# mastbaum/sxmc

Hardware: AMD Instinct MI355X
Metric: NLL evals/sec (10^8 samples, 3 obs, 12 signals) + experiments/sec at 1/2/4/8 GPUs (higher is better)
Workload: dtype f64 exact; f32-on-u16-codes filter decides the unambiguous samples

## Files before the change

sxmc_amd/csrc/fill_kernels.inc.h:

```cpp
#pragma once

#include "sxmc_device_types.h"

#pragma clang fp contract(off)

#ifndef SXMC_MEASURE
#define SXMC_MEASURE 0
#endif

namespace sxfill {

__device__ __forceinline__ constexpr unsigned sx_dbg(unsigned dbg_arg) { return SXMC_MEASURE ? dbg_arg : 0u; }

template <int N>
struct IntC {
  static constexpr int value = N;
  constexpr operator int() const { return N; }
};
template <unsigned long... I>
struct ISeq {};
template <int N, unsigned long... I>
struct MakeISeq : MakeISeq<N - 1, (unsigned long)(N - 1), I...> {};
template <unsigned long... I>
struct MakeISeq<0, I...> {
// ... 350 lines not shown

    double lo[NOBS], hi[NOBS], sc[NOBS];
    int st[NOBS];
#pragma unroll
    for (int k = 0; k < NOBS; k++) {
      lo[k] = d.lower[k];
      hi[k] = d.upper[k];
      sc[k] = d.scale[k];
      st[k] = d.bin_stride[k];
    }

    unsigned cnt = 0;

    auto stage = [&](Columns<NSLOT, PREW>& buf, const unsigned long long vc) {
      double f[NSLOT][SXMC_VEC];
#pragma unroll
      for (int k = 0; k < NSLOT; k++) {
        if (slot_loaded<NOBS, PREW, PROG>(k)) {
          f[k][0] = (double)buf.v[k].x;
          f[k][1] = (double)buf.v[k].y;
          f[k][2] = (double)buf.v[k].z;
          f[k][3] = (double)buf.v[k].w;
        } else {
          f[k][0] = f[k][1] = f[k][2] = f[k][3] = 0.0;
        }
      }
      typename PreVec<PREW>::type prebits = buf.pre;
#pragma unroll
      for (int k = 0; k < NSLOT; k++) {
        if (slot_loaded<NOBS, PREW, PROG>(k)) {
#pragma unroll
          for (int q = 0; q < SXMC_VEC; q++) asm volatile("" : "+v"(f[k][q]));
        }
      }
      if constexpr (PREW != 0) asm volatile("" : "+v"(prebits));
      const unsigned long long vl = vc + step;
      load_columns<NOBS, NSLOT, PREW, PROG>(buf, col, precol, (vl < v1 && !(dbg & 2u)) ? vl : vlast);
      if (dbg & 1u) {
#pragma unroll
        for (int k = 0; k < NSLOT; k++) {
#pragma unroll
          for (int q = 0; q < SXMC_VEC; q++) cnt += (f[k][q] == 12345.678) ? 1u : 0u;
        }
        if constexpr (PREW != 0) cnt += (pre_value<PREW>(prebits, 0) == 12345u) ? 1u : 0u;
        return;
      }

      if constexpr (PROG::dynamic) {
        for (int s = 0; s < nsyst; s++) {
          apply_op<NSLOT>(f, (unsigned)__builtin_amdgcn_readlane((int)opword, s), coef);
        }
      } else {
        run_static<NSLOT>(f, craw, PROG{}, typename MakeISeq<PROG::n>::type{});
      }

      const unsigned dead = (vc < v1) ? 0u : 1u;
      unsigned okbin[SXMC_VEC];
#pragma unroll
      for (int q = 0; q < SXMC_VEC; q++) {
        unsigned bad = dead;
        int bin = 0;
        if constexpr (PREW != 0) {
          const unsigned pv = pre_value<PREW>(prebits, q);
          if constexpr (PREW != kPreGranule) bad += (pv == pre_sentinel<PREW>()) ? 1u : 0u;
          bin = (int)pv;
        }
#pragma unroll
        for (int k = 0; k < NOBS; k++) {
          if (!slot_loaded<NOBS, PREW, PROG>(k)) continue;
          const double x = f[k][q];
          bad += !(x >= lo[k]) ? 1u : 0u;
          bad += !(x < hi[k]) ? 1u : 0u;
          const int idx = (int)((x - lo[k]) * sc[k]);
          if (LDS_HIST) {
            bin = (k == NOBS - 1 && PREW != kPreGranule) ? bin + idx : __mul24(idx, st[k]) + bin;
          } else {
            bin += idx * st[k];
          }
        }
        const unsigned in_domain = (bad == 0u) ? 1u : 0u;
        cnt += in_domain;
        const bool store = (bad == 0u) && ((unsigned)bin < B) && !(dbg & 4u);
        if (LDS_HIST) {
          const unsigned slot = store ? (unsigned)bin : trash;
          __hip_atomic_fetch_add(&hist[slot], 1u, __ATOMIC_RELAXED, __HIP_MEMORY_SCOPE_WORKGROUP);
        } else {
          okbin[q] = store ? (unsigned)bin : 0xFFFFFFFFu;
        }
      }
      if (!LDS_HIST) {
        if (sparse) {
#pragma unroll
          for (int q = 0; q < SXMC_VEC; q++) {
            const unsigned hc = (okbin[q] != 0xFFFFFFFFu) ? (okbin[q] * 0xC2B2AE35u) >> cshift : 0u;
            const unsigned hd = (okbin[q] != 0xFFFFFFFFu) ? (okbin[q] * 0x27D4EB2Fu) >> cshift : 0u;
            if (!((hist[hc >> 5] >> (hc & 31u)) & (hist[hd >> 5] >> (hd & 31u)) & 1u)) okbin[q] = 0xFFFFFFFFu;
          }
          unsigned hb[SXMC_VEC], word[SXMC_VEC];
#pragma unroll
          for (int q = 0; q < SXMC_VEC; q++) {
            hb[q] = (okbin[q] != 0xFFFFFFFFu) ? (okbin[q] * 0x9E3779B1u) >> d.sparse_filter_shift : 0u;
            word[q] = to_global(d.sparse_filter)[hb[q] >> 5];
          }
#pragma unroll
          for (int q = 0; q < SXMC_VEC; q++) {
            if (okbin[q] != 0xFFFFFFFFu && ((word[q] >> (hb[q] & 31u)) & 1u)) sparse_lookup(d, gbins, okbin[q]);
          }
        } else {
#pragma unroll
          for (int q = 0; q < SXMC_VEC; q++) {
            if (okbin[q] != 0xFFFFFFFFu) {
              __hip_atomic_fetch_add(&gbins[okbin[q]], 1u, __ATOMIC_RELAXED, __HIP_MEMORY_SCOPE_AGENT);
            }
          }
        }
      }
    };

    unsigned long long v = vfirst;
    const unsigned long long niter = (v1 - v0 + step - 1) / step;
    for (unsigned long long it = 0; it < niter; ++it, v += step) stage(bufA, v);

#pragma unroll
    for (int off = kWave / 2; off > 0; off >>= 1) cnt += __shfl_down(cnt, off, kWave);
    if (lane == 0 && cnt != 0u) {
      __hip_atomic_fetch_add(s_norm, cnt, __ATOMIC_RELAXED, __HIP_MEMORY_SCOPE_WORKGROUP);
    }
    __syncthreads();

    if (LDS_HIST) {
#pragma unroll 4
      for (unsigned b = tid; b < B; b += nthreads) {
        const unsigned c = hist[b];
        if (c != 0u) __hip_atomic_fetch_add(&gbins[b], c, __ATOMIC_RELAXED, __HIP_MEMORY_SCOPE_AGENT);
      }
      if (si + 1u < seg_end) {
        __syncthreads();
        for (unsigned b = tid; b < B; b += nthreads) hist[b] = 0u;
      }
    }
    if (tid == 0) {
      const unsigned c = *s_norm;
      if (c != 0u) __hip_atomic_fetch_add(to_global(d.norm), c, __ATOMIC_RELAXED, __HIP_MEMORY_SCOPE_AGENT);
      *s_norm = 0u;
    }
    __syncthreads();
    lds_clean = true;
  }
}

constexpr int kPreOrdered = 5;
constexpr int kPreBoxed = 6;
constexpr unsigned kOrdMixed = 0xFFFFFFFEu, kOrdSkip = 0xFFFFFFFFu;
typedef float vfloat2 __attribute__((ext_vector_type(2)));

template <unsigned OPC>
__device__ __forceinline__ void apply_ordered_scalar(double& x, const double* c) {
  constexpr int type = (int)(OPC & 15u);
  static_assert(sx_op_npars(OPC) == 1 && (type == SXMC_SYST_SHIFT || type == SXMC_SYST_SCALE || type == SXMC_SYST_CTSCALE),
                "not a monotone systematic");
  const double pc = 0.0 + c[0] * 1.0;
  if constexpr (type == SXMC_SYST_SHIFT) x = x + pc;
  if constexpr (type == SXMC_SYST_SCALE) x = x * (1 + pc);
  if constexpr (type == SXMC_SYST_CTSCALE) x = 1 + (x - 1) * (1 + pc);
}
template <int ORD, unsigned... OPS, unsigned long... I>
__device__ __forceinline__ void run_ordered_scalar(double& x, const double* c, StaticProg<OPS...>, ISeq<I...>) {
  ([&] {
    if constexpr ((int)((OPS >> 4) & 15u) == ORD) apply_ordered_scalar<OPS>(x, c + sx_prog_cstart<OPS...>((int)I));
  }(), ...);
}
template <int NSLOT, int ORD, bool WANT, unsigned... OPS, unsigned long... I>
__device__ __forceinline__ void run_static_part(double (&f)[NSLOT][SXMC_VEC], const double* c, StaticProg<OPS...>,
                                                ISeq<I...>) {
  ([&] {
    if constexpr (((int)((OPS >> 4) & 15u) == ORD) == WANT) apply_static<NSLOT, OPS>(f, c + sx_prog_cstart<OPS...>((int)I));
  }(), ...);
}
template <int NQ>
struct AffineForm {
  double a[NQ];
  double c;
  double mag;
};

template <int NQ, unsigned OPC>
__device__ __forceinline__ void apply_affine(AffineForm<NQ> (&f)[NQ], const double* coef) {
  constexpr int type = (int)(OPC & 15u), K = (int)((OPC >> 4) & 15u), E = (int)((OPC >> 8) & 15u);
  static_assert(sx_op_npars(OPC) == 1 && K < NQ, "not an affine systematic");
  const double p = 0.0 + coef[0] * 1.0;
  const double ap = __builtin_fabs(p);
  if constexpr (type == SXMC_SYST_SHIFT) {
    f[K].c = f[K].c + p;
    f[K].mag = f[K].mag + ap;
  }
  if constexpr (type == SXMC_SYST_SCALE) {
    const double s = 1 + p;
#pragma unroll
    for (int m = 0; m < NQ; m++) f[K].a[m] = f[K].a[m] * s;
    f[K].c = f[K].c * s;
    f[K].mag = f[K].mag * (1 + ap);
  }
  if constexpr (type == SXMC_SYST_CTSCALE) {
    const double s = 1 + p;
#pragma unroll
    for (int m = 0; m < NQ; m++) f[K].a[m] = f[K].a[m] * s;
    f[K].c = 1 + (f[K].c - 1) * s;
    f[K].mag = 1 + (f[K].mag + 1) * (1 + ap);
  }
  if constexpr (type == SXMC_SYST_RESOLUTION_SCALE) {
    static_assert(E < NQ, "slot out of range");
#pragma unroll
    for (int m = 0; m < NQ; m++) f[K].a[m] = f[K].a[m] + p * (f[K].a[m] - f[E].a[m]);
    f[K].c = f[K].c + p * (f[K].c - f[E].c);
    f[K].mag = f[K].mag + ap * (f[K].mag + f[E].mag);
  }
}
template <int NQ, int ORD, unsigned... OPS, unsigned long... I>
__device__ __forceinline__ void run_affine(AffineForm<NQ> (&f)[NQ], const double* c, StaticProg<OPS...>, ISeq<I...>) {
  ([&] {
    if constexpr ((int)((OPS >> 4) & 15u) != ORD) apply_affine<NQ, OPS>(f, c + sx_prog_cstart<OPS...>((int)I));
  }(), ...);
}
template <int ORD, unsigned... OPS>
constexpr bool prog_is_affine(StaticProg<OPS...>) {
  return (true && ... && ((int)((OPS >> 4) & 15u) == ORD || sx_op_npars(OPS) == 1));
}
__device__ __forceinline__ float uniform_f(float x) {
  return __builtin_bit_cast(float, __builtin_amdgcn_readfirstlane(__builtin_bit_cast(int, x)));
}

typedef unsigned vuint2g __attribute__((ext_vector_type(2)));
typedef unsigned vuint4g __attribute__((ext_vector_type(4)));

template <int NOBS, int NSLOT, typename PROG, bool ORDERED = false>
__device__ __forceinline__ void fill_sparse_body(const SxSignalDesc* __restrict__ descs,
                                                 const SxSegment* __restrict__ segs,
                                                 const unsigned* __restrict__ blk_off, unsigned smax, unsigned dbg_arg) {
  const unsigned dbg = sx_dbg(dbg_arg);
  static_assert(!PROG::dynamic, "static programs only");
  static_assert(!ORDERED || (NOBS >= 1 && NOBS < NSLOT), "unsupported");
  constexpr int ORD = NSLOT - 1, NSTREAM = ORDERED ? NSLOT - 1 : NSLOT;
  typedef typename MakeISeq<PROG::n>::type Seq;
  extern __shared__ unsigned lds[];
  const unsigned tid = threadIdx.x;
  const unsigned lane = tid & (kWave - 1);
  const unsigned wave = tid / kWave;
  unsigned* wkeys = lds + (size_t)wave * 2u * smax;
  unsigned* wcnt = wkeys + smax;
  for (unsigned b = lane; b < smax; b += kWave) wcnt[b] = 0u;

  const unsigned seg_end = blk_off[blockIdx.x + 1];
  for (unsigned si = blk_off[blockIdx.x]; si < seg_end; ++si) {
    const SxSegment& sg = segs[si];
    const SxSignalDesc& d = descs[sg.sig];
    const unsigned long long v0 = sg.v0;
    const unsigned long long v1 = sg.v1;
    const unsigned long long step = sg.step;
    const unsigned B = (unsigned)d.sparse_real_nbins;
    gptr<unsigned> gcnt = to_global(d.bins);
    gptr<const unsigned> tkeys = to_global(d.sparse_tkeys);
    gptr<const unsigned> tslot = to_global(d.sparse_tslot);
    gptr<const vuint2g> dir = to_global(reinterpret_cast<const vuint2g*>(d.sparse_dir));

    double craw[PROG::ncoef > 0 ? PROG::ncoef : 1];
#pragma unroll
    for (int q = 0; q < PROG::ncoef; q++) craw[q] = to_global(d.params)[(long)d.coef_par[q] * d.param_stride];
    __builtin_amdgcn_sched_barrier(0);

    gptr<const vfloat4> col[NSLOT];
#pragma unroll
    for (int k = 0; k < NSLOT; k++) {
      col[k] = to_global(reinterpret_cast<const vfloat4*>(d.cols + (unsigned long long)d.slot_col[k] * d.col_pitch));
    }
    gptr<const vuint2g> gkp = to_global(reinterpret_cast<const vuint2g*>(d.pre));
    const unsigned long long vlast = v1 - 1;
    const unsigned long long vfirst = v0 + tid;

    vfloat4 raw[NSLOT];
    vuint2g kp;
    auto load = [&](unsigned long long v) {
#pragma unroll
      for (int k = 0; k < NSTREAM; k++) {
        raw[k] = __builtin_nontemporal_load(&col[k][v]);
        __builtin_amdgcn_sched_barrier(0);
      }
      kp = gkp[v >> 6];
      __builtin_amdgcn_sched_barrier(0);
    };
    load(vfirst < v1 ? vfirst : vlast);

    double lo[NOBS], hi[NOBS], sc[NOBS];
    int stv[NOBS];
    unsigned nb[NOBS];
#pragma unroll
    for (int k = 0; k < NOBS; k++) {
      lo[k] = d.lower[k];
      hi[k] = d.upper[k];
      sc[k] = d.scale[k];
      stv[k] = d.bin_stride[k];
      asm volatile("" : "+v"(stv[k]));
      nb[k] = (unsigned)d.nbins[k];
    }

    const double olo = d.lower[ORDERED ? NOBS : 0], ohi = d.upper[ORDERED ? NOBS : 0], osc = d.scale[ORDERED ? NOBS : 0];
    const int ost = d.bin_stride[ORDERED ? NOBS : 0];
// ... 1094 lines not shown
        const unsigned nwords = (unsigned)d.nbins[0] * oSp;
        const float invSp = 1.0f / (float)oSp;
#pragma unroll 4
        for (unsigned w = tid; w < nwords; w += nthreads) {
          const unsigned idx = (unsigned)(((float)w + 0.5f) * invSp);
          const unsigned r = w - idx * oSp;
          unsigned n = 0u;
          for (unsigned rep = 0; rep < R; rep++) n += hist[(unsigned)c * cstride + rep * rstride + oSp + w];
          if (r < oS) {
            total += n;
            if (n != 0u) __hip_atomic_fetch_add(&gbins[idx * oS + r], n, __ATOMIC_RELAXED, __HIP_MEMORY_SCOPE_AGENT);
          }
        }
      }
#pragma unroll 4
      for (unsigned w = tid; LDS_HIST && !outer && w < wend; w += nthreads) {
        unsigned n = 0u;
        for (unsigned r = 0; r < R; r++) n += hist[(unsigned)c * cstride + r * rstride + w];
        total += n;
        if (n != 0u) __hip_atomic_fetch_add(&gbins[lds_slot(w)], n, __ATOMIC_RELAXED, __HIP_MEMORY_SCOPE_AGENT);
      }
      if (use_q) {
#pragma unroll
        for (int off = kWave / 2; off > 0; off >>= 1) total += __shfl_down(total, off, kWave);
        if (lane == 0 && total != 0u) {
          __hip_atomic_fetch_add(&s_norm[c], total, __ATOMIC_RELAXED, __HIP_MEMORY_SCOPE_WORKGROUP);
        }
        __syncthreads();
      }
      if (LDS_HIST && more) {
        __syncthreads();
        for (unsigned b = 4u * tid; b < cstride; b += 4u * nthreads) {
          *reinterpret_cast<vuint4g*>(&hist[(unsigned)c * cstride + b]) = vuint4g{0u, 0u, 0u, 0u};
        }
      }
      if (tid == 0) {
        const unsigned n = s_norm[c];
        if (n != 0u) __hip_atomic_fetch_add(to_global(dc.norm), n, __ATOMIC_RELAXED, __HIP_MEMORY_SCOPE_AGENT);
        s_norm[c] = 0u;
      }
    }
    __syncthreads();
    lds_clean = true;
  }
  SX_WG_STAMP(2);
}

template <unsigned OPC, int XT>
__device__ __forceinline__ void apply_box_interval(double& xl, double& xh, double tl, double th, bool& fin, const double* c) {
  constexpr int type = (int)(OPC & 15u), E = (int)((OPC >> 8) & 15u);
  static_assert(sx_op_npars(OPC) == 1, "not a one-coefficient systematic");
  const double pc = 0.0 + c[0] * 1.0;
  if constexpr (type == SXMC_SYST_SHIFT) {
    xl = xl + pc;
    xh = xh + pc;
  }
  if constexpr (type == SXMC_SYST_SCALE) {
    const double s = 1 + pc, a = xl * s, b = xh * s;
    xl = s >= 0.0 ? a : b;
    xh = s >= 0.0 ? b : a;
  }
  if constexpr (type == SXMC_SYST_CTSCALE) {
    const double s = 1 + pc, a = 1 + (xl - 1) * s, b = 1 + (xh - 1) * s;
    xl = s >= 0.0 ? a : b;
    xh = s >= 0.0 ? b : a;
  }
  if constexpr (type == SXMC_SYST_RESOLUTION_SCALE) {
    static_assert(E == XT, "the boxed observable reads one truth field");
    const double dl = xl - th, dh = xh - tl;
    const double a = pc * dl, b = pc * dh;
    const double ml = pc >= 0.0 ? a : b, mh = pc >= 0.0 ? b : a;
    fin = fin && (__builtin_fabs(dl) < __builtin_inf()) && (__builtin_fabs(dh) < __builtin_inf()) &&
          (__builtin_fabs(ml) < __builtin_inf()) && (__builtin_fabs(mh) < __builtin_inf());
    xl = xl + ml;
    xh = xh + mh;
  }
  fin = fin && (__builtin_fabs(xl) < __builtin_inf()) && (__builtin_fabs(xh) < __builtin_inf());
}
template <int BX, int XT, unsigned... OPS, unsigned long... I>
__device__ __forceinline__ void run_box_interval(double& xl, double& xh, double tl, double th, bool& fin, const double* c,
                                                 StaticProg<OPS...>, ISeq<I...>) {
  ([&] {
    if constexpr ((int)((OPS >> 4) & 15u) == BX) apply_box_interval<OPS, XT>(xl, xh, tl, th, fin, c + sx_prog_cstart<OPS...>((int)I));
  }(), ...);
}
template <int BX, int XT, unsigned... OPS>
constexpr bool prog_is_boxable(StaticProg<OPS...>) {
  return (true && ... &&
          (sx_op_npars(OPS) == 1 && (int)((OPS >> 4) & 15u) != XT &&
           ((int)(OPS & 15u) != SXMC_SYST_RESOLUTION_SCALE ||
            ((int)((OPS >> 4) & 15u) == BX && (int)((OPS >> 8) & 15u) == XT))));
}

#ifndef SXMC_BOX_DRAIN
#define SXMC_BOX_DRAIN 2
#endif
#ifndef SXMC_BOX_GQ
#define SXMC_BOX_GQ 0
#endif
#ifndef SXMC_BOX_PREFETCH
#define SXMC_BOX_PREFETCH 0
#endif
template <int NOBS, int NSLOT, typename PROG>
__device__ __forceinline__ void fill_boxed_body(const SxSignalDesc* __restrict__ descs, const SxSegment* __restrict__ segs,
                                                const unsigned* __restrict__ blk_off, unsigned layout, unsigned dbg_arg) {
  const unsigned dbg = sx_dbg(dbg_arg);
  static_assert(!PROG::dynamic && NOBS == 1 && NSLOT == 3, "one streamed observable, one truth field, the boxed observable");
  constexpr int BX = 2, XT = 1;
  static_assert(prog_is_boxable<BX, XT>(PROG{}), "not a program the boxed form can run");
  constexpr int NC = PROG::ncoef > 0 ? PROG::ncoef : 1;
#ifndef SXMC_BOX_RING
#define SXMC_BOX_RING 8
#endif
  constexpr int kRing = SXMC_BOX_RING;
  constexpr int kDrain = SXMC_BOX_DRAIN;
  static_assert(64 % kRing == 0, "a block of 64 units is a whole number of rounds of the ring");
  typedef typename MakeISeq<PROG::n>::type Seq;
  extern __shared__ unsigned lds[];
  const unsigned tid = threadIdx.x;
  const unsigned nthreads = blockDim.x;
  const unsigned lane = tid & (kWave - 1);
  unsigned* s_norm = lds;
  unsigned* hist = lds + 4;
  const unsigned rstride = layout & 0xFFFFFFu, rlog = (layout >> 24) & 7u, R = 1u << rlog;
  const unsigned cstride = rstride << rlog;
  const unsigned myrep = (lane & (R - 1u)) * rstride;
  const unsigned qlog = layout >> 28;
  const unsigned qwave = qlog ? (1u << qlog) / (nthreads / kWave) : 0u;
  const unsigned gq_min = (unsigned)kRing + 1u;
  const unsigned gq_cap = qwave / 2u > gq_min ? qwave / 2u : gq_min, rq_cap = qwave > gq_cap ? qwave - gq_cap : 0u;
  const unsigned gq_drain = (SXMC_BOX_GQ > 0 && (unsigned)SXMC_BOX_GQ + (unsigned)kRing < gq_cap) ? (unsigned)SXMC_BOX_GQ + (unsigned)kRing : gq_cap;
  unsigned* qrows = lds + 4 + cstride + 64 + 4 + (tid / kWave) * (2u * qwave);
  unsigned* qgran = qrows + 2u * rq_cap;

  bool lds_clean = false;
  const unsigned seg_end = blk_off[blockIdx.x + 1];
  for (unsigned si = blk_off[blockIdx.x]; si < seg_end; ++si) {
    const SxSegment& sg = segs[si];
    const SxSignalDesc& d = descs[sg.sig];
    const unsigned long long v0 = sg.v0, v1 = sg.v1, step = sg.step;
    const unsigned B = (unsigned)d.total_nbins;
    double craw[NC];
#pragma unroll
    for (int q = 0; q < PROG::ncoef; q++) craw[q] = to_global(d.params)[(long)d.coef_par[q] * d.param_stride];
    __builtin_amdgcn_sched_barrier(0);

    gptr<const vfloat4> col[NSLOT];
#pragma unroll
    for (int k = 0; k < NSLOT; k++) {
      col[k] = to_global(reinterpret_cast<const vfloat4*>(d.cols + (unsigned long long)d.slot_col[k] * d.col_pitch));
    }
    gptr<const unsigned> precol = to_global(reinterpret_cast<const unsigned*>(d.pre));
    gptr<const vfloat4> boxes = to_global(reinterpret_cast<const vfloat4*>(d.boxes));
    gptr<const vuint2g> qcol = to_global(d.qcol != nullptr ? reinterpret_cast<const vuint2g*>(d.qcol)
                                                           : reinterpret_cast<const vuint2g*>(d.cols));
    const unsigned vfirst32 = (unsigned)(v0 + tid), step32 = (unsigned)step, vlast32 = (unsigned)(v1 - 1);
    const unsigned vwave32 = vfirst32 - lane;
    const unsigned niter32 = (unsigned)((v1 - v0 + step - 1) / step);

    if (!lds_clean) {
      for (unsigned b = tid; b < cstride; b += nthreads) hist[b] = 0u;
      if (tid < 4) s_norm[tid] = 0u;
      __syncthreads();
    }

    const double lo = d.lower[0], hi = d.upper[0], sc = d.scale[0];
    const int st = d.bin_stride[0];
    const unsigned nbk = (unsigned)d.nbins[0];
    const double olo = d.lower[NOBS], ohi = d.upper[NOBS], osc = d.scale[NOBS];
    const int ost = d.bin_stride[NOBS];
    int stv = st, ostv = ost;
    asm volatile("" : "+v"(stv));
    asm volatile("" : "+v"(ostv));
    const unsigned s_in = (unsigned)st, s_out = s_in * nbk;
    const unsigned oS = B / nbk, oSp = oS | 1u;
    const float inv_in = 1.0f / (float)s_in, inv_out = 1.0f / (float)s_out;
    auto fdiv = [](unsigned x, float inv) -> unsigned { return (unsigned)(((float)x + 0.5f) * inv); };
    auto hist_word = [&](unsigned bin) -> unsigned {
      const unsigned h = fdiv(bin, inv_out), rem = bin - h * s_out, idx = fdiv(rem, inv_in);
      return (idx + 1u) * oSp + h * s_in + (rem - idx * s_in);
    };

    bool wild = false;
#pragma unroll
    for (int q = 0; q < PROG::ncoef; q++) wild = wild || !(__builtin_fabs(craw[q]) < __builtin_inf());

    float af, gf, thr;
    bool use_q = d.qcol != nullptr && rq_cap >= 8u && !wild;
    {
      AffineForm<1> form[1];
      form[0].a[0] = 1.0;
      form[0].c = 0.0;
      const double wlo = d.qbase[0], whi = d.qbase[0] + 65534.0 * d.qstep[0];
      form[0].mag = __builtin_fmax(__builtin_fabs(wlo), __builtin_fabs(whi));
      run_affine<1, BX>(form, craw, PROG{}, Seq{});
      const double alpha = form[0].a[0] * d.qstep[0] * sc;
      const double sum_abs = __builtin_fabs(alpha);
      double g = form[0].c - lo;
      g = g + form[0].a[0] * (d.qbase[0] + 0.5 * d.qstep[0]);
      g = g * sc;
      const double mu = sum_abs * 65536.0 + __builtin_fabs(g) + (double)nbk + 0.25;
      const double epsq = 0.5 * sum_abs * (1.0 + 0x1p-19);
      const double eps = epsq + mu * 0x1p-21 + (form[0].mag + __builtin_fabs(lo)) * sc * 0x1p-44;
      const bool ok = eps < 0.125;
      const double e = eps * 1.01, slack = 0x1p-23;
      af = uniform_f((float)alpha);
      gf = uniform_f((float)(g + e));
      thr = uniform_f((float)(2.0 * e + slack));
      use_q = use_q && (uniform_i(ok ? 1 : 0) != 0);
    }

    unsigned vcnt = 0u;
    unsigned nrow = 0u, ngran = 0u;

    unsigned gword = kOrdSkip, greal = 0u;
    vfloat4 bx_next;
    unsigned pre_next;
    auto meta_load = [&](unsigned it) {
      unsigned vg = vwave32 + (it + lane) * step32;
      vg = vg <= vlast32 ? vg : vlast32;
      bx_next = boxes[vg >> 6];
      pre_next = precol[vg >> 6];
    };
    auto granule_meta = [&](unsigned it) {
      unsigned vg = vwave32 + (it + lane) * step32;
      const bool live = vg <= vlast32;
      vg = live ? vg : vlast32;
      if constexpr (!SXMC_BOX_PREFETCH) meta_load(it);
      const vfloat4 bx = bx_next;
      const unsigned pre = pre_next;
      if constexpr (SXMC_BOX_PREFETCH) meta_load(it + 64u);
      double xl = (double)bx.x, xh = (double)bx.y;
      const double tl = (double)bx.z, th = (double)bx.w;
      bool fin = (__builtin_fabs(xl) < __builtin_inf()) && (__builtin_fabs(xh) < __builtin_inf()) &&
                 (__builtin_fabs(tl) < __builtin_inf()) && (__builtin_fabs(th) < __builtin_inf());
      run_box_interval<BX, XT>(xl, xh, tl, th, fin, craw, PROG{}, Seq{});
      const int i0 = (int)((xl - olo) * osc), i1 = (int)((xh - olo) * osc);
      const int e0 = !(xl >= olo) ? -1 : (!(xl < ohi) ? 0x7FFFFFFF : i0);
      const int e1 = !(xh >= olo) ? -1 : (!(xh < ohi) ? 0x7FFFFFFF : i1);
      const unsigned off = (pre & 0xFFFFFFu) + (unsigned)e0 * (unsigned)ost;
      const unsigned h = fdiv(off, inv_out), rem = off - h * s_out;
      const bool canon = off < (1u << 22) && rem < s_in && (h + 1u) * s_out <= B;
      const bool mixed = !use_q || !fin || e0 != e1 || !canon;
      const bool skip = fin && e0 == e1 && (e0 < 0 || e0 == 0x7FFFFFFF);
      gword = !live ? kOrdSkip : skip ? kOrdSkip : mixed ? kOrdMixed : h * s_in + rem;
      greal = off;
    };

    auto push_granule = [&](unsigned it) {
      if (lane == 0) qgran[2u * ngran] = vwave32 + it * step32;
      ngran += 1u;
    };
    auto push_rows = [&](unsigned rare, unsigned v, unsigned real_off) -> bool {
      unsigned long long mask[SXMC_VEC];
      unsigned total = 0u;
#pragma unroll
      for (int q = 0; q < SXMC_VEC; q++) {
        mask[q] = __builtin_amdgcn_ballot_w64(((rare >> q) & 1u) != 0u);
        total += (unsigned)__builtin_popcountll(mask[q]);
      }
      if (nrow + total > rq_cap) return false;
#pragma unroll
      for (int q = 0; q < SXMC_VEC; q++) {
        if (mask[q] == 0ull) continue;
        const unsigned below = __builtin_amdgcn_mbcnt_hi((unsigned)(mask[q] >> 32),
                                                         __builtin_amdgcn_mbcnt_lo((unsigned)mask[q], 0u));
        if ((rare >> q) & 1u) {
          const unsigned pos = nrow + below;
          qrows[2u * pos] = v * SXMC_VEC + (unsigned)q;
          qrows[2u * pos + 1u] = real_off;
        }
        nrow += (unsigned)__builtin_popcountll(mask[q]);
      }
      return true;
    };

    const int oS4 = (int)(4u * oSp);
    const int oclamp = (dbg & 4u) ? -1 : (int)nbk;
    auto coarse_unit = [&](const vuint2g& w, unsigned it, unsigned v, unsigned word0) {
      int base4 = (int)(4u * (4u + myrep + word0) + 4u * oSp);
      asm volatile("" : "+v"(base4));
      const float c0 = (float)(w.x & 0xFFFFu), c1 = (float)(w.x >> 16), c2 = (float)(w.y & 0xFFFFu), c3 = (float)(w.y >> 16);
      const vfloat2 a2 = {af, af}, g2 = {gf, gf};
      const vfloat2 u01 = __builtin_elementwise_fma(a2, vfloat2{c0, c1}, g2);
      const vfloat2 u23 = __builtin_elementwise_fma(a2, vfloat2{c2, c3}, g2);
      const float us[SXMC_VEC] = {u01.x, u01.y, u23.x, u23.y};
      int addr[SXMC_VEC];
      bool amb[SXMC_VEC];
#pragma unroll
      for (int q = 0; q < SXMC_VEC; q++) {
        const float u = us[q];
        amb[q] = !(__builtin_amdgcn_fractf(u) >= thr);
        int idx;
        asm("v_cvt_flr_i32_f32 %0, %1" : "=v"(idx) : "v"(u));
        int ie;
        asm("v_med3_i32 %0, %1, -1, %2" : "=v"(ie) : "v"(amb[q] ? -1 : idx), "s"(oclamp));
        addr[q] = mad24(ie, oS4, base4);
      }
      const float cmax = __builtin_fmaxf(__builtin_fmaxf(c0, c1), __builtin_fmaxf(c2, c3));
      const bool special = cmax >= (float)SXMC_QCODE_EXACT;
      const bool anyamb = (amb[0] | amb[1]) | (amb[2] | amb[3]);
      if (__builtin_amdgcn_ballot_w64(anyamb || special) != 0ull) {
        const float cs[SXMC_VEC] = {c0, c1, c2, c3};
        unsigned rare = 0u;
#pragma unroll
        for (int q = 0; q < SXMC_VEC; q++) {
          rare |= amb[q] ? (1u << q) : 0u;
          if (cs[q] >= (float)SXMC_QCODE_EXACT) {
            addr[q] = base4 - oS4;
            rare = cs[q] >= (float)SXMC_QCODE_NEVER ? (rare & ~(1u << q)) : (rare | (1u << q));
          }
        }
        const unsigned real_off = (unsigned)__builtin_amdgcn_readlane((int)greal, (int)(it & 63u));
        if (!push_rows(rare, v, real_off)) {
          push_granule(it);
          return;
        }
      }
      if (dbg & 32u) {
        vcnt += (unsigned)(addr[0] ^ addr[1] ^ addr[2] ^ addr[3]) == 12345u ? 1u : 0u;
        return;
      }
#pragma unroll
      for (int q = 0; q < SXMC_VEC; q++) {
        unsigned* wp = reinterpret_cast<unsigned*>(reinterpret_cast<char*>(lds) + addr[q]);
        __hip_atomic_fetch_add(wp, 1u, __ATOMIC_RELAXED, __HIP_MEMORY_SCOPE_WORKGROUP);
      }
    };

    auto count_exact = [&](bool ind, int bin) {
      vcnt += (ind && !((unsigned)bin < B)) ? 1u : 0u;
      if (ind && ((unsigned)bin < B)) {
        __hip_atomic_fetch_add(&hist[myrep + hist_word((unsigned)bin)], 1u, __ATOMIC_RELAXED, __HIP_MEMORY_SCOPE_WORKGROUP);
      }
    };
    auto drain = [&]() {
      if (dbg & 16u) nrow = ngran = 0u;
      vfloat4 rawf[kDrain][NSLOT];
      unsigned prew[kDrain];
      auto load_granule = [&](int s, unsigned g) {
        const unsigned vw = (unsigned)uniform_i((int)qgran[2u * g]);
        const unsigned vc = vw + lane < vlast32 ? vw + lane : vlast32;
#pragma unroll
        for (int k = 0; k < NSLOT; k++) rawf[s][k] = __builtin_nontemporal_load(&col[k][vc]);
        prew[s] = precol[vc >> 6];
      };
      unsigned row = 0u, w1 = 0u;
      float rowf = 0.0f;
      if (lane < nrow) {
        row = qrows[2u * lane];
        w1 = qrows[2u * lane + 1u];
        rowf = ((gptr<const float>)col[0])[row];
      }
#pragma unroll
      for (int s = 0; s < kDrain; s++) {
        if ((unsigned)s < ngran) load_granule(s, (unsigned)s);
      }
      for (unsigned i0 = 0; i0 < nrow; i0 += kWave) {
        if (i0 != 0u && i0 + lane < nrow) {
          row = qrows[2u * (i0 + lane)];
          w1 = qrows[2u * (i0 + lane) + 1u];
          rowf = ((gptr<const float>)col[0])[row];
        }
        if (i0 + lane < nrow) {
          double f[NSLOT][SXMC_VEC];
#pragma unroll
          for (int k = 0; k < NSLOT; k++) f[k][0] = f[k][1] = f[k][2] = f[k][3] = 0.0;
          f[0][0] = f[0][1] = f[0][2] = f[0][3] = (double)rowf;
          run_static_part<NSLOT, BX, false>(f, craw, PROG{}, Seq{});
          const double x = f[0][0];
          const bool ind = (x >= lo) & (x < hi);
          const int idx = (int)((x - lo) * sc);
          count_exact(ind, mad24(idx, stv, (int)w1));
        }
      }
      for (unsigned g0 = 0; g0 < ngran; g0 += (unsigned)kDrain) {
        if (g0 != 0u) {
#pragma unroll
          for (int s = 0; s < kDrain; s++) {
            if (g0 + (unsigned)s < ngran) load_granule(s, g0 + (unsigned)s);
          }
        }
#pragma unroll
        for (int s = 0; s < kDrain; s++) {
          if (g0 + (unsigned)s >= ngran) break;
          const unsigned off = (unsigned)uniform_i((int)prew[s]) & 0xFFFFFFu;
          double f[NSLOT][SXMC_VEC];
#pragma unroll
          for (int k = 0; k < NSLOT; k++) {
            f[k][0] = (double)rawf[s][k].x;
            f[k][1] = (double)rawf[s][k].y;
            f[k][2] = (double)rawf[s][k].z;
            f[k][3] = (double)rawf[s][k].w;
          }
          run_static<NSLOT>(f, craw, PROG{}, Seq{});
#pragma unroll
          for (int q = 0; q < SXMC_VEC; q++) {
            const double x = f[0][q], y = f[BX][q];
            const bool ind = (x >= lo) & (x < hi) & (y >= olo) & (y < ohi);
            const int idx = (int)((x - lo) * sc), oidx = (int)((y - olo) * osc);
            count_exact(ind, mad24(oidx, ostv, mad24(idx, stv, (int)off)));
          }
        }
      }
      nrow = ngran = 0u;
    };

    vuint2g rq[kRing];
    const unsigned vfirst8 = vfirst32 * 8u, vlast8 = vlast32 * 8u, step8 = step32 * 8u;
    auto issue = [&](int slot, unsigned it) {
      unsigned o = vfirst8 + it * step8;
      o = o < vlast8 ? o : vlast8;
      rq[slot] = __builtin_nontemporal_load((gptr<const vuint2g>)((gptr<const char>)qcol + (unsigned long long)o));
      __builtin_amdgcn_sched_barrier(0);
    };
    const unsigned climit = (unsigned)uniform_i((int)oS);
    {
      unsigned it = 0u;
      if constexpr (SXMC_BOX_PREFETCH) meta_load(0u);
#pragma unroll
      for (int i = 0; i < kRing; i++) issue(i, (unsigned)i);
      while (it < niter32) {
        if ((it & 63u) == 0u) granule_meta(it);
        const unsigned block_end = niter32 < (it | 63u) + 1u ? niter32 : (it | 63u) + 1u;
        bool full = false;
        while (it < block_end && !full) {
#pragma unroll
          for (int i = 0; i < kRing; i++) {
#pragma unroll
            for (int e = 0; e < 2; e++) asm volatile("" : "+v"(rq[i][e]));
            const unsigned iu = it + (unsigned)i;
            if (iu < block_end) {
              const unsigned word0 = (unsigned)__builtin_amdgcn_readlane((int)gword, (int)(iu & 63u));
              if (dbg & 1u) {
                vcnt += (rq[i].x == 12345u && word0 == 77u) ? 1u : 0u;
              } else if (word0 < climit) coarse_unit(rq[i], iu, vfirst32 + iu * step32, word0);
              else if (word0 == kOrdMixed) push_granule(iu);
            }
            issue(i, iu + (unsigned)kRing);
          }
          it = block_end - it < (unsigned)kRing ? block_end : it + (unsigned)kRing;
          full = ngran + (unsigned)kRing > gq_drain;
        }
        if (full) {
          drain();
          __builtin_amdgcn_s_waitcnt(0);
        }
      }
    }
    drain();

    {
      unsigned t = vcnt;
#pragma unroll
      for (int off = kWave / 2; off > 0; off >>= 1) t += __shfl_down(t, off, kWave);
      if (lane == 0 && t != 0u) __hip_atomic_fetch_add(&s_norm[0], t, __ATOMIC_RELAXED, __HIP_MEMORY_SCOPE_WORKGROUP);
    }
    __syncthreads();
    {
      gptr<unsigned> gbins = to_global(d.bins);
      const bool more = si + 1u < seg_end;
      const unsigned nwords = nbk * oSp;
      const float invSp = 1.0f / (float)oSp;
      unsigned total = 0u;
#pragma unroll 4
      for (unsigned w = tid; w < nwords; w += nthreads) {
        const unsigned idx = fdiv(w, invSp), r = w - idx * oSp;
        unsigned n = 0u;
        for (unsigned rep = 0; rep < R; rep++) n += hist[rep * rstride + oSp + w];
        if (r < oS) {
          total += n;
          const unsigned h = fdiv(r, inv_in);
          if (n != 0u) {
            __hip_atomic_fetch_add(&gbins[h * s_out + idx * s_in + (r - h * s_in)], n, __ATOMIC_RELAXED, __HIP_MEMORY_SCOPE_AGENT);
          }
        }
      }
#pragma unroll
      for (int off = kWave / 2; off > 0; off >>= 1) total += __shfl_down(total, off, kWave);
      if (lane == 0 && total != 0u) __hip_atomic_fetch_add(&s_norm[0], total, __ATOMIC_RELAXED, __HIP_MEMORY_SCOPE_WORKGROUP);
      __syncthreads();
      if (more) {
        for (unsigned b = 4u * tid; b < cstride; b += 4u * nthreads) {
          *reinterpret_cast<vuint4g*>(&hist[b]) = vuint4g{0u, 0u, 0u, 0u};
        }
      }
      if (tid == 0) {
        const unsigned n = s_norm[0];
        if (n != 0u) __hip_atomic_fetch_add(to_global(d.norm), n, __ATOMIC_RELAXED, __HIP_MEMORY_SCOPE_AGENT);
        s_norm[0] = 0u;
      }
    }
    __syncthreads();
    lds_clean = true;
  }
}

template <int NOBS, int NSLOT, bool LDS_HIST, typename PROG, int PREW>
__global__ __launch_bounds__(1024) void fill_kernel(const SxSignalDesc* __restrict__ descs,
                                                    const SxSegment* __restrict__ segs,
                                                    const unsigned* __restrict__ blk_off, unsigned hist_words,
                                                    unsigned dbg) {
  fill_body<NOBS, NSLOT, LDS_HIST, PROG, PREW>(descs, segs, blk_off, hist_words, dbg);
}

template <int NOBS, int NSLOT, typename PROG>
__global__ __launch_bounds__(1024) void fill_sparse_kernel(const SxSignalDesc* __restrict__ descs,
                                                           const SxSegment* __restrict__ segs,
                                                           const unsigned* __restrict__ blk_off, unsigned smax,
                                                           unsigned dbg) {
  fill_sparse_body<NOBS, NSLOT, PROG>(descs, segs, blk_off, smax, dbg);
}

#ifndef SXMC_ORDERED_BOUND
#define SXMC_ORDERED_BOUND 1024
#endif
template <int NOBS, int NSLOT, typename PROG, bool LDS_HIST = true>
__global__ __launch_bounds__(SXMC_ORDERED_BOUND) void fill_ordered_kernel(const SxSignalDesc* __restrict__ descs,
                                                            const SxSegment* __restrict__ segs,
                                                            const unsigned* __restrict__ blk_off, unsigned layout,
                                                            unsigned dbg) {
  SxChainDescs one;
  one.d[0] = one.d[1] = one.d[2] = one.d[3] = descs;
  fill_ordered_body<NOBS, NSLOT, PROG, 1, LDS_HIST>(one, segs, blk_off, layout, dbg);
}

template <int NOBS, int NSLOT, typename PROG>
__global__ __launch_bounds__(SXMC_ORDERED_BOUND) void fill_boxed_kernel(const SxSignalDesc* __restrict__ descs,
                                                          const SxSegment* __restrict__ segs,
                                                          const unsigned* __restrict__ blk_off, unsigned layout,
                                                          unsigned dbg) {
  fill_boxed_body<NOBS, NSLOT, PROG>(descs, segs, blk_off, layout, dbg);
}

}
```

sxmc_amd/csrc/layout_kernels.hip:

```cpp
#include "nll_device.h"

#include <hipcub/hipcub.hpp>

#include <cmath>
#include <cstring>
#include <limits>

#pragma clang fp contract(off)

namespace {

struct KeyPlan {
  unsigned mask;
  unsigned outside;
  unsigned radix[SXMC_MAX_NFIELDS];
};

__global__ __launch_bounds__(256) void bucket_key_kernel(const SxSignalDesc* __restrict__ dp, KeyPlan plan,
                                                         const unsigned* __restrict__ rows_in,
                                                         unsigned* __restrict__ keys, unsigned* __restrict__ rows) {
  const SxSignalDesc& d = *dp;
  const unsigned long long n = d.nsamples;
  const unsigned long long step = (unsigned long long)gridDim.x * blockDim.x;
  for (unsigned long long i = (unsigned long long)blockIdx.x * blockDim.x + threadIdx.x; i < n; i += step) {
    const unsigned long long row = rows_in ? rows_in[i] : i;
    bool ok = true;
    unsigned key = 0;
    for (int k = 0; k < d.nobs; k++) {
      if (!((plan.mask >> k) & 1u)) continue;
      const double x = (double)d.cols[(unsigned long long)k * d.col_pitch + row];
      ok = ok && (x >= d.lower[k]) && (x < d.upper[k]);
      key += (unsigned)(int)((x - d.lower[k]) * d.scale[k]) * plan.radix[k];
    }
    keys[i] = ok ? key : plan.outside;
    rows[i] = (unsigned)row;
  }
}

__global__ __launch_bounds__(256) void order_key_kernel(const float* __restrict__ col, unsigned long long n,
                                                        unsigned* __restrict__ keys, unsigned* __restrict__ rows) {
  const unsigned long long step = (unsigned long long)gridDim.x * blockDim.x;
  for (unsigned long long i = (unsigned long long)blockIdx.x * blockDim.x + threadIdx.x; i < n; i += step) {
    const float x = col[i];
    const unsigned u = __float_as_uint(x);
    keys[i] = (x != x) ? 0xFFFFFFFFu : ((u >> 31) ? ~u : (u | 0x80000000u));
    rows[i] = (unsigned)i;
  }
}

__global__ __launch_bounds__(256) void bucket_edges_kernel(const float* __restrict__ col,
                                                           const unsigned* __restrict__ valid,
                                                           unsigned long long ngranules, float* __restrict__ edges) {
  const unsigned long long step = (unsigned long long)gridDim.x * blockDim.x;
  for (unsigned long long p = (unsigned long long)blockIdx.x * blockDim.x + threadIdx.x; p < ngranules; p += step) {
    const unsigned nv = valid[p] ? valid[p] : 1u;
    edges[2 * p] = col[p * 256ull];
    edges[2 * p + 1] = col[p * 256ull + nv - 1u];
  }
}

struct BoxStrata {
  int n;
  unsigned bound[16];
};
__global__ __launch_bounds__(256) void box_key_kernel(const float* __restrict__ colx, const float* __restrict__ colt,
                                                      unsigned long long n, int pass, BoxStrata strata,
                                                      unsigned* __restrict__ keys, unsigned* __restrict__ rows) {
  const unsigned long long step = (unsigned long long)gridDim.x * blockDim.x;
  for (unsigned long long i = (unsigned long long)blockIdx.x * blockDim.x + threadIdx.x; i < n; i += step) {
    const float x = colx[i], d = x - colt[i];
    const unsigned ud = __float_as_uint(d), kd = (ud >> 31) ? ~ud : (ud | 0x80000000u);
    unsigned key;
    if (pass == 1) {
      key = (d != d) ? 0xFFFFFFFFu : kd;
    } else {
      const unsigned ux = __float_as_uint(x), kx = (ux >> 31) ? ~ux : (ux | 0x80000000u);
      unsigned s = 0;
      for (int k = 0; k + 1 < strata.n; k++) s += strata.bound[k] <= kd ? 1u : 0u;
      key = (d != d || x != x) ? 0xFFFFFFFFu : ((s << 28) | (kx >> 4));
    }
    keys[i] = key;
    rows[i] = (unsigned)i;
  }
}

__global__ __launch_bounds__(256) void bucket_boxes_kernel(const float* __restrict__ colx, const float* __restrict__ colt,
                                                           const unsigned* __restrict__ valid,
                                                           unsigned long long ngranules, float* __restrict__ boxes) {
  const unsigned lane = threadIdx.x & 63u;
  const unsigned long long wave = ((unsigned long long)blockIdx.x * blockDim.x + threadIdx.x) >> 6;
  const unsigned long long nwaves = ((unsigned long long)gridDim.x * blockDim.x) >> 6;
  for (unsigned long long p = wave; p < ngranules; p += nwaves) {
    const unsigned nv = valid[p];
    float xl = __builtin_inff(), xh = -__builtin_inff(), tl = __builtin_inff(), th = -__builtin_inff();
    bool bad = false;
    for (unsigned i = lane; i < nv; i += 64u) {
      const float x = colx[p * 256ull + i], t = colt[p * 256ull + i];
      bad = bad || !(fabsf(x) < __builtin_inff()) || !(fabsf(t) < __builtin_inff());
      xl = fminf(xl, x);
      xh = fmaxf(xh, x);
      tl = fminf(tl, t);
      th = fmaxf(th, t);
    }
    for (int off = 32; off > 0; off >>= 1) {
      xl = fminf(xl, __shfl_down(xl, off, 64));
      xh = fmaxf(xh, __shfl_down(xh, off, 64));
      tl = fminf(tl, __shfl_down(tl, off, 64));
      th = fmaxf(th, __shfl_down(th, off, 64));
    }
    const bool anybad = __ballot(bad) != 0ull || nv == 0u;
    if (lane == 0) {
      const float nanv = __int_as_float(0x7fc00000);
      boxes[4 * p] = anybad ? nanv : xl;
      boxes[4 * p + 1] = anybad ? nanv : xh;
      boxes[4 * p + 2] = anybad ? nanv : tl;
      boxes[4 * p + 3] = anybad ? nanv : th;
    }
  }
}

__global__ __launch_bounds__(256) void bucket_first_kernel(const unsigned* __restrict__ sorted_keys,
                                                           unsigned long long n, unsigned* __restrict__ first) {
  const unsigned long long step = (unsigned long long)gridDim.x * blockDim.x;
  for (unsigned long long i = (unsigned long long)blockIdx.x * blockDim.x + threadIdx.x; i < n; i += step) {
    const unsigned k = sorted_keys[i];
    if (i == 0 || sorted_keys[i - 1] != k) first[k] = (unsigned)i;
  }
}

struct GatherCols {
  int ncols;
  int col[SXMC_MAX_NFIELDS];
};

__global__ __launch_bounds__(256) void bucket_gather_kernel(const float* __restrict__ cols, unsigned long long pitch,
                                                            GatherCols gc, const unsigned* __restrict__ sorted_rows,
                                                            const unsigned* __restrict__ src,
                                                            const unsigned* __restrict__ valid,
                                                            unsigned long long ngranules, float* __restrict__ out,
                                                            unsigned long long out_pitch) {
  for (unsigned long long p = blockIdx.x; p < ngranules; p += gridDim.x) {
    const unsigned i = threadIdx.x;
    const bool live = i < valid[p];
    const unsigned row = live ? sorted_rows[(unsigned long long)src[p] + i] : 0u;
    for (int c = 0; c < gc.ncols; c++) {
      out[(unsigned long long)c * out_pitch + p * 256ull + i] =
          live ? cols[(unsigned long long)gc.col[c] * pitch + row] : __int_as_float(0x7fc00000);
    }
  }
}

struct CodePlan {
  int nslots;
  double base[SXMC_MAX_QSLOTS], step[SXMC_MAX_QSLOTS];
};

__device__ __forceinline__ unsigned ordered_bits(float x) {
  const unsigned u = __float_as_uint(x);
  return (u >> 31) ? ~u : (u | 0x80000000u);
}

__global__ __launch_bounds__(256) void column_minmax_kernel(const float* __restrict__ cols, unsigned long long pitch,
                                                            int ncols, unsigned long long n, unsigned* __restrict__ mm) {
  const unsigned long long step = (unsigned long long)gridDim.x * blockDim.x;
  for (int c = 0; c < ncols; c++) {
    unsigned lo = 0xFFFFFFFFu, hi = 0u;
    for (unsigned long long i = (unsigned long long)blockIdx.x * blockDim.x + threadIdx.x; i < n; i += step) {
      const float x = cols[(unsigned long long)c * pitch + i];
      if (fabsf(x) < __builtin_inff()) {
        const unsigned b = ordered_bits(x);
        lo = b < lo ? b : lo;
        hi = b > hi ? b : hi;
      }
    }
    for (int off = 32; off > 0; off >>= 1) {
      const unsigned l2 = __shfl_down(lo, off, 64), h2 = __shfl_down(hi, off, 64);
      lo = l2 < lo ? l2 : lo;
      hi = h2 > hi ? h2 : hi;
    }
    if ((threadIdx.x & 63u) == 0u) {
      if (lo != 0xFFFFFFFFu) atomicMin(&mm[2 * c], lo);
      if (hi != 0u) atomicMax(&mm[2 * c + 1], hi);
    }
  }
}

__global__ __launch_bounds__(256) void column_codes_kernel(const float* __restrict__ cols, unsigned long long pitch,
                                                           CodePlan plan, unsigned long long n,
                                                           unsigned* __restrict__ qcol, unsigned* __restrict__ tally) {
  const unsigned long long step = (unsigned long long)gridDim.x * blockDim.x;
  unsigned nexact = 0u, nnever = 0u;
  for (unsigned long long i = (unsigned long long)blockIdx.x * blockDim.x + threadIdx.x; i < n; i += step) {
    unsigned code[SXMC_MAX_QSLOTS] = {0u, 0u, 0u, 0u};
    bool never = false, exact = false;
    for (int m = 0; m < plan.nslots; m++) {
      const double x = (double)cols[(unsigned long long)m * pitch + i];
      if (!(fabs(x) < __builtin_inf())) {
        never = true;
        continue;
      }
      const double t = (x - plan.base[m]) / plan.step[m];
      if (!(t >= 0.0 && t < (double)(SXMC_QCODE_MAX + 1u))) {
        exact = true;
        continue;
      }
      const unsigned q = (unsigned)t;
      const double centre = plan.base[m] + ((double)q + 0.5) * plan.step[m];
      if (!(fabs(x - centre) <= 0.5 * plan.step[m] * (1.0 + 0x1p-20))) exact = true;
      code[m] = q;
    }
    if (never) code[0] = SXMC_QCODE_NEVER; else if (exact) code[0] = SXMC_QCODE_EXACT;
    nexact += (!never && exact) ? 1u : 0u;
    nnever += never ? 1u : 0u;
    for (int w = 0; w < (plan.nslots + 1) / 2; w++) {
      qcol[(unsigned long long)w * pitch + i] = (code[2 * w] << 16) | (2 * w + 1 < plan.nslots ? code[2 * w + 1] : 0u);
    }
  }
  if (nexact) atomicAdd(&tally[0], nexact);
  if (nnever) atomicAdd(&tally[1], nnever);
}

__global__ __launch_bounds__(256) void column_codes16_kernel(const float* __restrict__ col, double base, double qstep,
                                                             unsigned long long n, unsigned short* __restrict__ qcol,
                                                             unsigned* __restrict__ tally) {
  const unsigned long long step = (unsigned long long)gridDim.x * blockDim.x;
  unsigned nexact = 0u, nnever = 0u;
  for (unsigned long long i = (unsigned long long)blockIdx.x * blockDim.x + threadIdx.x; i < n; i += step) {
    const double x = (double)col[i];
    unsigned code;
    if (!(fabs(x) < __builtin_inf())) {
      code = SXMC_QCODE_NEVER;
      nnever++;
    } else {
      const double t = (x - base) / qstep;
      bool exact = !(t >= 0.0 && t < (double)(SXMC_QCODE_MAX + 1u));
      const unsigned q = exact ? 0u : (unsigned)t;
      const double centre = base + ((double)q + 0.5) * qstep;
      if (!(fabs(x - centre) <= 0.5 * qstep * (1.0 + 0x1p-20))) exact = true;
      code = exact ? SXMC_QCODE_EXACT : q;
      nexact += exact ? 1u : 0u;
    }
    qcol[i] = (unsigned short)code;
  }
  if (nexact) atomicAdd(&tally[0], nexact);
  if (nnever) atomicAdd(&tally[1], nnever);
}

struct SampleGeom {
  int nobs;
  int has_cuts;
  int nbins[3];
  double lower[3], upper[3], width[3];
  double scale[3];
  float bottom[3], top[3];
  float cut_lo[3], cut_hi[3];
};

__device__ __forceinline__ int sample_side(float xf, unsigned idx, double lower, double upper, double scale) {
  const double x = (double)xf;
  if (!(x >= lower)) return -1;
  if (!(x < upper)) return 1;
  const long long j = (long long)((x - lower) * scale);
  return j < (long long)idx ? -1 : j > (long long)idx ? 1 : 0;
}

__device__ __forceinline__ float sample_float(double xd, unsigned idx, const SampleGeom& g, int k) {
  const float x0 = (float)xd;
  float xf = x0;
  for (int step = 0; step < 4; step++) {
    const int s = sample_side(xf, idx, g.lower[k], g.upper[k], g.scale[k]);
    if (s == 0) return xf;
    xf = nextafterf(xf, s < 0 ? __builtin_inff() : -__builtin_inff());
  }
  if (sample_side(xf, idx, g.lower[k], g.upper[k], g.scale[k]) == 0) return xf;
  xf = x0;
  if (!((double)xf >= g.lower[k])) xf = g.bottom[k];
  if (!((double)xf < g.upper[k])) xf = g.top[k];
  return xf;
}

__global__ __launch_bounds__(256) void random_sample_kernel(const unsigned* __restrict__ cdf, unsigned nbins_total,
                                                            SampleGeom g, unsigned long long seed,
                                                            unsigned long long n, float dataset,
                                                            float* __restrict__ out, unsigned* __restrict__ exhausted) {
  const unsigned total = cdf[nbins_total - 1];
  const unsigned long long step = (unsigned long long)gridDim.x * blockDim.x;
  for (unsigned long long e = (unsigned long long)blockIdx.x * blockDim.x + threadIdx.x; e < n; e += step) {
    float x[3] = {0.0f, 0.0f, 0.0f};
    for (unsigned attempt = 0; attempt < 1024; attempt++) {
      const sxdev::Philox4 r = sxdev::philox4x32_10(e, attempt, seed);
      const unsigned target = (unsigned)(((unsigned long long)r.x * total) >> 32);
      unsigned lo = 0, hi = nbins_total - 1;
      while (lo < hi) {
        const unsigned mid = (lo + hi) >> 1;
        if (cdf[mid] > target) hi = mid; else lo = mid + 1;
      }
      unsigned flat = lo;
      const unsigned u[3] = {r.y, r.z, r.w};
      bool ok = true;
      for (int k = g.nobs - 1; k >= 0; k--) {
        const unsigned idx = flat % (unsigned)g.nbins[k];
        flat /= (unsigned)g.nbins[k];
        const double xd = g.lower[k] + ((double)idx + ((double)u[k] + 0.5) * 2.3283064365386963e-10) * g.width[k];
        x[k] = sample_float(xd, idx, g, k);
        if (g.has_cuts) ok = ok && !(x[k] > g.cut_hi[k] || x[k] < g.cut_lo[k]);
      }
      if (ok) break;
      if (attempt == 1023) atomicAdd(exhausted, 1u);
    }
    for (int k = 0; k < g.nobs; k++) out[e * (unsigned long long)(g.nobs + 1) + k] = x[k];
    out[e * (unsigned long long)(g.nobs + 1) + g.nobs] = dataset;
  }
}

unsigned grid_for(unsigned long long n, unsigned cap) {
  unsigned long long b = (n + 255) / 256;
  if (b < 1) b = 1;
  return (unsigned)(b > cap ? cap : b);
}

}

hipError_t sx_bucket_keys(const SxSignalDesc* d_desc, unsigned long long nsamples, unsigned mask, const unsigned* radix,
                          unsigned outside, const unsigned* d_rows_in, unsigned* d_keys, unsigned* d_rows,
                          hipStream_t s) {
  if (nsamples == 0) return hipSuccess;
  KeyPlan plan;
  plan.mask = mask;
  plan.outside = outside;
  for (int k = 0; k < SXMC_MAX_NFIELDS; k++) plan.radix[k] = radix[k];
  hipLaunchKernelGGL(bucket_key_kernel, dim3(grid_for(nsamples, 16384)), dim3(256), 0, s, d_desc, plan, d_rows_in, d_keys,
                     d_rows);
  return hipGetLastError();
}

hipError_t sx_order_keys(const float* d_col, unsigned long long nsamples, unsigned* d_keys, unsigned* d_rows,
                         hipStream_t s) {
  if (nsamples == 0) return hipSuccess;
  hipLaunchKernelGGL(order_key_kernel, dim3(grid_for(nsamples, 16384)), dim3(256), 0, s, d_col, nsamples, d_keys, d_rows);
  return hipGetLastError();
}

hipError_t sx_box_keys(const float* d_colx, const float* d_colt, unsigned long long nsamples, int pass, int nstrata,
                       const unsigned* bounds, unsigned* d_keys, unsigned* d_rows, hipStream_t s) {
  if (nsamples == 0) return hipSuccess;
  if (nstrata < 1 || nstrata > 16) return hipErrorInvalidValue;
  BoxStrata st{};
  st.n = nstrata;
  for (int k = 0; k + 1 < nstrata; k++) st.bound[k] = bounds ? bounds[k] : 0u;
  hipLaunchKernelGGL(box_key_kernel, dim3(grid_for(nsamples, 16384)), dim3(256), 0, s, d_colx, d_colt, nsamples, pass, st,
                     d_keys, d_rows);
  return hipGetLastError();
}

hipError_t sx_bucket_boxes(const float* d_colx, const float* d_colt, const unsigned* d_valid, unsigned long long ngranules,
                           float* d_boxes, hipStream_t s) {
  if (ngranules == 0) return hipSuccess;
  hipLaunchKernelGGL(bucket_boxes_kernel, dim3(grid_for(ngranules * 64ull, 16384)), dim3(256), 0, s, d_colx, d_colt, d_valid,
                     ngranules, d_boxes);
  return hipGetLastError();
}

hipError_t sx_bucket_edges(const float* d_col, const unsigned* d_valid, unsigned long long ngranules, float* d_edges,
                           hipStream_t s) {
  if (ngranules == 0) return hipSuccess;
  hipLaunchKernelGGL(bucket_edges_kernel, dim3(grid_for(ngranules, 4096)), dim3(256), 0, s, d_col, d_valid, ngranules,
                     d_edges);
  return hipGetLastError();
}

hipError_t sx_bucket_sort(const unsigned* keys_in, unsigned* keys_out, const unsigned* rows_in, unsigned* rows_out,
                          unsigned long long n, int bits, hipStream_t s) {
  if (n == 0) return hipSuccess;
  if (n > 0x7FFFFFFFull) return hipErrorInvalidValue;
  size_t temp_bytes = 0;
  hipError_t e = hipcub::DeviceRadixSort::SortPairs(nullptr, temp_bytes, keys_in, keys_out, rows_in, rows_out, (int)n, 0,
                                                    bits, s);
  if (e != hipSuccess) return e;
  void* temp = nullptr;
  e = hipMalloc(&temp, temp_bytes ? temp_bytes : 16);
  if (e != hipSuccess) return e;
  e = hipcub::DeviceRadixSort::SortPairs(temp, temp_bytes, keys_in, keys_out, rows_in, rows_out, (int)n, 0, bits, s);
  hipError_t e2 = hipStreamSynchronize(s);
  (void)hipFree(temp);
  return e != hipSuccess ? e : e2;
}

hipError_t sx_bucket_first(const unsigned* sorted_keys, unsigned long long n, unsigned* d_first, hipStream_t s) {
  if (n == 0) return hipSuccess;
  hipLaunchKernelGGL(bucket_first_kernel, dim3(grid_for(n, 16384)), dim3(256), 0, s, sorted_keys, n, d_first);
  return hipGetLastError();
}

hipError_t sx_bucket_gather(const float* cols, unsigned long long pitch, int ncols, const int* col_list,
                            const unsigned* sorted_rows, const unsigned* d_src, const unsigned* d_valid,
                            unsigned long long ngranules, float* out, unsigned long long out_pitch, hipStream_t s) {
  if (ngranules == 0 || ncols == 0) return hipSuccess;
  GatherCols gc;
  gc.ncols = ncols;
  for (int c = 0; c < SXMC_MAX_NFIELDS; c++) gc.col[c] = c < ncols ? col_list[c] : 0;
  const unsigned grid = (unsigned)(ngranules > 65536ull * 4 ? 65536ull * 4 : ngranules);
  hipLaunchKernelGGL(bucket_gather_kernel, dim3(grid), dim3(256), 0, s, cols, pitch, gc, sorted_rows, d_src, d_valid,
                     ngranules, out, out_pitch);
  return hipGetLastError();
}

hipError_t sx_column_minmax(const float* cols, unsigned long long pitch, int ncols, unsigned long long n, float* out,
                            hipStream_t s) {
  if (ncols <= 0 || ncols > SXMC_MAX_NFIELDS) return hipErrorInvalidValue;
  unsigned h[2 * SXMC_MAX_NFIELDS];
  for (int c = 0; c < ncols; c++) {
    h[2 * c] = 0xFFFFFFFFu;
    h[2 * c + 1] = 0u;
  }
  unsigned* d = nullptr;
  hipError_t e = hipMalloc((void**)&d, sizeof(unsigned) * 2 * ncols);
  if (e != hipSuccess) return e;
  e = hipMemcpyAsync(d, h, sizeof(unsigned) * 2 * ncols, hipMemcpyHostToDevice, s);
  if (e == hipSuccess && n) {
    hipLaunchKernelGGL(column_minmax_kernel, dim3(grid_for(n, 2048)), dim3(256), 0, s, cols, pitch, ncols, n, d);
    e = hipGetLastError();
  }
  if (e == hipSuccess) e = hipMemcpyAsync(h, d, sizeof(unsigned) * 2 * ncols, hipMemcpyDeviceToHost, s);
  hipError_t e2 = hipStreamSynchronize(s);
  (void)hipFree(d);
  if (e != hipSuccess) return e;
  if (e2 != hipSuccess) return e2;
  for (int c = 0; c < 2 * ncols; c++) {
    const bool none = h[2 * (c / 2)] == 0xFFFFFFFFu && h[2 * (c / 2) + 1] == 0u;
    const unsigned b = h[c], u = (b >> 31) ? (b & 0x7FFFFFFFu) : ~b;
    float x;
    std::memcpy(&x, &u, 4);
    out[c] = none ? ((c & 1) ? -1.0f : 1.0f) : x;
  }
  return hipSuccess;
}

hipError_t sx_column_codes(const float* cols, unsigned long long pitch, int nslots, const double* base, const double* step,
                           unsigned long long n, unsigned* qcol, unsigned long long* tally, hipStream_t s) {
  if (nslots < 1 || nslots > SXMC_MAX_QSLOTS) return hipErrorInvalidValue;
  CodePlan plan{};
  plan.nslots = nslots;
  for (int m = 0; m < nslots; m++) {
    plan.base[m] = base[m];
    plan.step[m] = step[m];
  }
  unsigned* d = nullptr;
  hipError_t e = hipMalloc((void**)&d, sizeof(unsigned) * 2);
  if (e != hipSuccess) return e;
  e = hipMemsetAsync(d, 0, sizeof(unsigned) * 2, s);
  if (e == hipSuccess && n) {
    hipLaunchKernelGGL(column_codes_kernel, dim3(grid_for(n, 16384)), dim3(256), 0, s, cols, pitch, plan, n, qcol, d);
    e = hipGetLastError();
  }
  unsigned h[2] = {0u, 0u};
  if (e == hipSuccess) e = hipMemcpyAsync(h, d, sizeof h, hipMemcpyDeviceToHost, s);
  hipError_t e2 = hipStreamSynchronize(s);
  (void)hipFree(d);
  if (tally) {
    tally[0] = h[0];
    tally[1] = h[1];
  }
  return e != hipSuccess ? e : e2;
}

hipError_t sx_column_codes16(const float* col, double base, double step, unsigned long long n, unsigned short* qcol,
                             unsigned long long* tally, hipStream_t s) {
  unsigned* d = nullptr;
  hipError_t e = hipMalloc((void**)&d, sizeof(unsigned) * 2);
  if (e != hipSuccess) return e;
  e = hipMemsetAsync(d, 0, sizeof(unsigned) * 2, s);
  if (e == hipSuccess && n) {
    hipLaunchKernelGGL(column_codes16_kernel, dim3(grid_for(n, 16384)), dim3(256), 0, s, col, base, step, n, qcol, d);
    e = hipGetLastError();
  }
  unsigned h[2] = {0u, 0u};
  if (e == hipSuccess) e = hipMemcpyAsync(h, d, sizeof h, hipMemcpyDeviceToHost, s);
  hipError_t e2 = hipStreamSynchronize(s);
  (void)hipFree(d);
  if (tally) {
    tally[0] = h[0];
    tally[1] = h[1];
  }
  return e != hipSuccess ? e : e2;
}

hipError_t sx_hist_cdf(const unsigned* d_bins, unsigned* d_cdf, int nbins_total, hipStream_t s) {
  size_t temp_bytes = 0;
  hipError_t e = hipcub::DeviceScan::InclusiveSum(nullptr, temp_bytes, d_bins, d_cdf, nbins_total, s);
  if (e != hipSuccess) return e;
  void* temp = nullptr;
  e = hipMalloc(&temp, temp_bytes ? temp_bytes : 16);
  if (e != hipSuccess) return e;
  e = hipcub::DeviceScan::InclusiveSum(temp, temp_bytes, d_bins, d_cdf, nbins_total, s);
  hipError_t e2 = hipStreamSynchronize(s);
  (void)hipFree(temp);
  return e != hipSuccess ? e : e2;
}

hipError_t sx_inclusive_sum_u32(const unsigned* d_in, unsigned* d_out, int n, void* temp, size_t& temp_bytes,
                                hipStream_t s) {
  return hipcub::DeviceScan::InclusiveSum(temp, temp_bytes, d_in, d_out, n, s);
}

hipError_t sx_random_sample(const unsigned* d_cdf, int nbins_total, int nobs, const int* nbins, const double* lower,
                            const double* upper, const double* scale, const float* cut_lo, const float* cut_hi,
                            unsigned long long seed, unsigned long long n, float dataset, float* d_out,
// ... 24 lines not shown
```

sxmc_amd/csrc/sxmc_device.h:

```cpp
#pragma once

#include <hip/hip_runtime.h>
#include <stdint.h>

#include <string>

#include "../../include/sxmc_hip.h"

#include "sxmc_device_types.h"

struct SxStepArgs {
  size_t nsignals, nsources;
  const double* means;
  const double* sigmas;
  sxmc_rng_state* rng;
  double* nll_current;
  double* nll_proposed;
  double* v_current;
  double* v_proposed;
  int* accepted;
  int* counter;
  float* jump_buffer;
  int nparameters;
  int debug_mode;
  const float* jump_width;
  const double* nexpected;
  const unsigned* n_mc;
  const short* source_id;
  const unsigned* norms;
  unsigned* gate = nullptr;
  unsigned gate_value = 0;
};

#define SXMC_MAX_LOCKSTEP 4
struct SxChainEnd {
  const SxSignalDesc* lookup_descs;
  const SxSignalDesc* hist_descs;
  unsigned long long nrows;
  const unsigned* weight;
  double* sums;
  unsigned* ticket;
  unsigned nblocks;
  SxStepArgs a;
};
struct SxChainEnds {
  SxChainEnd c[SXMC_MAX_LOCKSTEP];
};

struct SxLaunchShape {
  int nobs;
  int nslot;
  int lds_hist;
  int threads;
  int grid;
  size_t lds_bytes;
  int debug_mode;
  int static_prog;
  void* rtc_fill;
  void* rtc_sparse;
  int sparse_runs;
  size_t sparse_lds_bytes;
  unsigned lds_layout;
  int pre_width;
  void* ev_start = nullptr;
  void* ev_stop = nullptr;
  const void* tail = nullptr;
  int tail_blocks = 0;
};
bool sx_fill_has_step_form(const SxLaunchShape& sh);
size_t sx_tail_args_bytes();
void sx_tail_args_fill(void* image, const SxSignalDesc* lookup_descs, const SxSignalDesc* hist_descs, int nsig,
                       int max_bins, unsigned long long npoints, const unsigned* weight, unsigned long long* slots,
                       double* last_good, unsigned* sync, int nvb, const struct SxStepArgs& a);

struct SxRtcSpec {
  int nobs, nslot, lds_hist, pre_width, sparse_runs;
  int nchain;
  int max_threads;
  int nops;
  unsigned ops[SXMC_MAX_SYST];
};
bool sx_rtc_compile_only(const SxRtcSpec& k, size_t* code_bytes, std::string* err);
void* sx_rtc_get(const SxRtcSpec& k, std::string* err);
struct SxChainDescsHost {
  const SxSignalDesc* d[4];
};
hipError_t sx_rtc_launch_multi(void* fn, int grid, int threads, size_t lds_bytes, const SxChainDescsHost& chains,
                               const SxSegment* segs, const unsigned* blk_off, unsigned hist_words, unsigned dbg,
                               hipStream_t s, void* ev_start = nullptr, void* ev_stop = nullptr);
hipError_t sx_rtc_launch(void* fn, int grid, int threads, size_t lds_bytes, const SxSignalDesc* descs,
                         const SxSegment* segs, const unsigned* blk_off, unsigned w, unsigned dbg, hipStream_t s,
                         void* ev_start = nullptr, void* ev_stop = nullptr);

hipError_t sx_launch_zero(const SxSignalDesc* d_descs, int nsig, int max_bins, unsigned* ticket, hipStream_t s);
hipError_t sx_launch_step_end(const SxSignalDesc* lookup_descs, const SxSignalDesc* hist_descs, int nsig, int max_bins,
                              unsigned long long npoints, const unsigned* weight, unsigned long long* slots,
                              double* last_good, unsigned* sync, int nvb, const SxStepArgs& a, hipStream_t s);
hipError_t sx_launch_step_end2(const SxSignalDesc* lookup_a, const SxSignalDesc* lookup_b, const SxSignalDesc* hist_a,
                               const SxSignalDesc* hist_b, int nsig, int max_bins, unsigned long long npoints,
                               const unsigned* weight_a, const unsigned* weight_b, unsigned long long* slots,
                               double* last_good, unsigned* sync, int nvb, const unsigned* norms_b, double* v_b,
                               const int* cap, const SxStepArgs& a, hipStream_t s);
hipError_t sx_step_end_slots_init(unsigned long long* slots, double* last_good, int n);
int sx_step_end_resident_capacity(int nsig, int cus);
hipError_t sx_launch_chain_ends(const SxChainEnds& e, int nchains, int nsig, int max_bins, int block, hipStream_t s);
hipError_t sx_launch_finish_zero(const SxSignalDesc* d_descs, int nsig, int max_bins, size_t npartial,
                                 const double* sums, unsigned* ticket, const SxStepArgs& a, int block, hipStream_t s);
hipError_t sx_launch_eval_nll_finish(const SxSignalDesc* d_descs, int nsig, unsigned long long npoints,
                                      const unsigned* weight, double* sums, unsigned* ticket, const SxStepArgs& a,
                                      int grid, int block, hipStream_t s);
hipError_t sx_launch_eval_nll2(const SxSignalDesc* descs_a, const SxSignalDesc* descs_b, int nsig,
                               unsigned long long npoints, const unsigned* weight_a, const unsigned* weight_b,
                               const double* pars_a, const double* pars_b, const double* nexpected,
                               const unsigned* n_mc, const short* source_id, const unsigned* norms_a,
                               const unsigned* norms_b, double* sums_a, double* sums_b, int half, int block,
                               hipStream_t s);
hipError_t sx_launch_finish2_zero(const SxSignalDesc* descs_a, const SxSignalDesc* descs_b, int nsig, int max_bins,
                                  size_t npartial, const double* sums_a, const double* sums_b, const unsigned* norms_b,
                                  double* v_b, const int* cap, const SxStepArgs& a, int block, hipStream_t s);
hipError_t sx_launch_peek_next_proposal(int nparameters, const sxmc_rng_state* rng, const float* jump_width,
                                        const double* v_current, double* out, hipStream_t s);
hipError_t sx_launch_tail_step(const SxSignalDesc* d_descs, int nsig, unsigned long long npoints,
                               const unsigned* weight, const SxStepArgs& a, hipStream_t s);
hipError_t sx_launch_fill(const SxLaunchShape& shape, const SxSignalDesc* d_descs, const SxSegment* d_segs,
                          const unsigned* d_blk_off, hipStream_t s);
hipError_t sx_launch_fill_sparse_runs(const SxLaunchShape& shape, const SxSignalDesc* d_descs, const SxSegment* d_segs,
                                      const unsigned* d_blk_off, hipStream_t s);
bool sx_fill_static_supports_sparse_runs(int prog);

bool sx_fill_has_specialization(int nobs, int nslot);
int sx_fill_find_static_program(int nobs, int nslot, int nops, const unsigned* ops);
int sx_fill_find_ordered_program(int nobs, int nslot, int nops, const unsigned* ops);
int sx_fill_find_boxed_program(int nobs, int nslot, int nops, const unsigned* ops);
bool sx_fill_static_supports(int prog, int lds_hist, int prebin);
hipError_t sx_launch_prebin(const SxSignalDesc* d_desc, unsigned long long npad, unsigned mask, int width, void* out,
                            hipStream_t s);
hipError_t sx_bucket_keys(const SxSignalDesc* d_desc, unsigned long long nsamples, unsigned mask, const unsigned* radix,
                          unsigned outside, const unsigned* d_rows_in, unsigned* d_keys, unsigned* d_rows,
                          hipStream_t s);
hipError_t sx_order_keys(const float* d_col, unsigned long long nsamples, unsigned* d_keys, unsigned* d_rows,
                         hipStream_t s);
hipError_t sx_bucket_edges(const float* d_col, const unsigned* d_valid, unsigned long long ngranules, float* d_edges,
                           hipStream_t s);
hipError_t sx_box_keys(const float* d_colx, const float* d_colt, unsigned long long nsamples, int pass, int nstrata,
                       const unsigned* bounds, unsigned* d_keys, unsigned* d_rows, hipStream_t s);
hipError_t sx_bucket_boxes(const float* d_colx, const float* d_colt, const unsigned* d_valid, unsigned long long ngranules,
                           float* d_boxes, hipStream_t s);
hipError_t sx_column_codes16(const float* col, double base, double step, unsigned long long n, unsigned short* qcol,
                             unsigned long long* tally, hipStream_t s);
hipError_t sx_bucket_sort(const unsigned* keys_in, unsigned* keys_out, const unsigned* rows_in, unsigned* rows_out,
                          unsigned long long n, int bits, hipStream_t s);
hipError_t sx_bucket_first(const unsigned* sorted_keys, unsigned long long n, unsigned* d_first, hipStream_t s);
hipError_t sx_bucket_gather(const float* cols, unsigned long long pitch, int ncols, const int* col_list,
                            const unsigned* sorted_rows, const unsigned* d_src, const unsigned* d_valid,
                            unsigned long long ngranules, float* out, unsigned long long out_pitch, hipStream_t s);
hipError_t sx_column_minmax(const float* cols, unsigned long long pitch, int ncols, unsigned long long n, float* out,
                            hipStream_t s);
hipError_t sx_column_codes(const float* cols, unsigned long long pitch, int nslots, const double* base, const double* step,
                           unsigned long long n, unsigned* qcol, unsigned long long* tally, hipStream_t s);
hipError_t sx_hist_cdf(const unsigned* d_bins, unsigned* d_cdf, int nbins_total, hipStream_t s);
hipError_t sx_random_sample(const unsigned* d_cdf, int nbins_total, int nobs, const int* nbins, const double* lower,
                            const double* upper, const double* scale, const float* cut_lo, const float* cut_hi,
                            unsigned long long seed, unsigned long long n, float dataset, float* d_out,
                            unsigned* d_exhausted, hipStream_t s);
hipError_t sx_launch_eval_pdf(const SxSignalDesc* d_descs, int nsig, unsigned long long max_points,
                              hipStream_t s);
hipError_t sx_launch_eval_nll(const SxSignalDesc* d_descs, int nsig, unsigned long long npoints,
                              const unsigned* weight, const double* pars, const double* nexpected, const unsigned* n_mc,
                              const short* source_id, const unsigned* norms, double* sums,
                              int grid, int block, hipStream_t s);
hipError_t sx_launch_pow_int(const double* x, int n, int i, double* out, hipStream_t s);
hipError_t sx_launch_transpose(const float* aos, float* cols, unsigned long long nsamples,
                               int nfields, unsigned long long col_pitch, hipStream_t s);
hipError_t sx_launch_untranspose_obs(const float* cols, float* out, unsigned long long nsamples,
                                     int nobs, unsigned long long col_pitch, float dataset,
                                     hipStream_t s);

#define SXMC_KDE_MAX_DIM 4
#define SXMC_KDE_TILE 256
struct SxKdeArgs {
  float* rows;
  unsigned long long npad;
  unsigned* norm;
  double lower[SXMC_KDE_MAX_DIM];
  double upper[SXMC_KDE_MAX_DIM];
  double cscale[SXMC_KDE_MAX_DIM];
  double inv_h_sqrt2[SXMC_KDE_MAX_DIM];
};
hipError_t sx_kde_prepass(const SxSignalDesc& d, const SxKdeArgs& a, hipStream_t s);
hipError_t sx_kde_pairs(int D, const float* pts, unsigned long long pitch, const float* rows, unsigned tiles_per_split,
                        unsigned ntiles, int nsplit, double* part, hipStream_t s);
hipError_t sx_kde_combine(const double* part, unsigned long long pitch, int nsplit, unsigned long long npoints,
                          const int* codes, const unsigned* norm, double prefactor, float* out, long stride,
                          hipStream_t s);
struct SxKdeSampleArgs {
  double lower[SXMC_KDE_MAX_DIM];
  double upper[SXMC_KDE_MAX_DIM];
  double h[SXMC_KDE_MAX_DIM];
  double inv_cscale[SXMC_KDE_MAX_DIM];
  float bottom[SXMC_KDE_MAX_DIM];
  float top[SXMC_KDE_MAX_DIM];
  float cut_lo[SXMC_KDE_MAX_DIM];
  float cut_hi[SXMC_KDE_MAX_DIM];
  int has_cuts;
  float dataset;
};
hipError_t sx_kde_compact(const float* rows, int D, unsigned long long npad, unsigned* flag, unsigned* pos,
                          unsigned* idx, void* temp, size_t temp_bytes, hipStream_t s);
hipError_t sx_inclusive_sum_u32(const unsigned* d_in, unsigned* d_out, int n, void* temp, size_t& temp_bytes,
                                hipStream_t s);
hipError_t sx_kde_sample(int D, const float* rows, const unsigned* idx, unsigned n, const SxKdeSampleArgs& g,
                         unsigned long long seed, unsigned long long nevents, float* out, unsigned* exhausted,
                         hipStream_t s);
```

sxmc_amd/csrc/sxmc_device_types.h:

```cpp
#pragma once

#ifndef SXMC_MAX_NFIELDS
#define SXMC_MAX_NFIELDS 10
#define SXMC_MAX_SYST 16
#define SXMC_MAX_SYST_PARS 8
#define SXMC_SYST_SHIFT 0
#define SXMC_SYST_SCALE 1
#define SXMC_SYST_RESOLUTION_SCALE 2
#define SXMC_SYST_CTSCALE 3
#endif

#define SXMC_VEC 4
#define SXMC_OP_NOP (-1)
#define SXMC_SPARSE_EMPTY 0xFFu
#define SXMC_SPARSE_SLOW 0xFEu
#define SXMC_SPARSE_SMAX_LOG2 9
#define SXMC_MAX_QSLOTS 4
#define SXMC_QCODE_MAX 65533u
#define SXMC_QCODE_EXACT 0xFFFEu
#define SXMC_QCODE_NEVER 0xFFFFu

struct SxSystOp {
  short type;
  short obs_slot;
  short extra_slot;
  short npars;
  short pars[SXMC_MAX_SYST_PARS];
  short coef_start;
  short pad[3];
};

struct SxSignalDesc {
  const float* cols;
  unsigned long long col_pitch;
  unsigned long long nsamples;
  unsigned long long nvec;
  unsigned long long vec_start;
  unsigned* bins;
  unsigned* norm;
  int total_nbins;
  int nobs;
  int nslot;
  int nsyst;
  int ncoef;
  int param_stride;
  const double* params;
  int slot_col[SXMC_MAX_NFIELDS];
  int bin_stride[SXMC_MAX_NFIELDS];
  double lower[SXMC_MAX_NFIELDS];
  double upper[SXMC_MAX_NFIELDS];
  double scale[SXMC_MAX_NFIELDS];
  SxSystOp syst[SXMC_MAX_SYST];
  short coef_par[64];
  const void* pre;
  const float* edges;
  const float* boxes;
  const unsigned* sparse_filter;
  const unsigned* sparse_table;
  int sparse_filter_shift;
  int sparse_table_shift;
  int sparse_real_nbins;
  int sparse_coarse_shift;
  const unsigned* sparse_coarse;
  const unsigned* sparse_dir;
  const unsigned* sparse_tkeys;
  const unsigned* sparse_tslot;
  int nbins[SXMC_MAX_NFIELDS];
  const int* read_bins;
  unsigned long long npoints;
  float* pdf_out;
  int pdf_stride;
  int pad0;
  double bin_volume;
  const unsigned* qcol;
  double qbase[SXMC_MAX_QSLOTS];
  double qstep[SXMC_MAX_QSLOTS];
  unsigned* step_gate;
};

struct SxSegment {
  int sig;
  int pad;
  unsigned long long v0, v1, step;
};
```

sxmc_amd/csrc/sxmc_group.cpp:

```cpp
#include "sxmc_host.h"

using namespace sxhost;

namespace sxhost {
std::atomic<int> g_stepping_groups{0};
}

extern "C" {

int sxmc_group_create(const sxmc_hist_t* members, int nmembers, sxmc_group_t* out) {
  SX_REQUIRE(out && nmembers >= 0 && (members || nmembers == 0), "bad arguments");
  for (int i = 0; i < nmembers; i++) SX_REQUIRE(members[i], "null member");
  sxmc_group* g = new sxmc_group;
  g->members.assign(members, members + nmembers);
  hipError_t e = hipMalloc((void**)&g->d_ticket, 256);
  if (e == hipSuccess) e = hipMemset(g->d_ticket, 0, 256);
  if (e == hipSuccess) e = hipMalloc((void**)&g->d_step_sums, 1024 * sizeof(double));
  if (e == hipSuccess) e = hipMalloc((void**)&g->d_coop_slots, sizeof(unsigned long long) * 128);
  if (e == hipSuccess) e = hipMalloc((void**)&g->d_coop_last, sizeof(double) * 128);
  if (e == hipSuccess) e = sx_step_end_slots_init(g->d_coop_slots, g->d_coop_last, 128);
  if (e != hipSuccess) {
    if (g->d_ticket) (void)hipFree(g->d_ticket);
    if (g->d_step_sums) (void)hipFree(g->d_step_sums);
    if (g->d_coop_slots) (void)hipFree(g->d_coop_slots);
// ... 40 lines not shown
  SX_REQUIRE(bin_blocks_per_cu >= 0 && bin_blocks_per_cu <= 16, "bin_blocks_per_cu out of range");
  g->cfg_threads = bin_threads;
  g->cfg_bpc = bin_blocks_per_cu;
  return SXMC_OK;
}

int sxmc_group_optimize(sxmc_group_t g, sxmc_stream_t s, int* chosen_threads) {
  SX_FLUSH();
  SX_ORDER(s);
  SX_REQUIRE(g, "null group");
  SX_REQUIRE(!t_capturing, "not while recording a graph");
  if (chosen_threads) *chosen_threads = 0;
  int rc = group_refresh(g);
  if (rc) return rc;
  rc = group_check_bound(g, false);
  if (rc) return rc;
  if (g->classes.empty() || g->cfg_threads > 0 || g->cfg_bpc > 0) return SXMC_OK;
  for (const LaunchClass& c : g->classes)
    if (!c.light) return SXMC_OK;
  hipStream_t st = (hipStream_t)s;
  hipEvent_t e0, e1;
  SX_HIP(hipEventCreate(&e0));
  SX_HIP(hipEventCreate(&e1));
  bool has_codes = false;
  for (const LaunchClass& c : g->classes) has_codes = has_codes || c.codes;
  typedef std::pair<int, int> Shape;
  const std::vector<Shape> candidates =
      has_codes ? std::vector<Shape>{{512, 2}, {768, 1}, {1024, 1}, {896, 1}, {640, 1}}
                : std::vector<Shape>{{512, 1}, {448, 1}, {576, 1}, {640, 1}, {768, 1}};
  int best_threads = 0, best_bpc = 0;
  float best_ms = 0;
  int failure = SXMC_OK;
  auto timed_fill = [&]() -> float {
    float ms = 1e30f;
    for (int rep = 0; rep < 8 && failure == SXMC_OK; rep++) {
      hipError_t e = hipEventRecord(e0, st);
      g->trial_launches++;
      if (e == hipSuccess) failure = group_fill(g, st, false);
      if (failure == SXMC_OK && e == hipSuccess) e = hipEventRecord(e1, st);
      if (failure == SXMC_OK && e == hipSuccess) e = hipEventSynchronize(e1);
      float t = 0;
      if (failure == SXMC_OK && e == hipSuccess) e = hipEventElapsedTime(&t, e0, e1);
      if (failure == SXMC_OK && e != hipSuccess) failure = fail(SXMC_ERR_HIP, std::string("optimize: ") + hipGetErrorString(e));
      if (rep > 0 && t < ms) ms = t;
    }
    return ms;
  };
  for (const Shape& shape : candidates) {
    const int cand = shape.first;
    g->cfg_threads = cand;
    g->cfg_bpc = shape.second;
    if ((failure = group_refresh(g)) != SXMC_OK) break;
    const float ms = timed_fill();
    if (failure != SXMC_OK) break;
    if (best_threads == 0 || ms < best_ms) {
      best_threads = cand;
      best_bpc = shape.second;
      best_ms = ms;
    }
  }
  const bool is_auto = best_threads == candidates[0].first && best_bpc == candidates[0].second;
  g->cfg_threads = (failure == SXMC_OK && !is_auto) ? best_threads : 0;
  g->cfg_bpc = (failure == SXMC_OK && !is_auto) ? best_bpc : 0;
  bool has_bucketed = false;
  for (const LaunchClass& c : g->classes) has_bucketed = has_bucketed || ((c.shape.pre_width == 3 || c.shape.pre_width == 5 || c.shape.pre_width == 6) && c.shape.lds_hist);
  if (failure == SXMC_OK && has_bucketed && g->cfg_teams == 0) {
    float ms_of[2] = {best_ms, 1e30f};
    for (int pass = 0; pass < 2 && failure == SXMC_OK; pass++) {
      g->cfg_teams = pass == 0 ? 0 : 3;
      if ((failure = group_refresh(g)) != SXMC_OK) break;
      const float ms = timed_fill();
      ms_of[pass] = ms;
    }
    g->cfg_teams = (failure == SXMC_OK && ms_of[1] < 0.985f * ms_of[0]) ? 3 : 0;
  }
  if (failure == SXMC_OK && has_codes && g->cfg_codes < 0) {
    float ms_of[2] = {1e30f, 1e30f};
    for (int pass = 0; pass < 2 && failure == SXMC_OK; pass++) {
      g->cfg_codes = pass == 0 ? -1 : 0;
      if ((failure = group_refresh(g)) != SXMC_OK) break;
      const float ms = timed_fill();
      ms_of[pass] = ms;
    }
    g->cfg_codes = (failure == SXMC_OK && ms_of[1] < 0.97f * ms_of[0]) ? 0 : -1;
  }
  (void)hipEventDestroy(e0);
  (void)hipEventDestroy(e1);
  if (failure != SXMC_OK) return failure;
  if (chosen_threads) *chosen_threads = best_threads;
  return group_refresh(g);
}

int sxmc_group_set_partition_teams(sxmc_group_t g, int teams) {
  SX_REQUIRE(g, "null group");
  SX_REQUIRE(teams >= 0 && teams <= 64, "teams must be 0 (default: one) to 64");
  g->cfg_teams = teams;
  return SXMC_OK;
}

int sxmc_group_set_partition(sxmc_group_t g, int mode) {
  SX_REQUIRE(g, "null group");
  SX_REQUIRE(mode >= 0 && mode <= 2, "partition mode must be 0 (auto), 1 (sliced) or 2 (interleaved)");
  g->cfg_partition = mode;
  return SXMC_OK;
}

int sxmc_group_set_sparse(sxmc_group_t g, int enable) {
  SX_REQUIRE(g, "null group");
  g->cfg_sparse = enable ? 1 : 0;
  return SXMC_OK;
}

int sxmc_group_set_prebinning(sxmc_group_t g, int enable) {
  SX_REQUIRE(g, "null group");
  g->cfg_prebin = enable ? 1 : 0;
  return SXMC_OK;
}

int sxmc_group_set_bucketing(sxmc_group_t g, int enable) {
  SX_REQUIRE(g, "null group");
  g->cfg_bucket = enable ? 1 : 0;
  return SXMC_OK;
}

int sxmc_group_set_ordering(sxmc_group_t g, int enable) {
  SX_REQUIRE(g, "null group");
  g->cfg_order = enable == 2 ? 2 : enable ? 1 : 0;
  return SXMC_OK;
}

int sxmc_group_set_boxes(sxmc_group_t g, int enable) {
  SX_REQUIRE(g, "null group");
  g->cfg_box = enable < 0 ? -1 : enable ? 1 : 0;
  g->box_blocked = false;
  return SXMC_OK;
}

int sxmc_group_set_box_limit(sxmc_group_t g, double bins) {
  SX_REQUIRE(g && bins >= 0.0, "bad arguments");
  g->box_limit = (float)bins;
  return SXMC_OK;
}

int sxmc_group_set_fill_form(sxmc_group_t g, int form) {
  SX_REQUIRE(g && (form == 1 || form == 2), "form: 1 boxed, 2 ordered");
  SX_FLUSH();
  int rc = group_refresh(g);
  if (rc) return rc;
  SX_REQUIRE(g->twin && !g->twin->classes.empty() && g->cfg_box < 0, "the group's plan has one form only");
  g->fill_form = form;
  return SXMC_OK;
}

static int box_image_width(sxmc_group* g, double* width) {
  *width = HUGE_VAL;
  const LaunchClass* cls = nullptr;
  for (const LaunchClass& c : g->classes) cls = (c.dual && !cls) ? &c : cls;
  if (!cls || cls->member_idx.empty() || cls->box_obs < 0) return SXMC_OK;
  const SxSignalDesc& d = g->h_descs[(size_t)cls->member_idx[0]];
  if (!d.params) return SXMC_OK;
  int lo_idx = 1 << 30, hi_idx = -1;
  for (int q = 0; q < d.nsyst; q++) {
    if (d.syst[q].obs_slot != cls->box_obs) continue;
    lo_idx = std::min(lo_idx, (int)d.syst[q].pars[0]);
    hi_idx = std::max(hi_idx, (int)d.syst[q].pars[0]);
  }
  if (hi_idx < 0 || d.param_stride < 1 || (long)(hi_idx - lo_idx) * d.param_stride >= 256) return SXMC_OK;
  if (!g->h_pin) SX_HIP(hipHostMalloc((void**)&g->h_pin, 256 * sizeof(double)));
  const size_t span = (size_t)(hi_idx - lo_idx) * (size_t)d.param_stride + 1;
  SX_HIP(hipMemcpyAsync(g->h_pin, d.params + (long)lo_idx * d.param_stride, span * sizeof(double), hipMemcpyDeviceToHost,
                        g->last_stream));
  SX_HIP(hipStreamSynchronize(g->last_stream));
  double xl = 0.5 * (d.lower[cls->box_obs] + d.upper[cls->box_obs]), xh = xl + (double)cls->box_dx;
  const double tl = xl, th = xl + (double)cls->box_dt;
  bool fin = true;
  for (int q = 0; q < d.nsyst && fin; q++) {
    const SxSystOp& op = d.syst[q];
    if (op.obs_slot != cls->box_obs) continue;
    const double c0 = g->h_pin[(size_t)((int)op.pars[0] - lo_idx) * (size_t)d.param_stride];
    const double pc = 0.0 + c0 * 1.0;
    if (op.type == SXMC_SYST_SHIFT) {
      xl = xl + pc;
      xh = xh + pc;
    } else if (op.type == SXMC_SYST_SCALE || op.type == SXMC_SYST_CTSCALE) {
      const double s = 1 + pc;
      const double a = op.type == SXMC_SYST_SCALE ? xl * s : 1 + (xl - 1) * s;
      const double b = op.type == SXMC_SYST_SCALE ? xh * s : 1 + (xh - 1) * s;
      xl = s >= 0.0 ? a : b;
      xh = s >= 0.0 ? b : a;
    } else if (op.type == SXMC_SYST_RESOLUTION_SCALE) {
      const double dl = xl - th, dh = xh - tl, a = pc * dl, b = pc * dh;
      xl = xl + (pc >= 0.0 ? a : b);
      xh = xh + (pc >= 0.0 ? b : a);
    }
    fin = std::isfinite(xl) && std::isfinite(xh);
  }
  if (fin) *width = (xh - xl) * d.scale[cls->box_obs];
  return SXMC_OK;
}

int sxmc_group_adapt_fill_form(sxmc_group_t g, int* form, int* changed) {
  SX_REQUIRE(g, "null group");
  SX_FLUSH();
  if (form) *form = 0;
  if (changed) *changed = 0;
  if (t_capturing) return fail(SXMC_ERR_STATE, "the form of the fill is not chosen while a graph is being recorded");
  int rc = group_refresh(g);
  if (rc) return rc;
  if (!(g->twin && !g->twin->classes.empty() && g->cfg_box < 0)) return SXMC_OK;
  SX_HIP(hipStreamSynchronize(g->last_stream));
  double width = HUGE_VAL;
  rc = box_image_width(g, &width);
  if (rc) return rc;
  const int want = width < 0.8 * (double)g->box_limit ? 1 : (width < (double)g->box_limit ? g->fill_form : 2);
  if (changed) *changed = want != g->fill_form ? 1 : 0;
  g->fill_form = want;
  if (form) *form = want;
  return SXMC_OK;
}

int sxmc_group_fill_form(sxmc_group_t g, int* form) {
  SX_REQUIRE(g && form, "null argument");
  SX_FLUSH();
  int rc = group_refresh(g);
  if (rc) return rc;
  *form = (g->twin && !g->twin->classes.empty() && g->cfg_box < 0) ? g->fill_form : 0;
  return SXMC_OK;
}

int sxmc_group_set_codes(sxmc_group_t g, int enable) {
  SX_REQUIRE(g, "null group");
  g->cfg_codes = enable < 0 ? -1 : enable ? 1 : 0;
  return SXMC_OK;
}

int sxmc_group_set_codes_queue_log(sxmc_group_t g, int log2_entries) {
  SX_REQUIRE(g, "null group");
  SX_REQUIRE(log2_entries == 0 || (log2_entries >= (int)kMinQueueLog && log2_entries <= 11),
             "the queues of ambiguous rows hold 2^9 .. 2^11 entries (0: as many as fit)");
  g->cfg_queue_log = log2_entries;
  return SXMC_OK;
}

int sxmc_group_codes_info(sxmc_group_t g, int* members, unsigned long long* rows, unsigned long long* exact_rows,
                          unsigned long long* never_rows) {
  SX_REQUIRE(g && members && rows && exact_rows && never_rows, "null argument");
  int rc = group_refresh(g);
  if (rc) return rc;
  *members = 0;
  *rows = *exact_rows = *never_rows = 0;
  for (const LaunchClass& c : g->classes) {
    if (!c.codes) continue;
    for (int idx : c.member_idx) {
      const SampleStore::Bucketed* bk = g->member_bucket[(size_t)idx];
      if (!bk || !bk->d_qcol) continue;
      *members += 1;
      *rows += (unsigned long long)bk->ngranules * 256ull;
      *exact_rows += bk->q_exact_rows;
      *never_rows += bk->q_never_rows;
    }
  }
  return SXMC_OK;
}

int sxmc_group_codes_windows(sxmc_group_t g, int member, int* nfields, double* base, double* step) {
  SX_REQUIRE(g && nfields && base && step, "null argument");
  SX_REQUIRE(member >= 0 && member < (int)g->members.size(), "no such member");
  int rc = group_refresh(g);
  if (rc) return rc;
  *nfields = 0;
  for (const LaunchClass& c : g->classes) {
    if (!c.codes) continue;
    for (int idx : c.member_idx) {
      const SampleStore::Bucketed* bk = g->member_bucket[(size_t)idx];
      if (idx != member || !bk || !bk->d_qcol) continue;
      *nfields = bk->nq;
      for (int m = 0; m < bk->nq; m++) {
        base[m] = bk->qbase[m];
        step[m] = bk->qstep[m];
      }
    }
  }
  return SXMC_OK;
}

int sxmc_group_set_runtime_kernels(sxmc_group_t g, int enable) {
  SX_REQUIRE(g, "null group");
  g->cfg_rtc = enable ? 1 : 0;
  return SXMC_OK;
}

int sxmc_group_launch_info(sxmc_group_t g, char* out, size_t n) {
  SX_REQUIRE(g && out && n > 0, "null argument");
  int rc = group_refresh(g);
  if (rc) return rc;
  std::string text;
  const bool two = g->twin && !g->twin->classes.empty() && g->cfg_box < 0;
  const sxmc_group* plan = (two && g->fill_form == 2) ? g->twin : g;
  for (size_t i = 0; i < plan->classes.size(); i++) {
    const LaunchClass& c = plan->classes[i];
    char line[512];
    const char* kind = c.shape.rtc_fill ? "runtime" : c.shape.static_prog >= 0 ? "builtin" : c.shape.nobs ? "decoded" : "generic";
    std::snprintf(line, sizeof line,
                  "launch %zu: members=%zu nobs=%d nslot=%d hist=%s program=%s table=%s%s threads=%d grid=%d partition=%d teams=%d\n",
                  i, c.member_idx.size(), c.shape.nobs, c.shape.nslot, c.shape.lds_hist ? "lds" : "global", kind,
                  c.shape.pre_width == 6 ? (c.dual ? "boxed+codes(now)|ordered+codes" : "boxed+codes")
                  : (two && plan == g->twin && c.shape.pre_width == 5) ? (c.codes ? "boxed+codes|ordered+codes(now)" : "boxed+codes|ordered(now)")
                  : c.shape.pre_width == 5 ? (c.codes ? "ordered+codes" : "ordered") : c.shape.pre_width == 3 ? "bucketed" : c.shape.pre_width ? "prebinned" : "rows",
                  c.runs_mode ? (c.shape.rtc_sparse ? "+runs(runtime)" : "+runs(builtin)") : "", c.shape.threads,
                  c.shape.grid, c.partition, c.teams);
    text += line;
  }
  if (!g->rtc_note.empty()) text += "runtime specialisation failed: " + g->rtc_note.substr(0, 300) + "\n";
  if (!g->plan_note.empty()) text += "note: " + g->plan_note + "\n";
  std::snprintf(out, n, "%s", text.c_str());
  return SXMC_OK;
}

int sxmc_group_set_lut_output(sxmc_group_t g, int enable) {
  SX_REQUIRE(g, "null group");
  g->cfg_lut = enable ? 1 : 0;
  return SXMC_OK;
}

#if SXMC_MEASURE
int sxmc_measure_set_gated_step(sxmc_group_t g, sxmc_stream_t fill_stream, int node) {
  SX_REQUIRE(g && node >= 0 && node < 16, "bad arguments");
  g->split_fill_stream = (hipStream_t)fill_stream;
  g->split_node = node;
  return SXMC_OK;
}
int sxmc_measure_stream_fork(sxmc_stream_t from, sxmc_stream_t to) {
  SX_REQUIRE(from && to, "null stream");
  hipEvent_t ev = nullptr;
  SX_HIP(hipEventCreateWithFlags(&ev, hipEventDisableTiming));
  SX_HIP(hipEventRecord(ev, (hipStream_t)from));
  SX_HIP(hipStreamWaitEvent((hipStream_t)to, ev, 0));
  return SXMC_OK;
}

int sxmc_group_set_debug_mode(sxmc_group_t g, int mode) {
  SX_REQUIRE(g, "null group");
  g->debug_mode = mode;
  return SXMC_OK;
}
#endif

int sxmc_group_eval_async(sxmc_group_t g, int do_eval_pdf, sxmc_stream_t s) {
  SX_FLUSH();
  SX_ORDER(s);
  SX_REQUIRE(g, "null group");
  int rc = group_refresh(g);
  if (rc) return rc;
  rc = group_check_bound(g, do_eval_pdf != 0);
  if (rc) return rc;
  hipStream_t st = (hipStream_t)s;
  g->last_stream = st;
  const bool sparse = do_eval_pdf && g->sparse_ready && g->cfg_sparse;
  rc = group_fill(g, st, sparse);
  if (rc) return rc;
  if (do_eval_pdf && g->max_points > 0) {
    SX_HIP(sx_launch_eval_pdf(sparse ? g->d_descs_sparse : g->d_descs, (int)g->members.size(), g->max_points, st));
  }
  return SXMC_OK;
}

int sxmc_group_eval_nll_async(sxmc_group_t g, sxmc_stream_t s, const double* d_pars, const double* d_nexpected,
                              const unsigned* d_n_mc, const short* d_source_id, const unsigned* d_norms,
                              double* d_sums, int* npartial_out) {
  SX_FLUSH();
  SX_ORDER(s);
  SX_REQUIRE(g && d_pars && d_nexpected && d_n_mc && d_source_id && d_norms && d_sums && npartial_out,
             "null argument");
  int rc = group_refresh(g);
  if (rc) return rc;
  rc = group_check_bound(g, true);
  if (rc) return rc;
  if (!g->same_points) return fail(SXMC_ERR_STATE, "members do not share one set of evaluation points");
  hipStream_t st = (hipStream_t)s;
  g->last_stream = st;
  const bool sparse = g->sparse_ready && g->cfg_sparse;
  if (!g->cfg_lut) {
    rc = ensure_event_classes(g, sparse);
    if (rc) return rc;
  }
  rc = group_fill(g, st, sparse);
  if (rc) return rc;
  SX_REQUIRE(g->members.size() <= 1024, "too many members for the fused evaluation");
  unsigned long long ne = g->members[0]->npoints;
  const SxSignalDesc* descs = sparse ? g->d_descs_sparse : g->d_descs;
  const unsigned* weight = nullptr;
  if (!g->cfg_lut) {
    rc = ensure_event_classes(g, sparse);
    if (rc) return rc;
    const sxmc_group::EventClasses& ec = g->ec[sparse ? 1 : 0];
    ne = ec.K;
    descs = ec.d_descs;
    weight = ec.d_weight;
  }
  const int block = 128;
  const int grid = (int)std::min<unsigned long long>(1024, std::max<unsigned long long>(1, (ne + block - 1) / block));
  SX_HIP(sx_launch_eval_nll(descs, (int)g->members.size(), ne, weight, d_pars, d_nexpected, d_n_mc, d_source_id,
                            d_norms, d_sums, grid, block, st));
  *npartial_out = grid;
  return SXMC_OK;
}

int sxmc_group_mcmc_step_async(sxmc_group_t g, sxmc_stream_t s, const double* d_means, const double* d_sigmas,
                               sxmc_rng_state* d_rng, double* d_nll_current, double* d_nll_proposed,
                               double* d_v_current, double* d_v_proposed, int* d_accepted, int* d_counter,
                               float* d_jump_buffer, int nparameters, size_t nsources, const float* d_jump_width,
                               const double* d_nexpected, const unsigned* d_n_mc, const short* d_source_id,
                               const unsigned* d_norms, int debug_mode) {
  SX_FLUSH();
  SX_ORDER(s);
  SX_REQUIRE(g && d_means && d_sigmas && d_rng && d_nll_current && d_nll_proposed && d_v_current && d_v_proposed &&
                 d_accepted && d_counter && d_jump_buffer && d_jump_width && d_nexpected && d_n_mc && d_source_id &&
                 d_norms,
             "null argument");
  SX_REQUIRE(nparameters > 0, "nparameters must be positive");
  int rc = group_refresh(g);
  if (rc) return rc;
  rc = group_check_bound(g, true);
  if (rc) return rc;
  if (!g->same_points) return fail(SXMC_ERR_STATE, "members do not share one set of evaluation points");
  SX_REQUIRE(g->members.size() <= 1024, "too many members for the fused step");
  hipStream_t st = (hipStream_t)s;
  g->last_stream = st;
  const bool sparse = g->sparse_ready && g->cfg_sparse;
  unsigned long long ne = g->members[0]->npoints;
  const SxSignalDesc* descs = sparse ? g->d_descs_sparse : g->d_descs;
  const unsigned* weight = nullptr;
  if (!g->cfg_lut) {
    rc = ensure_event_classes(g, sparse);
    if (rc) return rc;
    const sxmc_group::EventClasses& ec = g->ec[sparse ? 1 : 0];
    ne = ec.K;
    descs = ec.d_descs;
    weight = ec.d_weight;
  }
  rc = group_fill(g, st, sparse);
  if (rc) return rc;
  const int block = 128;
  const int grid = (int)std::min<unsigned long long>(1024, std::max<unsigned long long>(1, (ne + block - 1) / block));
  SxStepArgs a;
  a.nsignals = g->members.size();
  a.nsources = nsources;
  a.means = d_means;
  a.sigmas = d_sigmas;
  a.rng = d_rng;
  a.nll_current = d_nll_current;
  a.nll_proposed = d_nll_proposed;
  a.v_current = d_v_current;
  a.v_proposed = d_v_proposed;
  a.accepted = d_accepted;
  a.counter = d_counter;
  a.jump_buffer = d_jump_buffer;
  a.nparameters = nparameters;
  a.debug_mode = debug_mode;
  a.jump_width = d_jump_width;
  a.nexpected = d_nexpected;
  a.n_mc = d_n_mc;
  a.source_id = d_source_id;
  a.norms = d_norms;
// ... 234 lines not shown

int sxmc_group_last_step_launches(sxmc_group_t g, int* launches) {
  SX_REQUIRE(g && launches, "null argument");
  *launches = g->last_step_launches;
  return SXMC_OK;
}

int sxmc_group_set_tail_kernel(sxmc_group_t g, int enable) {
  SX_REQUIRE(g, "null group");
  g->cfg_tail = enable ? 1 : 0;
  return SXMC_OK;
}

int sxmc_group_set_cooperative_step_end(sxmc_group_t g, int enable) {
  SX_REQUIRE(g, "null group");
  g->cfg_coop = enable ? 1 : 0;
  return SXMC_OK;
}

int sxmc_group_set_fused_step(sxmc_group_t g, int enable) {
  SX_REQUIRE(g, "null group");
  g->cfg_fused = enable ? 1 : 0;
  return SXMC_OK;
}

int sxmc_group_step_end_timeouts(sxmc_group_t g, sxmc_stream_t s, unsigned* timeouts) {
  SX_REQUIRE(g && timeouts, "null argument");
  SX_FLUSH();
  if (int rc_ = settle()) return rc_;
  if (s) {
    SX_HIP(hipMemcpyAsync(timeouts, g->d_ticket + 6, sizeof(unsigned), hipMemcpyDeviceToHost, (hipStream_t)s));
    SX_HIP(hipStreamSynchronize((hipStream_t)s));
  } else {
    SX_HIP(hipMemcpy(timeouts, g->d_ticket + 6, sizeof(unsigned), hipMemcpyDeviceToHost));
  }
  if (*timeouts != 0u) {
    hipStream_t st = (hipStream_t)s;
    SX_HIP(hipStreamSynchronize(g->last_stream));
    SX_HIP(sx_step_end_slots_init(g->d_coop_slots, g->d_coop_last, 128));
    SX_HIP(hipMemsetAsync(g->d_ticket, 0, 256, st));
    SX_HIP(hipStreamSynchronize(st));
    g->prezeroed = 0;
    for (sxmc_hist* h : g->members) h->cleared_by = nullptr;
    g->cfg_coop = 0;
  }
  return SXMC_OK;
}

int sxmc_rtc_compile_check(int nobs, int nslot, int lds_hist, int pre_width, int sparse_runs, const unsigned* ops,
                           int nops, size_t* code_bytes) {
  SX_REQUIRE(nops >= 0 && nops <= SXMC_MAX_SYST && (ops || nops == 0), "bad program");
  SxRtcSpec k{};
  k.nobs = nobs;
  k.nslot = nslot;
  k.lds_hist = lds_hist;
  k.pre_width = pre_width;
  k.sparse_runs = sparse_runs;
  k.nops = nops;
  for (int i = 0; i < nops; i++) k.ops[i] = ops[i];
  std::string err;
  if (!sx_rtc_compile_only(k, code_bytes, &err)) return fail(SXMC_ERR_HIP, err);
  return SXMC_OK;
}

int sxmc_rtc_compile_check_lockstep(int nobs, int nslot, int pre_width, int nchains, const unsigned* ops, int nops,
                                    size_t* code_bytes) {
  SX_REQUIRE(nops >= 0 && nops <= SXMC_MAX_SYST && (ops || nops == 0) && nchains >= 2 && nchains <= 4, "bad program");
  SxRtcSpec k{};
  k.nobs = nobs;
  k.nslot = nslot;
  k.lds_hist = 1;
  k.pre_width = pre_width;
  k.nchain = nchains;
  k.nops = nops;
  for (int i = 0; i < nops; i++) k.ops[i] = ops[i];
  std::string err;
  if (!sx_rtc_compile_only(k, code_bytes, &err)) return fail(SXMC_ERR_HIP, err);
  return SXMC_OK;
}

int sxmc_group_synchronize(sxmc_group_t g) {
  SX_FLUSH();
  if (int rc_ = settle()) return rc_;
  SX_REQUIRE(g, "null group");
  SX_HIP(hipStreamSynchronize(g->last_stream));
  return SXMC_OK;
}

int sxmc_group_profile(sxmc_group_t g, int enable, int capacity) {
  SX_REQUIRE(g, "null group");
  g->prof = enable != 0;
  g->prof_n = 0;
  if (g->prof) {
    if (capacity < 1) capacity = 1;
    while ((int)g->ev0.size() < capacity) {
      hipEvent_t a, b;
      SX_HIP(hipEventCreate(&a));
      SX_HIP(hipEventCreate(&b));
      g->ev0.push_back(a);
      g->ev1.push_back(b);
    }
  }
  return SXMC_OK;
}

int sxmc_group_profile_read(sxmc_group_t g, double* fill_ms_total, int* nlaunches) {
  SX_REQUIRE(g && fill_ms_total && nlaunches, "null argument");
  double tot = 0;
  for (int i = 0; i < g->prof_n; i++) {
    SX_HIP(hipEventSynchronize(g->ev1[i]));
    float ms = 0;
    SX_HIP(hipEventElapsedTime(&ms, g->ev0[i], g->ev1[i]));
    tot += ms;
  }
  *fill_ms_total = tot;
  *nlaunches = g->prof_n;
  return SXMC_OK;
}

int sxmc_group_algorithmic_bytes(sxmc_group_t g, double* fill_read, double* hist, double* event) {
  SX_REQUIRE(g && fill_read && hist && event, "null argument");
  int rc = group_refresh(g);
  if (rc) return rc;
  if (g->twin && !g->twin->classes.empty() && g->cfg_box < 0 && g->fill_form == 2) {
    double fr2 = 0, hb2 = 0, ev2 = 0, fr1 = 0;
    rc = sxmc_group_algorithmic_bytes(g->twin, &fr2, &hb2, &ev2);
    if (rc) return rc;
    g->fill_form = 1;
    rc = sxmc_group_algorithmic_bytes(g, &fr1, hist, event);
    g->fill_form = 2;
    *fill_read = fr2;
    return rc;
  }
  double fr = 0, hb = 0, ev = 0;
  for (size_t i = 0; i < g->members.size(); i++) {
    const sxmc_hist* h = g->members[i];
    const SxSignalDesc& d = g->h_descs[i];
    int pre_w = 0, pre_dims = 0;
    bool codes = false;
    for (const LaunchClass& c : g->classes) {
      for (int idx : c.member_idx) {
        if (idx == (int)i && c.shape.pre_width) {
          pre_w = c.shape.pre_width;
          for (int k = 0; k < d.nobs; k++) pre_dims += (c.pre_mask >> k) & 1u;
        }
        if (idx == (int)i) codes = c.codes;
      }
    }
    if (const SampleStore::Bucketed* bk = i < g->member_bucket.size() ? g->member_bucket[i] : nullptr) {
      const bool ord = bk->sort && bk->sort->ordered >= 0;
      const bool box = ord && bk->sort->box_truth >= 0;
      const double row_bytes = (codes && bk->d_qcol) ? (bk->q16 ? 2.0 : 4.0 * (double)((bk->nq + 1) / 2))
                                                     : 4.0 * (double)(bk->fields.size() - (ord ? 1 : 0));
      fr += (double)bk->nkept * row_bytes + ((box ? 16.0 : ord ? 8.0 : 0.0) + (bk->runs > 1 ? 8.0 : 4.0)) * (double)bk->ngranules;
    } else {
      fr += (double)h->nsamples * (4.0 * (d.nslot - pre_dims) + pre_w);
    }
    if (h->total_nbins <= kLdsMaxBins) {
      hb += 4.0 * (double)h->total_nbins;
    } else if (g->sparse_ready && g->cfg_sparse) {
      hb += 2.0 * 4.0 * (double)std::max(h->ntargets, 1);
    } else {
      hb += 2.0 * 4.0 * (double)h->total_nbins;
    }
    ev += 16.0 * (double)d.npoints;
  }
  *fill_read = fr;
  *hist = hb;
  *event = ev;
  return SXMC_OK;
}

}
```

sxmc_amd/csrc/sxmc_host.h:

```cpp
#pragma once

#include <hip/hip_runtime.h>

#include <algorithm>
#include <atomic>
#include <chrono>
#include <climits>
#include <cmath>
#include <cstdio>
#include <cstdlib>
#include <cstring>
#include <memory>
#include <mutex>
#include <shared_mutex>
#include <string>
#include <thread>
#include <vector>

#include <rocprofiler-sdk-roctx/roctx.h>

#include "sxmc_device.h"
#include "sxmc_plan.h"

extern "C" {
hipError_t sx_nll_init_rngs(int, int, hipStream_t, int, unsigned long long, sxmc_rng_state*);
hipError_t sx_nll_philox_dump(hipStream_t, sxmc_rng_state*, unsigned*, int);
hipError_t sx_nll_pick_new_vector(int, int, hipStream_t, int, sxmc_rng_state*, const float*, const double*,
                                  double*);
hipError_t sx_nll_jump_decider(int, int, hipStream_t, sxmc_rng_state*, double*, const double*, double*,
                               const double*, unsigned, int*, int*, float*);
hipError_t sx_nll_event_chunks(int, int, hipStream_t, const float*, const double*, size_t, size_t,
                               const double*, const unsigned*, const short*, const unsigned*, double*);
hipError_t sx_nll_event_reduce(int, hipStream_t, size_t, const double*, double*);
hipError_t sx_nll_total(hipStream_t, size_t, const double*, size_t, size_t, const double*, const double*,
                        const double*, const double*, const unsigned*, const short*, const unsigned*, double*);
hipError_t sx_nll_finish_combo(int, hipStream_t, size_t, const double*, size_t, size_t, const double*,
                               const double*, sxmc_rng_state*, double*, double*, double*, double*, int*, int*,
                               float*, int, const float*, const double*, const unsigned*, const short*,
                               const unsigned*, bool);
}


#ifndef SXMC_MEASURE
#define SXMC_MEASURE 0
#endif

struct sxmc_group;
struct sxmc_hist;

namespace sxhost {

extern thread_local std::string g_last_error;
extern thread_local bool t_capturing;
extern thread_local unsigned long long t_capture_epoch;
extern thread_local std::vector<sxmc_group*> t_capture_groups;
int fail(int code, const std::string& msg);
inline const char* measure_env(const char* name) {
#if SXMC_MEASURE
  return std::getenv(name);
#else
  (void)name;
  return nullptr;
#endif
}
bool tracing();
struct TraceRange {
  bool on;
  explicit TraceRange(const char* name) : on(tracing()) {
    if (on) roctxRangePushA(name);
  }
  ~TraceRange() {
    if (on) roctxRangePop();
  }
  TraceRange(const TraceRange&) = delete;
  TraceRange& operator=(const TraceRange&) = delete;
};


}

#define SX_HIP(expr)                                                                                                \
  do {                                                                                                              \
    hipError_t _e = (expr);                                                                                         \
    if (_e != hipSuccess) {                                                                                         \
      return ::sxhost::fail(SXMC_ERR_HIP, std::string(#expr) + ": " + hipGetErrorString(_e) + " (" __FILE__ ":" +    \
                                              std::to_string(__LINE__) + ")");                                       \
    }                                                                                                               \
  } while (0)

#define SX_REQUIRE(cond, msg)                                  \
  do {                                                         \
    if (!(cond)) return ::sxhost::fail(SXMC_ERR_INVALID, msg); \
  } while (0)

namespace sxhost {
constexpr int kLdsMaxBins = 40960 - 128;

struct HostSyst {
  int type, obs, extra_field;
  std::vector<short> pars;
};

struct DeviceProps {
  int cus = 0;
  int lds_per_cu = 0;
  bool valid = false;
};

int get_props(DeviceProps& p);
}

struct SampleStore {
  float* d_cols = nullptr;
  struct PreColumn {
    unsigned mask;
    int width;
    void* ptr;
  };
  std::vector<PreColumn> pre;
  std::mutex pre_mutex;
  void* find_pre(unsigned mask, int width) const {
    for (const PreColumn& p : pre)
      if (p.mask == mask && p.width == width) return p.ptr;
    return nullptr;
  }
  struct BucketSort {
    unsigned mask = 0;
    int ordered = -1;
    int box_truth = -1;
    bool rejected = true;
    unsigned* d_rows = nullptr;
    size_t nkept = 0;
    unsigned nkeys_total = 0;
    unsigned radix[SXMC_MAX_NFIELDS] = {0};
    std::vector<unsigned> keys;
    std::vector<unsigned> key_pre;
    std::vector<unsigned> lsrc, lvalid, lwhich;
  };
  struct Bucketed {
    unsigned mask = 0;
    std::vector<int> fields;
    int runs = 1;
    bool complete = false;
    const BucketSort* sort = nullptr;
    float* d_cols = nullptr;
    size_t pitch = 0;
    unsigned* d_gpre = nullptr;
    unsigned* d_gkp = nullptr;
    float* d_gedge = nullptr;
    float* d_gbox = nullptr;
    double box_dx = 0, box_dt = 0;
    bool q16 = false;
    size_t ngranules = 0;
    size_t nkept = 0;
    unsigned* d_qcol = nullptr;
    int nq = 0;
    bool codes_tried = false;
    double qbase[SXMC_MAX_QSLOTS] = {0}, qstep[SXMC_MAX_QSLOTS] = {0};
    unsigned long long q_exact_rows = 0, q_never_rows = 0;
  };
  std::vector<std::unique_ptr<BucketSort>> sorts;
  std::vector<std::unique_ptr<Bucketed>> bucketed;
  BucketSort* find_sort(unsigned mask, int ordered, int box_truth = -1) const {
    for (const auto& b : sorts)
      if (b->mask == mask && b->ordered == ordered && b->box_truth == box_truth) return b.get();
    return nullptr;
  }
  Bucketed* find_bucketed(const BucketSort* sort, const std::vector<int>& fields, int runs) const {
    for (const auto& b : bucketed)
      if (b->sort == sort && b->fields == fields && b->runs == runs) return b.get();
    return nullptr;
  }
  ~SampleStore() {
    if (d_cols) (void)hipFree(d_cols);
    for (PreColumn& p : pre) (void)hipFree(p.ptr);
    for (auto& b : bucketed) {
      if (b->d_cols) (void)hipFree(b->d_cols);
      if (b->d_gpre) (void)hipFree(b->d_gpre);
      if (b->d_gkp) (void)hipFree(b->d_gkp);
      if (b->d_gedge) (void)hipFree(b->d_gedge);
      if (b->d_gbox) (void)hipFree(b->d_gbox);
      if (b->d_qcol) (void)hipFree(b->d_qcol);
    }
    for (auto& b : sorts)
      if (b->d_rows) (void)hipFree(b->d_rows);
  }
};

struct sxmc_hist {
  std::shared_ptr<SampleStore> store;
  int nfields = 0, nobs = 0;
  size_t nsamples = 0, nvec = 0, pitch = 0;
  unsigned dataset = 0;
  std::vector<double> lower, upper, scale;
  std::vector<int> nbins, stride;
  int total_nbins = 0;
  double bin_volume = 0;
  unsigned* d_bins = nullptr;
  int* d_read_bins = nullptr;
  size_t read_bins_cap = 0;
  std::vector<void*> retired;
  unsigned* d_cdf = nullptr;
  float* d_sample = nullptr;
  size_t cap_sample = 0;
  bool has_points = false;
  size_t npoints = 0;
  float* pdf = nullptr;
  int pdf_off = 0, pdf_stride = 1;
  unsigned* norm = nullptr;
  int norm_off = 0;
  const double* params = nullptr;
  int par_off = 0, par_stride = 1;
  std::vector<sxhost::HostSyst> systs;
  hipStream_t stream = nullptr;
  unsigned long long version = 1;
  sxmc_group* self = nullptr;
  int cfg_threads = 0, cfg_bpc = 0;
  bool outputs_host_visible = false;
  bool want_optimize = true;
  unsigned* d_cnt = nullptr;
  int* d_read_slot = nullptr;
  unsigned* d_filter = nullptr;
  unsigned* d_table = nullptr;
  unsigned* d_coarse = nullptr;
  int ntargets = 0, filter_shift = 0, table_shift = 0, coarse_shift = 0;
  unsigned* d_bdir = nullptr;
  unsigned* d_btkeys = nullptr;
  unsigned* d_btslot = nullptr;
  unsigned btab_mask = 0;
  unsigned long long btab_points_version = 0;
  bool btab_valid = false;
  std::vector<unsigned> targets;
  std::vector<int> h_read_bins;
  std::vector<int> h_read_slot;
  unsigned long long points_version = 0;
  bool bins_valid = true;
  const sxmc_group* cleared_by = nullptr;
  std::shared_ptr<struct DeferredBatch> deferred;
  std::shared_ptr<struct BatchInFlight> inflight;
};

struct DeferredBatch {
  std::mutex m;
  std::vector<sxmc_hist*> members;
  std::atomic<size_t> n{0};
  int do_eval_pdf = 0;
  std::thread::id owner;
};

struct BatchInFlight {
  hipStream_t stream = nullptr;
  std::atomic<bool> done{false};
  bool host_visible = false;
};


namespace sxhost {
struct LaunchClass {
  SxLaunchShape shape;
  std::vector<unsigned> prog;
  bool prog_simple = false;
  unsigned pre_mask = 0;
  std::vector<int> member_idx;
  SxSignalDesc* d_descs = nullptr;
  SxSignalDesc* d_descs_sparse = nullptr;
  SxSegment* d_segs = nullptr;
  unsigned* d_blk_off = nullptr;
  unsigned long long total_vec = 0;
  int partition = 0;
  bool light = false;
  bool runs_mode = false;
  int teams = 1;
  bool codes = false;
  bool dual = false;
  float box_dx = 0, box_dt = 0;
  int box_obs = -1, box_truth = -1;
  unsigned padded_rstride = 0;
  unsigned plain_rstride = 0;
};

void free_class(LaunchClass& c);
}

struct sxmc_group {
  std::vector<sxmc_hist*> members;
  std::vector<unsigned long long> seen;
  std::vector<unsigned long long> seen_points;
  std::vector<SxSignalDesc> h_descs;
  SxSignalDesc* d_descs = nullptr;
  SxSignalDesc* d_descs_sparse = nullptr;
  bool sparse_ready = false;
  int max_bins_sparse = 0;
  int cfg_sparse = 1;
  std::vector<sxhost::LaunchClass> classes;
  int cfg_threads = 0, cfg_bpc = 0;
  int cfg_seen_threads = -1, cfg_seen_bpc = -1;
  int cfg_partition = 0, cfg_seen_partition = -1;
  int cfg_teams = 0, cfg_seen_teams = -1;
  int cfg_prebin = 1, cfg_seen_prebin = -1;
  int cfg_bucket = 1, cfg_seen_bucket = -1;
  bool order_blocked = false;
  int cfg_order = 1, cfg_seen_order = -1;
  int cfg_box = -1, cfg_seen_box = -2;
  bool box_blocked = false;
// ... 131 lines not shown
```

sxmc_amd/csrc/sxmc_launch_plan.cpp:

```cpp
#include "sxmc_host.h"

using namespace sxhost;

namespace sxhost {

using sxplan::apportion_workgroups;
std::vector<unsigned long long> unit_counts(const std::vector<SxSignalDesc>& descs) {
  std::vector<unsigned long long> nvec;
  for (const SxSignalDesc& d : descs) nvec.push_back(d.nvec);
  return nvec;
}
void interleaved_segments(const std::vector<SxSignalDesc>& descs, const std::vector<int>& K, int threads, int grid,
                          std::vector<SxSegment>& segs, std::vector<unsigned>& blk_off) {
  sxplan::interleaved_segments(unit_counts(descs), K, threads, grid, segs, blk_off);
}
void build_partition(const std::vector<SxSignalDesc>& descs, int grid, int threads, int want_mode,
                     std::vector<SxSegment>& segs, std::vector<unsigned>& blk_off, int& mode_out,
                     unsigned long long align = 1, int groups = 1) {
  sxplan::build_partition(unit_counts(descs), grid, threads, want_mode, segs, blk_off, mode_out, align, groups);
}


void member_slots(const sxmc_hist* h, std::vector<int>& slot_col) {
  slot_col.clear();
  for (int k = 0; k < h->nobs; k++) slot_col.push_back(k);
  std::vector<int> extra;
  for (const HostSyst& s : h->systs) {
    if (s.obs >= h->nobs) extra.push_back(s.obs);
    if (s.type == SXMC_SYST_RESOLUTION_SCALE && s.extra_field >= h->nobs) extra.push_back(s.extra_field);
  }
  std::sort(extra.begin(), extra.end());
  extra.erase(std::unique(extra.begin(), extra.end()), extra.end());
  for (int c : extra) slot_col.push_back(c);
}

int slot_of(const std::vector<int>& slot_col, int field) {
  for (size_t k = 0; k < slot_col.size(); k++)
    if (slot_col[k] == field) return (int)k;
  return 0;
}

void free_bucket_tables(sxmc_hist* h) {
  if (h->d_bdir) (void)hipFree(h->d_bdir);
  if (h->d_btkeys) (void)hipFree(h->d_btkeys);
  if (h->d_btslot) (void)hipFree(h->d_btslot);
  h->d_bdir = h->d_btkeys = h->d_btslot = nullptr;
  h->btab_valid = false;
}

void free_sparse(sxmc_hist* h) {
  free_bucket_tables(h);
  if (h->d_cnt) (void)hipFree(h->d_cnt);
  if (h->d_read_slot) (void)hipFree(h->d_read_slot);
  if (h->d_filter) (void)hipFree(h->d_filter);
  if (h->d_table) (void)hipFree(h->d_table);
  if (h->d_coarse) (void)hipFree(h->d_coarse);
  h->d_coarse = nullptr;
  h->d_cnt = nullptr;
  h->d_read_slot = nullptr;
  h->d_filter = nullptr;
  h->d_table = nullptr;
  h->ntargets = 0;
  h->targets.clear();
  h->h_read_slot.clear();
}

using sxplan::ceil_log2;

int build_sparse(sxmc_hist* h, const std::vector<int>& rb) {
  free_sparse(h);
  sxplan::SparseTables st;
  sxplan::build_sparse_tables(rb, st);
  const std::vector<unsigned>&targets = st.targets, &filter = st.filter, &table = st.table, &coarse = st.coarse;
  const std::vector<int>& slot = st.slot;
  const size_t T = targets.size();
  const int cbits = st.cbits, fbits = st.fbits, tbits = st.tbits;
  SX_HIP(hipMalloc((void**)&h->d_cnt, sizeof(unsigned) * std::max<size_t>(T, 4)));
  SX_HIP(hipMemset(h->d_cnt, 0, sizeof(unsigned) * std::max<size_t>(T, 4)));
  SX_HIP(hipMalloc((void**)&h->d_read_slot, sizeof(int) * std::max<size_t>(slot.size(), 1)));
  if (!slot.empty()) SX_HIP(hipMemcpy(h->d_read_slot, slot.data(), sizeof(int) * slot.size(), hipMemcpyHostToDevice));
  SX_HIP(hipMalloc((void**)&h->d_filter, sizeof(unsigned) * filter.size()));
  SX_HIP(hipMemcpy(h->d_filter, filter.data(), sizeof(unsigned) * filter.size(), hipMemcpyHostToDevice));
  SX_HIP(hipMalloc((void**)&h->d_table, sizeof(unsigned) * table.size()));
  SX_HIP(hipMemcpy(h->d_table, table.data(), sizeof(unsigned) * table.size(), hipMemcpyHostToDevice));
  SX_HIP(hipMalloc((void**)&h->d_coarse, sizeof(unsigned) * coarse.size()));
  SX_HIP(hipMemcpy(h->d_coarse, coarse.data(), sizeof(unsigned) * coarse.size(), hipMemcpyHostToDevice));
  h->h_read_slot = slot;
  h->coarse_shift = 32 - cbits;
  h->ntargets = (int)T;
  h->targets = targets;
  h->filter_shift = 32 - fbits;
  h->table_shift = 32 - tbits;
  return SXMC_OK;
}

void make_sparse_desc(const sxmc_hist* h, SxSignalDesc& d) {
  d.sparse_real_nbins = h->total_nbins;
  d.bins = h->d_cnt;
  d.total_nbins = std::max(h->ntargets, 1);
  d.read_bins = h->d_read_slot;
  d.sparse_filter = h->d_filter;
  d.sparse_table = h->d_table;
  d.sparse_filter_shift = h->filter_shift;
  d.sparse_table_shift = h->table_shift;
  d.sparse_coarse = h->d_coarse;
  d.sparse_coarse_shift = h->coarse_shift;
}

int fill_desc(const sxmc_hist* h, SxSignalDesc& d) {
  std::memset(&d, 0, sizeof(d));
  std::vector<int> slot_col;
  member_slots(h, slot_col);
  d.cols = h->store->d_cols;
  d.col_pitch = h->pitch;
  d.nsamples = h->nsamples;
  d.nvec = h->nvec;
  d.bins = h->d_bins;
  d.norm = h->norm ? h->norm + h->norm_off : nullptr;
  d.total_nbins = h->total_nbins;
  d.nobs = h->nobs;
  d.nslot = (int)slot_col.size();
  d.nsyst = (int)h->systs.size();
  d.param_stride = h->par_stride;
  d.params = h->params ? h->params + h->par_off : nullptr;
  for (int k = 0; k < d.nslot; k++) d.slot_col[k] = slot_col[k];
  for (int k = 0; k < h->nobs; k++) {
    d.nbins[k] = h->nbins[(size_t)k];
    d.bin_stride[k] = h->stride[k];
    d.lower[k] = h->lower[k];
    d.upper[k] = h->upper[k];
    d.scale[k] = h->scale[k];
  }
  int ncoef = 0;
  for (int s = 0; s < d.nsyst; s++) {
    const HostSyst& hs = h->systs[s];
    SxSystOp& op = d.syst[s];
    op.type = (short)hs.type;
    op.obs_slot = (short)slot_of(slot_col, hs.obs);
    op.extra_slot = (short)(hs.type == SXMC_SYST_RESOLUTION_SCALE ? slot_of(slot_col, hs.extra_field) : 0);
    op.npars = (short)hs.pars.size();
    op.coef_start = (short)ncoef;
    for (size_t i = 0; i < hs.pars.size(); i++) {
      op.pars[i] = hs.pars[i];
      if (ncoef < 64) d.coef_par[ncoef] = hs.pars[i];
      ncoef++;
    }
  }
  d.ncoef = ncoef;
  d.read_bins = h->has_points ? h->d_read_bins : nullptr;
  d.npoints = h->has_points ? h->npoints : 0;
  d.pdf_out = h->pdf ? h->pdf + h->pdf_off : nullptr;
  d.pdf_stride = h->pdf_stride;
  d.bin_volume = h->bin_volume;
  return SXMC_OK;
}

struct DevBuf {
  void* p = nullptr;
  ~DevBuf() {
    if (p) (void)hipFree(p);
  }
  hipError_t alloc(size_t bytes) { return hipMalloc(&p, bytes ? bytes : 16); }
  template <typename T>
  T* as() const {
    return static_cast<T*>(p);
  }
};

int box_strata() {
  static const int n = [] {
    const char* e = measure_env("SXMC_BOX_STRATA");
    return e ? std::min(std::max(std::atoi(e), 1), 16) : 2;
  }();
  return n;
}

int get_bucket_sort(sxmc_hist* h, const SxSignalDesc* d_full_desc, unsigned mask, int ordered,
                    const SampleStore::BucketSort** out, int box_truth = -1) {
  *out = nullptr;
  SampleStore& st = *h->store;
  std::lock_guard<std::mutex> lock(st.pre_mutex);
  if (SampleStore::BucketSort* have = st.find_sort(mask, ordered, box_truth)) {
    *out = have->rejected ? nullptr : have;
    return SXMC_OK;
  }
  st.sorts.push_back(std::make_unique<SampleStore::BucketSort>());
  SampleStore::BucketSort* b = st.sorts.back().get();
  b->mask = mask;
  b->ordered = ordered;
  b->box_truth = box_truth;
  const size_t n = h->nsamples;
  if (n == 0 || n > 0x7FFFFF00ull) return SXMC_OK;

  unsigned long long nkeys = 1;
  for (int k = h->nobs - 1; k >= 0; k--) {
    if (!((mask >> k) & 1u)) continue;
    b->radix[k] = (unsigned)nkeys;
    nkeys *= (unsigned long long)h->nbins[(size_t)k] + 1ull;
    if (nkeys > (1ull << 20)) return SXMC_OK;
  }
  const unsigned outside = (unsigned)nkeys;
  const int bits = ceil_log2((size_t)nkeys + 1);

  DevBuf keys0, keys1, rows0, dfirst;
  SX_HIP(keys0.alloc(n * 4));
  SX_HIP(keys1.alloc(n * 4));
  SX_HIP(rows0.alloc(n * 4));
  SX_HIP(hipMalloc((void**)&b->d_rows, n * 4));
  SX_HIP(dfirst.alloc((nkeys + 1) * 4));
  SX_HIP(hipMemset(dfirst.p, 0xFF, (nkeys + 1) * 4));
  const unsigned* order_rows = nullptr;
  DevBuf rows1;
  if (ordered >= 0) {
    SX_HIP(rows1.alloc(n * 4));
    if (box_truth >= 0) {
      const float* colx = st.d_cols + (size_t)ordered * h->pitch;
      const float* colt = st.d_cols + (size_t)box_truth * h->pitch;
      const int nstrata = box_strata();
      unsigned bounds[16] = {0};
      if (nstrata > 1) {
        SX_HIP(sx_box_keys(colx, colt, n, 1, 1, nullptr, keys0.as<unsigned>(), rows0.as<unsigned>(), nullptr));
        SX_HIP(sx_bucket_sort(keys0.as<unsigned>(), keys1.as<unsigned>(), rows0.as<unsigned>(), rows1.as<unsigned>(), n, 32,
                              nullptr));
        for (int k = 0; k + 1 < nstrata; k++) {
          SX_HIP(hipMemcpy(&bounds[k], keys1.as<unsigned>() + (size_t)((double)n * (k + 1) / nstrata), 4,
                           hipMemcpyDeviceToHost));
        }
      }
      SX_HIP(sx_box_keys(colx, colt, n, 2, nstrata, bounds, keys0.as<unsigned>(), rows0.as<unsigned>(), nullptr));
    } else {
      SX_HIP(sx_order_keys(st.d_cols + (size_t)ordered * h->pitch, n, keys0.as<unsigned>(),
                           rows0.as<unsigned>(), nullptr));
    }
    SX_HIP(sx_bucket_sort(keys0.as<unsigned>(), keys1.as<unsigned>(), rows0.as<unsigned>(), rows1.as<unsigned>(), n, 32,
                          nullptr));
    order_rows = rows1.as<unsigned>();
  }
  SX_HIP(sx_bucket_keys(d_full_desc, n, mask, b->radix, outside, order_rows, keys0.as<unsigned>(), rows0.as<unsigned>(),
                        nullptr));
  SX_HIP(sx_bucket_sort(keys0.as<unsigned>(), keys1.as<unsigned>(), rows0.as<unsigned>(), b->d_rows, n, bits, nullptr));
  SX_HIP(sx_bucket_first(keys1.as<unsigned>(), n, dfirst.as<unsigned>(), nullptr));
  std::vector<unsigned> first((size_t)nkeys + 1);
  SX_HIP(hipMemcpy(first.data(), dfirst.p, first.size() * 4, hipMemcpyDeviceToHost));

  sxplan::GranulePlan gp;
  sxplan::bucket_granules(first, outside, n, gp);
  if (!gp.worth_it) {
    (void)hipFree(b->d_rows);
    b->d_rows = nullptr;
    return SXMC_OK;
  }
  b->lsrc = gp.lsrc;
  b->lvalid = gp.lvalid;
  b->lwhich = gp.lwhich;
  b->keys = gp.present;
  b->nkeys_total = outside;
  b->nkept = gp.kept;
  sxplan::bucket_key_offsets(gp.present, mask, b->radix, h->nbins.data(), h->stride.data(), h->nobs, b->key_pre);
  b->rejected = false;
  *out = b;
  return SXMC_OK;
}

int get_bucketed(sxmc_hist* h, const SampleStore::BucketSort* bs, const std::vector<int>& fields, int runs,
                 const SampleStore::Bucketed** out) {
  *out = nullptr;
  SampleStore& st = *h->store;
  std::lock_guard<std::mutex> lock(st.pre_mutex);
  if (SampleStore::Bucketed* have = st.find_bucketed(bs, fields, runs)) {
    if (!have->complete) return fail(SXMC_ERR_HIP, "an earlier attempt to lay this table out failed");
    *out = have;
    return SXMC_OK;
  }
  SX_REQUIRE(!fields.empty() && runs >= 1, "bad bucketed layout request");
  const bool pack_rows = bs->ordered >= 0 && h->total_nbins <= kLdsMaxBins;
  st.bucketed.push_back(std::make_unique<SampleStore::Bucketed>());
  SampleStore::Bucketed* b = st.bucketed.back().get();
  b->mask = bs->mask;
  b->fields = fields;
  b->runs = runs;
  b->sort = bs;
  sxplan::BucketedLayout lay;
  sxplan::bucketed_layout(bs->lsrc, bs->lvalid, bs->lwhich, bs->keys, bs->key_pre, bs->nkeys_total, runs, pack_rows, lay);
  const size_t P = lay.P, A = lay.A;
  const std::vector<unsigned>&psrc = lay.psrc, &pvalid = lay.pvalid, &ppre = lay.ppre, &pkp = lay.pkp;
  b->ngranules = P;
  b->nkept = bs->nkept;
  b->pitch = std::max<size_t>(64, P * 256);
  DevBuf dsrc, dvalid;
  SX_HIP(hipMalloc((void**)&b->d_cols, sizeof(float) * b->pitch * fields.size()));
  SX_HIP(hipMalloc((void**)&b->d_gpre, sizeof(unsigned) * A));
  SX_HIP(hipMalloc((void**)&b->d_gkp, sizeof(unsigned) * 2 * A));
  SX_HIP(hipMemcpy(b->d_gpre, ppre.data(), sizeof(unsigned) * A, hipMemcpyHostToDevice));
  SX_HIP(hipMemcpy(b->d_gkp, pkp.data(), sizeof(unsigned) * 2 * A, hipMemcpyHostToDevice));
  SX_HIP(dsrc.alloc(A * 4));
  SX_HIP(dvalid.alloc(A * 4));
  SX_HIP(hipMemcpy(dsrc.p, psrc.data(), A * 4, hipMemcpyHostToDevice));
  SX_HIP(hipMemcpy(dvalid.p, pvalid.data(), A * 4, hipMemcpyHostToDevice));
  SX_HIP(sx_bucket_gather(st.d_cols, h->pitch, (int)fields.size(), fields.data(), bs->d_rows, dsrc.as<unsigned>(),
                          dvalid.as<unsigned>(), P, b->d_cols, b->pitch, nullptr));
  if (bs->ordered >= 0 && bs->box_truth >= 0) {
    SX_REQUIRE(fields.size() >= 2, "a boxed layout streams its observable and the truth field");
    SX_HIP(hipMalloc((void**)&b->d_gbox, sizeof(float) * 4 * A));
    SX_HIP(hipMemset(b->d_gbox, 0xFF, sizeof(float) * 4 * A));
    SX_HIP(sx_bucket_boxes(b->d_cols + (fields.size() - 1) * b->pitch, b->d_cols + (fields.size() - 2) * b->pitch,
                           dvalid.as<unsigned>(), P, b->d_gbox, nullptr));
    {
      std::vector<float> hb(4 * P);
      if (P) SX_HIP(hipMemcpy(hb.data(), b->d_gbox, sizeof(float) * 4 * P, hipMemcpyDeviceToHost));
      std::vector<double> ex, et;
      for (size_t p = 0; p < P; p++) {
        const float x0 = hb[4 * p], x1 = hb[4 * p + 1], t0 = hb[4 * p + 2], t1 = hb[4 * p + 3];
        if (!(std::isfinite(x0) && std::isfinite(x1) && std::isfinite(t0) && std::isfinite(t1))) continue;
        ex.push_back((double)x1 - (double)x0);
        et.push_back((double)t1 - (double)t0);
      }
      auto trimmed = [](std::vector<double>& v) {
        if (v.empty()) return 0.0;
        std::sort(v.begin(), v.end());
        const size_t keep = std::max<size_t>(1, v.size() * 9 / 10);
        double sum = 0;
        for (size_t i = 0; i < keep; i++) sum += v[i];
        return sum / (double)keep;
      };
      b->box_dx = trimmed(ex);
      b->box_dt = trimmed(et);
    }
  } else if (bs->ordered >= 0) {
    SX_HIP(hipMalloc((void**)&b->d_gedge, sizeof(float) * 2 * A));
    SX_HIP(hipMemset(b->d_gedge, 0, sizeof(float) * 2 * A));
    SX_HIP(sx_bucket_edges(b->d_cols + (fields.size() - 1) * b->pitch, dvalid.as<unsigned>(), P, b->d_gedge, nullptr));
  }
  SX_HIP(hipDeviceSynchronize());
  b->complete = true;
  *out = b;
  return SXMC_OK;
}

bool codes_enabled(const sxmc_group* g) {
  if (g->cfg_codes >= 0) return g->cfg_codes != 0;
  static const bool on = [] {
    const char* e = std::getenv("SXMC_CODES");
    return !e || std::atoi(e) != 0;
  }();
  return on;
}

int get_bucket_codes(sxmc_hist* h, const SampleStore::Bucketed* bkc, const SxSignalDesc& cd) {
  SampleStore& st = *h->store;
  std::lock_guard<std::mutex> lock(st.pre_mutex);
  SampleStore::Bucketed* b = const_cast<SampleStore::Bucketed*>(bkc);
  if (b->codes_tried) return SXMC_OK;
  b->codes_tried = true;
  const bool boxed = b->sort && b->sort->ordered >= 0 && b->sort->box_truth >= 0;
  const int nq = (int)b->fields.size() - ((b->sort && b->sort->ordered >= 0) ? 1 : 0) - (boxed ? 1 : 0);
  if ((boxed ? nq != 1 : nq < 2) || nq > SXMC_MAX_QSLOTS || b->ngranules == 0 || b->ngranules >= ((size_t)1 << 22) || !b->sort) {
    return SXMC_OK;
  }
  const unsigned long long n = (unsigned long long)b->ngranules * 256ull;
  float mm[2 * SXMC_MAX_NFIELDS];
  SX_HIP(sx_column_minmax(b->d_cols, b->pitch, nq, n, mm, nullptr));
  sxplan::CodeWindows cw;
  sxplan::code_windows(mm, nq, cd.nobs, cd.lower, cd.upper, cw);
  for (int m = 0; m < nq; m++) {
    b->qbase[m] = cw.base[(size_t)m];
    b->qstep[m] = cw.step[(size_t)m];
  }
  double ambiguous = 0;
  for (int m = 0; m < nq && m < cd.nobs; m++) ambiguous += (double)cd.nbins[m] * cw.step[(size_t)m] / (cd.upper[m] - cd.lower[m]);
  static const bool gate_lifted = [] {
    const char* e = measure_env("SXMC_CODES_GATE");
    return e && e[0] == '1';
  }();
  if (!(ambiguous <= 2e-3) && !gate_lifted) return SXMC_OK;
  if (hipMalloc((void**)&b->d_qcol, boxed ? sizeof(unsigned short) * b->pitch
                                          : sizeof(unsigned) * b->pitch * (size_t)((nq + 1) / 2)) != hipSuccess) {
    (void)hipGetLastError();
    b->d_qcol = nullptr;
    return SXMC_OK;
  }
  unsigned long long tally[2] = {0, 0};
  b->q16 = boxed;
  hipError_t e = boxed ? sx_column_codes16(b->d_cols, b->qbase[0], b->qstep[0], n, reinterpret_cast<unsigned short*>(b->d_qcol),
                                           tally, nullptr)
                       : sx_column_codes(b->d_cols, b->pitch, nq, b->qbase, b->qstep, n, b->d_qcol, tally, nullptr);
  if (e != hipSuccess || (double)tally[0] > 0.02 * (double)std::max<size_t>(b->nkept, 1)) {
    (void)hipFree(b->d_qcol);
    b->d_qcol = nullptr;
    if (e != hipSuccess) return fail(SXMC_ERR_HIP, std::string("codes of a bucketed table: ") + hipGetErrorString(e));
    return SXMC_OK;
  }
  b->nq = nq;
  b->q_exact_rows = tally[0];
  b->q_never_rows = tally[1];
  return SXMC_OK;
}

using sxplan::ordered_rstride_padded;
using sxplan::ordered_queue_bytes;
unsigned ordered_queue_log(size_t room, int cap) {
  unsigned qlog = 11;
  if (cap > 0) qlog = (unsigned)std::min(std::max(cap, (int)kMinQueueLog), 11);
  while (qlog >= kMinQueueLog && ordered_queue_bytes(qlog) > room) qlog--;
  return qlog >= kMinQueueLog ? qlog : 0;
}

int build_bucket_tables(sxmc_hist* h, const SampleStore::BucketSort* bs) {
  if (h->btab_valid && h->btab_mask == bs->mask && h->btab_points_version == h->points_version) return SXMC_OK;
  free_bucket_tables(h);
  sxplan::BucketTables bt;
  sxplan::bucket_tables(bs->nkeys_total, bs->mask, bs->radix, h->nbins.data(), h->stride.data(), h->nobs, h->targets, bt);
  const std::vector<unsigned>&dir = bt.dir, &tkeys = bt.tkeys, &tslot = bt.tslot;
  SX_HIP(hipMalloc((void**)&h->d_bdir, sizeof(unsigned) * dir.size()));
  SX_HIP(hipMemcpy(h->d_bdir, dir.data(), sizeof(unsigned) * dir.size(), hipMemcpyHostToDevice));
  SX_HIP(hipMalloc((void**)&h->d_btkeys, sizeof(unsigned) * std::max<size_t>(tkeys.size(), 4)));
  SX_HIP(hipMalloc((void**)&h->d_btslot, sizeof(unsigned) * std::max<size_t>(tkeys.size(), 4)));
  if (!tkeys.empty()) {
    SX_HIP(hipMemcpy(h->d_btkeys, tkeys.data(), sizeof(unsigned) * tkeys.size(), hipMemcpyHostToDevice));
    SX_HIP(hipMemcpy(h->d_btslot, tslot.data(), sizeof(unsigned) * tslot.size(), hipMemcpyHostToDevice));
  }
  h->btab_mask = bs->mask;
  h->btab_points_version = h->points_version;
  h->btab_valid = true;
  return SXMC_OK;
}

unsigned ordered_rstride(int max_bins) { return (((unsigned)max_bins + 63u) & ~63u) + 16u; }
size_t ordered_lds_bytes(int max_bins, int nchain, unsigned rlog) {
  return (4 + ((size_t)nchain * ordered_rstride(max_bins) << rlog) + 64) * 4;
}

void compact_desc(const SxSignalDesc& full, const std::vector<int>& keep, int nobs2, SxSignalDesc& cd, int ordered = -1) {
  cd = full;
  if (ordered >= 0) {
    cd.bin_stride[nobs2] = full.bin_stride[ordered];
    cd.nbins[nobs2] = full.nbins[ordered];
    cd.lower[nobs2] = full.lower[ordered];
    cd.upper[nobs2] = full.upper[ordered];
    cd.scale[nobs2] = full.scale[ordered];
  }
  int nslot = 0;
  for (int k = 0; k < full.nslot; k++) {
    if (keep[(size_t)k] < 0) continue;
    const int q = keep[(size_t)k];
    cd.slot_col[q] = q;
    if (q < nobs2) {
      cd.bin_stride[q] = full.bin_stride[k];
      cd.nbins[q] = full.nbins[k];
      cd.lower[q] = full.lower[k];
      cd.upper[q] = full.upper[k];
      cd.scale[q] = full.scale[k];
    }
    nslot++;
  }
  cd.nobs = nobs2;
  cd.nslot = nslot;
  for (int q = 0; q < full.nsyst; q++) {
    cd.syst[q].obs_slot = (short)keep[(size_t)full.syst[q].obs_slot];
    cd.syst[q].extra_slot =
        (short)(full.syst[q].type == SXMC_SYST_RESOLUTION_SCALE ? keep[(size_t)full.syst[q].extra_slot] : 0);
  }
}

bool fused_step_requested(const sxmc_group* g) {
  static const int env_default = [] {
    const char* e = std::getenv("SXMC_FUSED_STEP");
    return (e && e[0] == '1') ? 1 : 0;
  }();
// ... 833 lines not shown
```

sxmc_amd/csrc/sxmc_plan.h:

```cpp
#pragma once

#include <algorithm>
#include <cmath>
#include <cstddef>
#include <utility>
#include <vector>

#include "sxmc_device_types.h"

namespace sxplan {

inline int ceil_log2(size_t x) {
  int b = 0;
  while (((size_t)1 << b) < x) b++;
  return b;
}

inline bool apportion_workgroups(const std::vector<unsigned long long>& sizes, int grid, int threads,
                                 std::vector<int>& K) {
  K.assign(sizes.size(), 0);
  unsigned long long total = 0;
  for (unsigned long long n : sizes) total += n;
  if (total == 0) return true;
  int used = 0;
// ... 78 lines not shown
    for (size_t j = 0; j < nvec.size() && r0 < r1; j++) {
      const unsigned long long s0 = start, s1 = start + nvec[j];
      start = s1;
      if (s1 <= r0) continue;
      SxSegment sg{};
      sg.sig = (int)j;
      sg.v0 = r0 - s0;
      sg.v1 = std::min(r1, s1) - s0;
      sg.step = (unsigned long long)threads;
      segs.push_back(sg);
      r0 = std::min(r1, s1);
    }
    blk_off.push_back((unsigned)segs.size());
  }
  mode_out = 1;
}

inline void eval_point_bins(const float* points, size_t n, int D, const double* lower, const double* upper,
                            const double* scale, const int* stride, int total_nbins, unsigned dataset,
                            std::vector<int>& rb) {
  const size_t row = (size_t)D + 1;
  rb.resize(n);
  for (size_t ip = 0; ip < n; ip++) {
    bool in_domain = true;
    int bin_id = 0;
    for (int k = 0; k < D; k++) {
      const double element = points[row * ip + (size_t)k];
      if (!(element >= lower[k] && element < upper[k])) {
        in_domain = false;
        break;
      }
      bin_id += (int)((element - lower[k]) * scale[k]) * stride[k];
    }
    if (in_domain && (unsigned)bin_id >= (unsigned)total_nbins) in_domain = false;
    if (points[row * ip + (size_t)D] != (float)dataset) bin_id = -2;
    rb[ip] = in_domain ? bin_id : -1;
  }
}

struct SparseTables {
  std::vector<unsigned> targets;
  std::vector<int> slot;
  std::vector<unsigned> coarse, filter, table;
  int cbits = 0, fbits = 0, tbits = 0;
};

inline void build_sparse_tables(const std::vector<int>& rb, SparseTables& o) {
  o.targets.clear();
  for (int b : rb)
    if (b >= 0) o.targets.push_back((unsigned)b);
  std::sort(o.targets.begin(), o.targets.end());
  o.targets.erase(std::unique(o.targets.begin(), o.targets.end()), o.targets.end());
  const size_t T = o.targets.size();
  o.slot.resize(rb.size());
  for (size_t i = 0; i < rb.size(); i++) {
    o.slot[i] = rb[i] < 0 ? rb[i]
                          : (int)(std::lower_bound(o.targets.begin(), o.targets.end(), (unsigned)rb[i]) - o.targets.begin());
  }
  o.fbits = std::min(26, std::max(16, ceil_log2(64 * std::max<size_t>(T, 1))));
  o.tbits = std::max(6, ceil_log2(2 * std::max<size_t>(T, 1)));
  o.cbits = std::min(20, std::max(10, ceil_log2(16 * std::max<size_t>(T, 1))));
  o.coarse.assign((size_t)1 << (o.cbits - 5), 0u);
  o.filter.assign((size_t)1 << (o.fbits - 5), 0u);
  o.table.assign((size_t)2 << o.tbits, 0xFFFFFFFFu);
  const unsigned mask = (1u << o.tbits) - 1u;
  for (size_t t = 0; t < T; t++) {
    const unsigned bin = o.targets[t];
    const unsigned hb = (bin * 0x9E3779B1u) >> (32 - o.fbits);
    o.filter[hb >> 5] |= 1u << (hb & 31u);
    const unsigned hc = (bin * 0xC2B2AE35u) >> (32 - o.cbits), hd = (bin * 0x27D4EB2Fu) >> (32 - o.cbits);
    o.coarse[hc >> 5] |= 1u << (hc & 31u);
    o.coarse[hd >> 5] |= 1u << (hd & 31u);
    unsigned hp = (bin * 0x85EBCA6Bu) >> (32 - o.tbits);
    while (o.table[2 * (size_t)hp] != 0xFFFFFFFFu) hp = (hp + 1u) & mask;
    o.table[2 * (size_t)hp] = bin;
    o.table[2 * (size_t)hp + 1] = (unsigned)t;
  }
}

struct GranulePlan {
  std::vector<unsigned> present;
  std::vector<unsigned> lsrc, lvalid, lwhich;
  size_t kept = 0;
  bool worth_it = false;
};

inline void bucket_granules(const std::vector<unsigned>& first, unsigned outside, size_t n, GranulePlan& g) {
  g = GranulePlan();
  g.kept = first[outside] != 0xFFFFFFFFu ? first[outside] : n;
  for (unsigned k = 0; k < outside; k++)
    if (first[k] != 0xFFFFFFFFu) g.present.push_back(k);
  for (size_t i = 0; i < g.present.size(); i++) {
    const size_t lo = first[g.present[i]], hi = i + 1 < g.present.size() ? first[g.present[i + 1]] : g.kept;
    for (size_t at = lo; at < hi; at += 256) {
      g.lsrc.push_back((unsigned)at);
      g.lvalid.push_back((unsigned)std::min<size_t>(256, hi - at));
      g.lwhich.push_back((unsigned)i);
    }
  }
  g.worth_it = !((double)g.lsrc.size() * 256.0 > 1.3 * (double)g.kept + 16384.0);
  if (!g.worth_it) {
    g.lsrc.clear();
    g.lvalid.clear();
    g.lwhich.clear();
  }
}

inline void bucket_key_offsets(const std::vector<unsigned>& present, unsigned mask, const unsigned* radix,
                               const int* nbins, const int* stride, int nobs, std::vector<unsigned>& key_pre) {
  key_pre.resize(present.size());
  for (size_t i = 0; i < present.size(); i++) {
    long long pre = 0;
    for (int k = 0; k < nobs; k++) {
      if (!((mask >> k) & 1u)) continue;
      const unsigned idx = (present[i] / radix[k]) % ((unsigned)nbins[k] + 1u);
      pre += (long long)idx * stride[k];
    }
    key_pre[i] = (unsigned)pre;
  }
}

struct BucketedLayout {
  std::vector<unsigned> psrc, pvalid, ppre, pkp;
  size_t P = 0, A = 1;
};

inline void bucketed_layout(const std::vector<unsigned>& lsrc, const std::vector<unsigned>& lvalid,
                            const std::vector<unsigned>& lwhich, const std::vector<unsigned>& keys,
                            const std::vector<unsigned>& key_pre, unsigned outside, int runs, bool pack_rows,
                            BucketedLayout& o) {
  const size_t L = lsrc.size();
  const size_t T = (L + (size_t)runs - 1) / (size_t)runs;
  o.P = T * (size_t)runs;
  o.A = std::max<size_t>(o.P, 1);
  o.psrc.assign(o.A, 0u);
  o.pvalid.assign(o.A, 0u);
  o.ppre.assign(o.A, 0u);
  o.pkp.assign(2 * o.A, 0u);
  for (size_t p = 0; p < o.P; p++) {
    const size_t r = p % (size_t)runs, t = p / (size_t)runs, l = r * T + t;
    if (l < L) {
      o.psrc[p] = lsrc[l];
      o.pvalid[p] = lvalid[l];
      o.ppre[p] = key_pre[lwhich[l]];
      if (pack_rows) o.ppre[p] |= (lvalid[l] - 1u) << 24;
      o.pkp[2 * p] = keys[lwhich[l]];
    } else {
      o.pkp[2 * p] = L ? keys[lwhich[L - 1]] : outside;
    }
    o.pkp[2 * p + 1] = o.ppre[p];
  }
}

struct BucketTables {
  std::vector<unsigned> dir, tkeys, tslot;
};

inline void bucket_tables(unsigned nkeys, unsigned mask, const unsigned* radix, const int* nbins, const int* stride,
                          int D, const std::vector<unsigned>& targets, BucketTables& o) {
  o.dir.assign(2 * ((size_t)nkeys + 1), 0u);
  o.tkeys.clear();
  o.tslot.clear();
  for (size_t k = 0; k <= nkeys; k++) o.dir[2 * k + 1] = SXMC_SPARSE_EMPTY;
  for (unsigned key = 0; key < nkeys; key++) {
    for (int k = 0; k < D; k++) {
      if (!((mask >> k) & 1u)) continue;
      if ((key / radix[k]) % ((unsigned)nbins[k] + 1u) == (unsigned)nbins[k]) o.dir[2 * (size_t)key + 1] = SXMC_SPARSE_SLOW;
    }
  }
  std::vector<std::vector<std::pair<unsigned, unsigned>>> by_key;
  std::vector<int> where((size_t)nkeys, -1);
  for (size_t t = 0; t < targets.size(); t++) {
    const unsigned flat = targets[t];
    unsigned key = 0, pre = 0;
    for (int k = 0; k < D; k++) {
      if (!((mask >> k) & 1u)) continue;
      const unsigned idx = (flat / (unsigned)stride[k]) % (unsigned)nbins[k];
      key += idx * radix[k];
      pre += idx * (unsigned)stride[k];
    }
    if (where[key] < 0) {
      where[key] = (int)by_key.size();
      by_key.emplace_back();
    }
    by_key[(size_t)where[key]].push_back({flat - pre, (unsigned)t});
  }
  for (unsigned key = 0; key < nkeys; key++) {
    if (where[key] < 0) continue;
    const auto& list = by_key[(size_t)where[key]];
    int lg = std::max(2, ceil_log2(4 * list.size()));
    if (lg > SXMC_SPARSE_SMAX_LOG2) lg = std::max(2, ceil_log2(2 * list.size()));
    if (lg > SXMC_SPARSE_SMAX_LOG2) {
      o.dir[2 * (size_t)key + 1] = SXMC_SPARSE_SLOW;
      continue;
    }
    const size_t off = o.tkeys.size(), S = (size_t)1 << lg, cells = S / 4;
    o.tkeys.resize(off + S, 0xFFFFFFFFu);
    o.tslot.resize(off + S, 0u);
    unsigned probes = 1;
    for (const auto& e : list) {
      size_t cell = lg > 2 ? (size_t)((e.first * 0x9E3779B1u) >> (34 - lg)) : 0;
      unsigned dist = 1;
      for (;; cell = (cell + 1) & (cells - 1), dist++) {
        size_t at = off + 4 * cell, free_slot = 4;
        for (size_t m = 0; m < 4; m++)
          if (o.tkeys[at + m] == 0xFFFFFFFFu) {
            free_slot = m;
            break;
          }
        if (free_slot < 4) {
          o.tkeys[at + free_slot] = e.first;
          o.tslot[at + free_slot] = e.second;
          break;
        }
      }
      probes = std::max(probes, dist);
    }
    if (probes > 255) {
      o.dir[2 * (size_t)key + 1] = SXMC_SPARSE_SLOW;
      continue;
    }
    lg |= (int)(probes << 8);
    o.dir[2 * (size_t)key] = (unsigned)off;
    o.dir[2 * (size_t)key + 1] = (unsigned)lg;
  }
}

struct EventClasses {
  size_t K = 0;
  std::vector<unsigned> first, weight;
  std::vector<int> tables;
};

inline void event_classes(const std::vector<const std::vector<int>*>& arr, size_t E, EventClasses& o) {
  const size_t S = arr.size();
  std::vector<int> distinct;
  for (size_t j = 0; j < S; j++) {
    bool seen = false;
    for (size_t q = 0; q < distinct.size() && !seen; q++) seen = *arr[(size_t)distinct[q]] == *arr[j];
    if (!seen) distinct.push_back((int)j);
  }
  std::vector<unsigned> order(E);
  for (size_t i = 0; i < E; i++) order[i] = (unsigned)i;
  auto less = [&](unsigned a, unsigned b) {
    for (int q : distinct) {
      const int x = (*arr[(size_t)q])[a], y = (*arr[(size_t)q])[b];
      if (x != y) return x < y;
    }
    return false;
  };
  auto same = [&](unsigned a, unsigned b) {
    for (int q : distinct)
      if ((*arr[(size_t)q])[a] != (*arr[(size_t)q])[b]) return false;
    return true;
  };
  std::sort(order.begin(), order.end(), less);
  o.first.clear();
  o.weight.clear();
  for (size_t i = 0; i < E; i++) {
    if (i > 0 && same(order[i - 1], order[i])) {
      o.weight.back()++;
    } else {
      o.first.push_back(order[i]);
      o.weight.push_back(1u);
    }
  }
  o.K = o.first.size();
  o.tables.assign(std::max<size_t>(S * o.K, 1), 0);
  for (size_t j = 0; j < S; j++)
    for (size_t k = 0; k < o.K; k++) o.tables[j * o.K + k] = (*arr[j])[o.first[k]];
}

struct CodeWindows {
  std::vector<double> base, step;
};
inline void code_windows(const float* minmax, int nfields, int nobs, const double* lower, const double* upper,
                         CodeWindows& o) {
  o.base.assign((size_t)nfields, 0.0);
  o.step.assign((size_t)nfields, 1.0);
  double ulo = 0, uhi = -1;
  for (int m = 0; m < nfields; m++) {
    double wlo = minmax[2 * m], whi = minmax[2 * m + 1];
    const bool none = !(wlo <= whi);
    if (m < nobs) {
      const double lo = lower[m], hi = upper[m], w = hi - lo;
      wlo = none ? lo - w : std::max(wlo, lo - w);
      whi = none ? hi + w : std::min(whi, hi + w);
      if (!(wlo < whi)) {
        wlo = lo - w;
        whi = hi + w;
      }
      if (uhi < ulo) {
        ulo = wlo;
        uhi = whi;
      } else {
        ulo = std::min(ulo, wlo);
        uhi = std::max(uhi, whi);
      }
    } else if (none) {
      wlo = 0;
      whi = 1;
    } else if (ulo <= uhi) {
      const double w = uhi - ulo, clo = std::max(wlo, ulo - 3 * w), chi = std::min(whi, uhi + 3 * w);
      if (clo < chi) {
        wlo = clo;
        whi = chi;
// ... 19 lines not shown
```

Measured before the change: 12760.

## Sort box-layout samples into core granules and bulk-fill bins whose image stays constant

```diff
diff --git a/sxmc_amd/csrc/fill_kernels.inc.h b/sxmc_amd/csrc/fill_kernels.inc.h
--- a/sxmc_amd/csrc/fill_kernels.inc.h
+++ b/sxmc_amd/csrc/fill_kernels.inc.h
@@ -526,6 +526,7 @@
 constexpr int kPreOrdered = 5;
 constexpr int kPreBoxed = 6;
 constexpr unsigned kOrdMixed = 0xFFFFFFFEu, kOrdSkip = 0xFFFFFFFFu;
+constexpr unsigned kBoxConst = 0x80000000u;
 typedef float vfloat2 __attribute__((ext_vector_type(2)));
 
 template <unsigned OPC>
@@ -1926,6 +1927,8 @@
     }
     gptr<const unsigned> precol = to_global(reinterpret_cast<const unsigned*>(d.pre));
     gptr<const vfloat4> boxes = to_global(reinterpret_cast<const vfloat4*>(d.boxes));
+    gptr<const vfloat2> redges = to_global(reinterpret_cast<const vfloat2*>(d.edges));
+    const bool has_edges = d.edges != nullptr;
     gptr<const vuint2g> qcol = to_global(d.qcol != nullptr ? reinterpret_cast<const vuint2g*>(d.qcol)
                                                            : reinterpret_cast<const vuint2g*>(d.cols));
     const unsigned vfirst32 = (unsigned)(v0 + tid), step32 = (unsigned)step, vlast32 = (unsigned)(v1 - 1);
@@ -1989,12 +1992,16 @@
 
     unsigned gword = kOrdSkip, greal = 0u;
     vfloat4 bx_next;
+    vfloat2 re_next;
     unsigned pre_next;
     auto meta_load = [&](unsigned it) {
       unsigned vg = vwave32 + (it + lane) * step32;
       vg = vg <= vlast32 ? vg : vlast32;
       bx_next = boxes[vg >> 6];
       pre_next = precol[vg >> 6];
+      const float nanv = __builtin_nanf("");
+      re_next = vfloat2{nanv, nanv};
+      if (has_edges) re_next = redges[vg >> 6];
     };
     auto granule_meta = [&](unsigned it) {
       unsigned vg = vwave32 + (it + lane) * step32;
@@ -2002,6 +2009,7 @@
       vg = live ? vg : vlast32;
       if constexpr (!SXMC_BOX_PREFETCH) meta_load(it);
       const vfloat4 bx = bx_next;
+      const vfloat2 re = re_next;
       const unsigned pre = pre_next;
       if constexpr (SXMC_BOX_PREFETCH) meta_load(it + 64u);
       double xl = (double)bx.x, xh = (double)bx.y;
@@ -2017,7 +2025,17 @@
       const bool canon = off < (1u << 22) && rem < s_in && (h + 1u) * s_out <= B;
       const bool mixed = !use_q || !fin || e0 != e1 || !canon;
       const bool skip = fin && e0 == e1 && (e0 < 0 || e0 == 0x7FFFFFFF);
-      gword = !live ? kOrdSkip : skip ? kOrdSkip : mixed ? kOrdMixed : h * s_in + rem;
+      double r0 = (double)re.x, r1 = (double)re.y;
+      run_ordered_scalar<0>(r0, craw, PROG{}, Seq{});
+      run_ordered_scalar<0>(r1, craw, PROG{}, Seq{});
+      const bool rfin = !wild && !(dbg & 128u) && (__builtin_fabs(r0) < __builtin_inf()) && (__builtin_fabs(r1) < __builtin_inf());
+      const int j0 = (int)((r0 - lo) * sc), j1 = (int)((r1 - lo) * sc);
+      const bool rin = rfin && (r0 >= lo) && (r0 < hi) && (r1 >= lo) && (r1 < hi) && j0 == j1 && (unsigned)j0 < nbk;
+      const bool rout = rfin && ((!(r0 >= lo) && !(r1 >= lo)) || (!(r0 < hi) && !(r1 < hi)));
+      const bool constant = rin && fin && e0 == e1 && canon && !skip;
+      gword = (!live || skip || rout) ? kOrdSkip
+              : constant ? (kBoxConst | (h * s_in + rem + ((unsigned)j0 + 1u) * oSp))
+              : mixed ? kOrdMixed : h * s_in + rem;
       greal = off;
     };
 
@@ -2210,6 +2228,11 @@
                 vcnt += (rq[i].x == 12345u && word0 == 77u) ? 1u : 0u;
               } else if (word0 < climit) coarse_unit(rq[i], iu, vfirst32 + iu * step32, word0);
               else if (word0 == kOrdMixed) push_granule(iu);
+              else if (word0 != kOrdSkip) {
+                if (lane == 0 && !(dbg & 64u)) {
+                  __hip_atomic_fetch_add(&hist[word0 & ~kBoxConst], 256u, __ATOMIC_RELAXED, __HIP_MEMORY_SCOPE_WORKGROUP);
+                }
+              }
             }
             issue(i, iu + (unsigned)kRing);
           }
diff --git a/sxmc_amd/csrc/layout_kernels.hip b/sxmc_amd/csrc/layout_kernels.hip
--- a/sxmc_amd/csrc/layout_kernels.hip
+++ b/sxmc_amd/csrc/layout_kernels.hip
@@ -81,6 +81,69 @@
     }
     keys[i] = key;
     rows[i] = (unsigned)i;
+  }
+}
+
+__global__ __launch_bounds__(256) void box_core_kernel(const float* __restrict__ colx, const float* __restrict__ colt,
+                                                       const float* __restrict__ colr,
+                                                       const unsigned* __restrict__ bucket_key, unsigned outside,
+                                                       SxCorePlan cp, unsigned long long n, int pass, BoxStrata strata,
+                                                       const unsigned* __restrict__ rows_in,
+                                                       unsigned* __restrict__ cell_count, const unsigned* __restrict__ cell_keep,
+                                                       unsigned* __restrict__ keys, unsigned* __restrict__ rows,
+                                                       unsigned char* __restrict__ row_core) {
+  const unsigned long long step = (unsigned long long)gridDim.x * blockDim.x;
+  for (unsigned long long i = (unsigned long long)blockIdx.x * blockDim.x + threadIdx.x; i < n; i += step) {
+    const unsigned row = pass == 0 ? (unsigned)i : rows_in[i];
+    const float x = colx[row], t = colt[row], r = colr[row];
+    const unsigned bk = bucket_key[row];
+    const int k = (bk != outside && fabsf(r) < __builtin_inff()) ? sx_core_bin(cp, x, t) : -1;
+    const unsigned cell = bk * (unsigned)cp.nbins + (unsigned)(k >= 0 ? k : 0);
+    if (pass == 0) {
+      if (k >= 0) atomicAdd(&cell_count[cell], 1u);
+      continue;
+    }
+    bool core = false;
+    if (k >= 0 && cell_keep[cell] != 0u) core = atomicAdd(&cell_count[cell], 1u) < cell_keep[cell];
+    const float d = x - t;
+    const unsigned ud = __float_as_uint(d), kd = (ud >> 31) ? ~ud : (ud | 0x80000000u);
+    const unsigned ux = __float_as_uint(x), kx = (ux >> 31) ? ~ux : (ux | 0x80000000u);
+    unsigned s = 0;
+    for (int q = 0; q + 1 < strata.n; q++) s += strata.bound[q] <= kd ? 1u : 0u;
+    keys[i] = core ? (unsigned)k : (d != d || x != x) ? 0xFFFFFFFFu : (0x80000000u | (s << 27) | (kx >> 5));
+    rows[i] = row;
+    row_core[row] = core ? 1 : 0;
+  }
+}
+
+__global__ __launch_bounds__(256) void box_split_key_kernel(unsigned* __restrict__ keys, const unsigned* __restrict__ rows,
+                                                            const unsigned char* __restrict__ row_core, unsigned outside,
+                                                            unsigned long long n) {
+  const unsigned long long step = (unsigned long long)gridDim.x * blockDim.x;
+  for (unsigned long long i = (unsigned long long)blockIdx.x * blockDim.x + threadIdx.x; i < n; i += step) {
+    const unsigned k = keys[i];
+    keys[i] = k >= outside ? 2u * outside : 2u * k + ((row_core[rows[i]] ? 0u : 1u) ^ (k & 1u));
+  }
+}
+
+__global__ __launch_bounds__(256) void bucket_core_edges_kernel(const float* __restrict__ colr,
+                                                                const unsigned* __restrict__ valid,
+                                                                unsigned long long ngranules, float* __restrict__ edges) {
+  const unsigned lane = threadIdx.x & 63u;
+  const unsigned long long wave = ((unsigned long long)blockIdx.x * blockDim.x + threadIdx.x) >> 6;
+  const unsigned long long nwaves = ((unsigned long long)gridDim.x * blockDim.x) >> 6;
+  for (unsigned long long p = wave; p < ngranules; p += nwaves) {
+    const float4 v = *reinterpret_cast<const float4*>(colr + p * 256ull + 4u * lane);
+    const float next = __shfl_down(v.x, 1, 64);
+    bool ok = valid[p] == 256u && fabsf(v.x) < __builtin_inff() && fabsf(v.w) < __builtin_inff() && v.x <= v.y &&
+              v.y <= v.z && v.z <= v.w && (lane == 63u || v.w <= next);
+    ok = __ballot(!ok) == 0ull;
+    const float first = __shfl(v.x, 0, 64), last = __shfl(v.w, 63, 64);
+    if (lane == 0) {
+      const float nanv = __int_as_float(0x7fc00000);
+      edges[2 * p] = ok ? first : nanv;
+      edges[2 * p + 1] = ok ? last : nanv;
+    }
   }
 }
 
@@ -353,6 +416,38 @@
   return hipGetLastError();
 }
 
+hipError_t sx_box_core_keys(const float* d_colx, const float* d_colt, const float* d_colr, const unsigned* d_bucket_key,
+                            unsigned outside, const SxCorePlan& cp, unsigned long long nsamples, int pass, int nstrata,
+                            const unsigned* bounds, const unsigned* d_rows_in, unsigned* d_cell_count,
+                            const unsigned* d_cell_keep, unsigned* d_keys, unsigned* d_rows, unsigned char* d_row_core,
+                            hipStream_t s) {
+  if (nsamples == 0) return hipSuccess;
+  if (nstrata < 1 || nstrata > 16 || cp.nbins < 1 || cp.nbins > SXMC_CORE_MAX_BINS) return hipErrorInvalidValue;
+  BoxStrata st{};
+  st.n = nstrata;
+  for (int k = 0; k + 1 < nstrata; k++) st.bound[k] = bounds ? bounds[k] : 0u;
+  hipLaunchKernelGGL(box_core_kernel, dim3(grid_for(nsamples, 16384)), dim3(256), 0, s, d_colx, d_colt, d_colr,
+                     d_bucket_key, outside, cp, nsamples, pass, st, d_rows_in, d_cell_count, d_cell_keep, d_keys, d_rows,
+                     d_row_core);
+  return hipGetLastError();
+}
+
+hipError_t sx_box_split_keys(unsigned* d_keys, const unsigned* d_rows, const unsigned char* d_row_core, unsigned outside,
+                             unsigned long long nsamples, hipStream_t s) {
+  if (nsamples == 0) return hipSuccess;
+  hipLaunchKernelGGL(box_split_key_kernel, dim3(grid_for(nsamples, 16384)), dim3(256), 0, s, d_keys, d_rows, d_row_core,
+                     outside, nsamples);
+  return hipGetLastError();
+}
+
+hipError_t sx_bucket_core_edges(const float* d_colr, const unsigned* d_valid, unsigned long long ngranules, float* d_edges,
+                                hipStream_t s) {
+  if (ngranules == 0) return hipSuccess;
+  hipLaunchKernelGGL(bucket_core_edges_kernel, dim3(grid_for(ngranules * 64ull, 16384)), dim3(256), 0, s, d_colr, d_valid,
+                     ngranules, d_edges);
+  return hipGetLastError();
+}
+
 hipError_t sx_bucket_boxes(const float* d_colx, const float* d_colt, const unsigned* d_valid, unsigned long long ngranules,
                            float* d_boxes, hipStream_t s) {
   if (ngranules == 0) return hipSuccess;
diff --git a/sxmc_amd/csrc/sxmc_device.h b/sxmc_amd/csrc/sxmc_device.h
--- a/sxmc_amd/csrc/sxmc_device.h
+++ b/sxmc_amd/csrc/sxmc_device.h
@@ -146,6 +146,15 @@
                        const unsigned* bounds, unsigned* d_keys, unsigned* d_rows, hipStream_t s);
 hipError_t sx_bucket_boxes(const float* d_colx, const float* d_colt, const unsigned* d_valid, unsigned long long ngranules,
                            float* d_boxes, hipStream_t s);
+hipError_t sx_box_core_keys(const float* d_colx, const float* d_colt, const float* d_colr, const unsigned* d_bucket_key,
+                            unsigned outside, const SxCorePlan& cp, unsigned long long nsamples, int pass, int nstrata,
+                            const unsigned* bounds, const unsigned* d_rows_in, unsigned* d_cell_count,
+                            const unsigned* d_cell_keep, unsigned* d_keys, unsigned* d_rows, unsigned char* d_row_core,
+                            hipStream_t s);
+hipError_t sx_box_split_keys(unsigned* d_keys, const unsigned* d_rows, const unsigned char* d_row_core, unsigned outside,
+                             unsigned long long nsamples, hipStream_t s);
+hipError_t sx_bucket_core_edges(const float* d_colr, const unsigned* d_valid, unsigned long long ngranules, float* d_edges,
+                                hipStream_t s);
 hipError_t sx_column_codes16(const float* col, double base, double step, unsigned long long n, unsigned short* qcol,
                              unsigned long long* tally, hipStream_t s);
 hipError_t sx_bucket_sort(const unsigned* keys_in, unsigned* keys_out, const unsigned* rows_in, unsigned* rows_out,
diff --git a/sxmc_amd/csrc/sxmc_device_types.h b/sxmc_amd/csrc/sxmc_device_types.h
--- a/sxmc_amd/csrc/sxmc_device_types.h
+++ b/sxmc_amd/csrc/sxmc_device_types.h
@@ -78,6 +78,30 @@
   unsigned* step_gate;
 };
 
+#define SXMC_CORE_MAX_BINS 64
+#if defined(__HIPCC__) || defined(__HIPCC_RTC__)
+#define SX_HD __host__ __device__
+#else
+#define SX_HD
+#endif
+struct SxCorePlan {
+  int nbins;
+  int pad;
+  double lower, upper, scale;
+  float D;
+  float in_lo[SXMC_CORE_MAX_BINS];
+  float in_hi[SXMC_CORE_MAX_BINS];
+};
+SX_HD inline int sx_core_bin(const SxCorePlan& cp, float xf, float tf) {
+  const float df = xf - tf;
+  if (!(df >= -cp.D && df <= cp.D)) return -1;
+  const double x = (double)xf;
+  if (!(x >= cp.lower && x < cp.upper)) return -1;
+  const int k = (int)((x - cp.lower) * cp.scale);
+  if (k < 0 || k >= cp.nbins) return -1;
+  return (xf >= cp.in_lo[k] && xf <= cp.in_hi[k]) ? k : -1;
+}
+
 struct SxSegment {
   int sig;
   int pad;
diff --git a/sxmc_amd/csrc/sxmc_group.cpp b/sxmc_amd/csrc/sxmc_group.cpp
--- a/sxmc_amd/csrc/sxmc_group.cpp
+++ b/sxmc_amd/csrc/sxmc_group.cpp
@@ -216,8 +216,9 @@
   return SXMC_OK;
 }
 
-static int box_image_width(sxmc_group* g, double* width) {
+static int box_image_width(sxmc_group* g, double* width, bool* core_ok) {
   *width = HUGE_VAL;
+  core_ok[0] = core_ok[1] = true;
   const LaunchClass* cls = nullptr;
   for (const LaunchClass& c : g->classes) cls = (c.dual && !cls) ? &c : cls;
   if (!cls || cls->member_idx.empty() || cls->box_obs < 0) return SXMC_OK;
@@ -260,6 +261,30 @@
     fin = std::isfinite(xl) && std::isfinite(xh);
   }
   if (fin) *width = (xh - xl) * d.scale[cls->box_obs];
+  int types[SXMC_MAX_SYST], nops = 0;
+  double coef[2][SXMC_MAX_SYST];
+  for (int q = 0; q < d.nsyst; q++) {
+    const SxSystOp& op = d.syst[q];
+    if (op.obs_slot != cls->box_obs) continue;
+    types[nops] = op.type;
+    coef[0][nops] = g->h_pin[(size_t)((int)op.pars[0] - lo_idx) * (size_t)d.param_stride];
+    coef[1][nops] = 1.25 * coef[0][nops];
+    nops++;
+  }
+  const int bo = cls->box_obs;
+  for (int idx : cls->member_idx) {
+    const SampleStore::Bucketed* bk = g->member_bucket[(size_t)idx];
+    if (!bk) continue;
+    for (size_t i = 0; i < bk->core_bin.size(); i++) {
+      const double* u = &bk->core_box[4 * i];
+      for (int w = 0; w < 2; w++) {
+        int b0 = 0, b1 = 0;
+        const bool ok = sxplan::box_image_bins(types, coef[w], nops, u[0], u[1], u[2], u[3], d.lower[bo], d.upper[bo],
+                                               d.scale[bo], &b0, &b1);
+        core_ok[w] = core_ok[w] && ok && b0 == bk->core_bin[i] && b1 == bk->core_bin[i];
+      }
+    }
+  }
   return SXMC_OK;
 }
 
@@ -274,9 +299,11 @@
   if (!(g->twin && !g->twin->classes.empty() && g->cfg_box < 0)) return SXMC_OK;
   SX_HIP(hipStreamSynchronize(g->last_stream));
   double width = HUGE_VAL;
-  rc = box_image_width(g, &width);
-  if (rc) return rc;
-  const int want = width < 0.8 * (double)g->box_limit ? 1 : (width < (double)g->box_limit ? g->fill_form : 2);
+  bool core_ok[2] = {true, true};
+  rc = box_image_width(g, &width, core_ok);
+  if (rc) return rc;
+  const int want = (width < 0.8 * (double)g->box_limit && core_ok[1]) ? 1
+                   : ((width < (double)g->box_limit && core_ok[0]) ? g->fill_form : 2);
   if (changed) *changed = want != g->fill_form ? 1 : 0;
   g->fill_form = want;
   if (form) *form = want;
@@ -374,6 +401,17 @@
                   c.runs_mode ? (c.shape.rtc_sparse ? "+runs(runtime)" : "+runs(builtin)") : "", c.shape.threads,
                   c.shape.grid, c.partition, c.teams);
     text += line;
+    if (c.shape.pre_width == 6) {
+      size_t ncore = 0, ngran = 0;
+      for (int idx : c.member_idx) {
+        const SampleStore::Bucketed* bk = (size_t)idx < plan->member_bucket.size() ? plan->member_bucket[(size_t)idx] : nullptr;
+        if (!bk) continue;
+        ncore += bk->ncore;
+        ngran += bk->ngranules;
+      }
+      text.pop_back();
+      text += " core_granules=" + std::to_string(ncore) + "/" + std::to_string(ngran) + "\n";
+    }
   }
   if (!g->rtc_note.empty()) text += "runtime specialisation failed: " + g->rtc_note.substr(0, 300) + "\n";
   if (!g->plan_note.empty()) text += "note: " + g->plan_note + "\n";
@@ -914,7 +952,7 @@
       const bool box = ord && bk->sort->box_truth >= 0;
       const double row_bytes = (codes && bk->d_qcol) ? (bk->q16 ? 2.0 : 4.0 * (double)((bk->nq + 1) / 2))
                                                      : 4.0 * (double)(bk->fields.size() - (ord ? 1 : 0));
-      fr += (double)bk->nkept * row_bytes + ((box ? 16.0 : ord ? 8.0 : 0.0) + (bk->runs > 1 ? 8.0 : 4.0)) * (double)bk->ngranules;
+      fr += (double)bk->nkept * row_bytes + ((box ? (bk->d_gedge ? 24.0 : 16.0) : ord ? 8.0 : 0.0) + (bk->runs > 1 ? 8.0 : 4.0)) * (double)bk->ngranules;
     } else {
       fr += (double)h->nsamples * (4.0 * (d.nslot - pre_dims) + pre_w);
     }
diff --git a/sxmc_amd/csrc/sxmc_host.h b/sxmc_amd/csrc/sxmc_host.h
--- a/sxmc_amd/csrc/sxmc_host.h
+++ b/sxmc_amd/csrc/sxmc_host.h
@@ -136,6 +136,9 @@
     std::vector<unsigned> keys;
     std::vector<unsigned> key_pre;
     std::vector<unsigned> lsrc, lvalid, lwhich;
+    SxCorePlan core = SxCorePlan();
+    int core_col = -1;
+    size_t core_rows = 0;
   };
   struct Bucketed {
     unsigned mask = 0;
@@ -150,6 +153,9 @@
     float* d_gedge = nullptr;
     float* d_gbox = nullptr;
     double box_dx = 0, box_dt = 0;
+    size_t ncore = 0;
+    std::vector<int> core_bin;
+    std::vector<double> core_box;
     bool q16 = false;
     size_t ngranules = 0;
     size_t nkept = 0;
diff --git a/sxmc_amd/csrc/sxmc_launch_plan.cpp b/sxmc_amd/csrc/sxmc_launch_plan.cpp
--- a/sxmc_amd/csrc/sxmc_launch_plan.cpp
+++ b/sxmc_amd/csrc/sxmc_launch_plan.cpp
@@ -167,6 +167,20 @@
   }
 };
 
+bool box_core_enabled() {
+  static const bool on = [] {
+    const char* e = measure_env("SXMC_BOX_CORE");
+    return !e || std::atoi(e) != 0;
+  }();
+  return on;
+}
+bool box_core_split_enabled() {
+  static const bool on = [] {
+    const char* e = measure_env("SXMC_BOX_CORE_SPLIT");
+    return !e || std::atoi(e) != 0;
+  }();
+  return on;
+}
 int box_strata() {
   static const int n = [] {
     const char* e = measure_env("SXMC_BOX_STRATA");
@@ -202,13 +216,14 @@
   const unsigned outside = (unsigned)nkeys;
   const int bits = ceil_log2((size_t)nkeys + 1);
 
-  DevBuf keys0, keys1, rows0, dfirst;
+  DevBuf keys0, keys1, rows0, dfirst, rowcore;
+  bool split = false;
   SX_HIP(keys0.alloc(n * 4));
   SX_HIP(keys1.alloc(n * 4));
   SX_HIP(rows0.alloc(n * 4));
   SX_HIP(hipMalloc((void**)&b->d_rows, n * 4));
-  SX_HIP(dfirst.alloc((nkeys + 1) * 4));
-  SX_HIP(hipMemset(dfirst.p, 0xFF, (nkeys + 1) * 4));
+  SX_HIP(dfirst.alloc((2 * nkeys + 1) * 4));
+  SX_HIP(hipMemset(dfirst.p, 0xFF, (2 * nkeys + 1) * 4));
   const unsigned* order_rows = nullptr;
   DevBuf rows1;
   if (ordered >= 0) {
@@ -218,7 +233,16 @@
       const float* colt = st.d_cols + (size_t)box_truth * h->pitch;
       const int nstrata = box_strata();
       unsigned bounds[16] = {0};
-      if (nstrata > 1) {
+      int colr = -1, nother = 0;
+      for (int k = 0; k < h->nobs; k++) {
+        if (((mask >> k) & 1u) || k == ordered) continue;
+        colr = k;
+        nother++;
+      }
+      const bool want_core = box_core_enabled() && nother == 1 && nkeys * (unsigned long long)SXMC_CORE_MAX_BINS < (1ull << 24);
+      const sxplan::CoreDesign design;
+      double coreD = 0.0;
+      if (nstrata > 1 || want_core) {
         SX_HIP(sx_box_keys(colx, colt, n, 1, 1, nullptr, keys0.as<unsigned>(), rows0.as<unsigned>(), nullptr));
         SX_HIP(sx_bucket_sort(keys0.as<unsigned>(), keys1.as<unsigned>(), rows0.as<unsigned>(), rows1.as<unsigned>(), n, 32,
                               nullptr));
@@ -226,8 +250,69 @@
           SX_HIP(hipMemcpy(&bounds[k], keys1.as<unsigned>() + (size_t)((double)n * (k + 1) / nstrata), 4,
                            hipMemcpyDeviceToHost));
         }
-      }
-      SX_HIP(sx_box_keys(colx, colt, n, 2, nstrata, bounds, keys0.as<unsigned>(), rows0.as<unsigned>(), nullptr));
+        if (want_core) {
+          unsigned q[2] = {0xFFFFFFFFu, 0xFFFFFFFFu};
+          SX_HIP(hipMemcpy(&q[0], keys1.as<unsigned>() + (size_t)((double)n * design.quantile), 4, hipMemcpyDeviceToHost));
+          SX_HIP(hipMemcpy(&q[1], keys1.as<unsigned>() + std::min(n - 1, (size_t)((double)n * (1.0 - design.quantile))), 4,
+                           hipMemcpyDeviceToHost));
+          for (unsigned kq : q) {
+            const unsigned u = (kq >> 31) ? (kq ^ 0x80000000u) : ~kq;
+            float f;
+            std::memcpy(&f, &u, 4);
+            coreD = (kq == 0xFFFFFFFFu || !std::isfinite(f)) ? HUGE_VAL : std::max(coreD, (double)std::fabs(f));
+          }
+        }
+      }
+      bool have_core = false;
+      if (want_core) {
+        int types[8], nops = 0;
+        bool ops_ok = true;
+        for (const HostSyst& hs : h->systs) {
+          if (hs.obs != ordered) continue;
+          if (nops == 8) {
+            ops_ok = false;
+            break;
+          }
+          types[nops++] = hs.type;
+        }
+        have_core = ops_ok && sxplan::core_plan(types, nops, h->nbins[(size_t)ordered], h->lower[(size_t)ordered],
+                                                h->upper[(size_t)ordered], h->scale[(size_t)ordered], coreD, design, b->core);
+      }
+      if (have_core) {
+        const unsigned ncells = (unsigned)nkeys * (unsigned)b->core.nbins;
+        DevBuf rowsR, keysB, dcount, dkeep;
+        SX_HIP(rowsR.alloc(n * 4));
+        SX_HIP(keysB.alloc(n * 4));
+        SX_HIP(dcount.alloc((size_t)ncells * 4));
+        SX_HIP(dkeep.alloc((size_t)ncells * 4));
+        const float* colrp = st.d_cols + (size_t)colr * h->pitch;
+        SX_HIP(sx_order_keys(colrp, n, keys0.as<unsigned>(), rows0.as<unsigned>(), nullptr));
+        SX_HIP(sx_bucket_sort(keys0.as<unsigned>(), keys1.as<unsigned>(), rows0.as<unsigned>(), rowsR.as<unsigned>(), n, 32,
+                              nullptr));
+        SX_HIP(sx_bucket_keys(d_full_desc, n, mask, b->radix, outside, nullptr, keysB.as<unsigned>(), rows0.as<unsigned>(),
+                              nullptr));
+        SX_HIP(hipMemset(dcount.p, 0, (size_t)ncells * 4));
+        SX_HIP(sx_box_core_keys(colx, colt, colrp, keysB.as<unsigned>(), outside, b->core, n, 0, nstrata, bounds, nullptr,
+                                dcount.as<unsigned>(), nullptr, nullptr, nullptr, nullptr, nullptr));
+        std::vector<unsigned> cnt(ncells);
+        SX_HIP(hipMemcpy(cnt.data(), dcount.p, (size_t)ncells * 4, hipMemcpyDeviceToHost));
+        for (unsigned& c : cnt) {
+          c = sxplan::core_keep_count(c, design.min_granules);
+          b->core_rows += c;
+        }
+        SX_HIP(hipMemcpy(dkeep.p, cnt.data(), (size_t)ncells * 4, hipMemcpyHostToDevice));
+        SX_HIP(hipMemset(dcount.p, 0, (size_t)ncells * 4));
+        SX_HIP(rowcore.alloc(n));
+        SX_HIP(sx_box_core_keys(colx, colt, colrp, keysB.as<unsigned>(), outside, b->core, n, 1, nstrata, bounds,
+                                rowsR.as<unsigned>(), dcount.as<unsigned>(), dkeep.as<unsigned>(), keys0.as<unsigned>(),
+                                rows0.as<unsigned>(), rowcore.as<unsigned char>(), nullptr));
+        split = box_core_split_enabled();
+        SX_HIP(hipDeviceSynchronize());
+        b->core_col = colr;
+      } else {
+        b->core = SxCorePlan();
+        SX_HIP(sx_box_keys(colx, colt, n, 2, nstrata, bounds, keys0.as<unsigned>(), rows0.as<unsigned>(), nullptr));
+      }
     } else {
       SX_HIP(sx_order_keys(st.d_cols + (size_t)ordered * h->pitch, n, keys0.as<unsigned>(),
                            rows0.as<unsigned>(), nullptr));
@@ -238,13 +323,19 @@
   }
   SX_HIP(sx_bucket_keys(d_full_desc, n, mask, b->radix, outside, order_rows, keys0.as<unsigned>(), rows0.as<unsigned>(),
                         nullptr));
-  SX_HIP(sx_bucket_sort(keys0.as<unsigned>(), keys1.as<unsigned>(), rows0.as<unsigned>(), b->d_rows, n, bits, nullptr));
+  if (split) SX_HIP(sx_box_split_keys(keys0.as<unsigned>(), rows0.as<unsigned>(), rowcore.as<unsigned char>(), outside, n, nullptr));
+  const unsigned outside2 = split ? 2u * outside : outside;
+  SX_HIP(sx_bucket_sort(keys0.as<unsigned>(), keys1.as<unsigned>(), rows0.as<unsigned>(), b->d_rows, n, bits + (split ? 1 : 0),
+                        nullptr));
   SX_HIP(sx_bucket_first(keys1.as<unsigned>(), n, dfirst.as<unsigned>(), nullptr));
-  std::vector<unsigned> first((size_t)nkeys + 1);
+  std::vector<unsigned> first((size_t)outside2 + 1);
   SX_HIP(hipMemcpy(first.data(), dfirst.p, first.size() * 4, hipMemcpyDeviceToHost));
 
   sxplan::GranulePlan gp;
-  sxplan::bucket_granules(first, outside, n, gp);
+  sxplan::bucket_granules(first, outside2, n, gp);
+  if (split) {
+    for (unsigned& k : gp.present) k /= 2u;
+  }
   if (!gp.worth_it) {
     (void)hipFree(b->d_rows);
     b->d_rows = nullptr;
@@ -305,15 +396,41 @@
     SX_HIP(hipMemset(b->d_gbox, 0xFF, sizeof(float) * 4 * A));
     SX_HIP(sx_bucket_boxes(b->d_cols + (fields.size() - 1) * b->pitch, b->d_cols + (fields.size() - 2) * b->pitch,
                            dvalid.as<unsigned>(), P, b->d_gbox, nullptr));
+    SX_HIP(hipMalloc((void**)&b->d_gedge, sizeof(float) * 2 * A));
+    SX_HIP(hipMemset(b->d_gedge, 0xFF, sizeof(float) * 2 * A));
+    if (bs->core.nbins > 0) SX_HIP(sx_bucket_core_edges(b->d_cols, dvalid.as<unsigned>(), P, b->d_gedge, nullptr));
     {
-      std::vector<float> hb(4 * P);
+      std::vector<float> hb(4 * P), he(2 * P);
       if (P) SX_HIP(hipMemcpy(hb.data(), b->d_gbox, sizeof(float) * 4 * P, hipMemcpyDeviceToHost));
+      if (P) SX_HIP(hipMemcpy(he.data(), b->d_gedge, sizeof(float) * 2 * P, hipMemcpyDeviceToHost));
       std::vector<double> ex, et;
+      const SxCorePlan& cp = bs->core;
+      std::vector<double> un((size_t)4 * (size_t)std::max(cp.nbins, 0));
+      std::vector<char> seen((size_t)std::max(cp.nbins, 0), 0);
       for (size_t p = 0; p < P; p++) {
         const float x0 = hb[4 * p], x1 = hb[4 * p + 1], t0 = hb[4 * p + 2], t1 = hb[4 * p + 3];
         if (!(std::isfinite(x0) && std::isfinite(x1) && std::isfinite(t0) && std::isfinite(t1))) continue;
+        const int k = std::isfinite(he[2 * p]) && (double)x0 >= cp.lower && (double)x0 < cp.upper
+                          ? (int)(((double)x0 - cp.lower) * cp.scale) : -1;
+        const double Dw = (double)cp.D * (1.0 + 0x1p-20);
+        if (k >= 0 && k < cp.nbins && x0 >= cp.in_lo[k] && x1 <= cp.in_hi[k] && (double)t0 >= (double)x0 - Dw &&
+            (double)t1 <= (double)x1 + Dw) {
+          double* u = &un[(size_t)4 * (size_t)k];
+          u[0] = seen[(size_t)k] ? std::min(u[0], (double)x0) : (double)x0;
+          u[1] = seen[(size_t)k] ? std::max(u[1], (double)x1) : (double)x1;
+          u[2] = seen[(size_t)k] ? std::min(u[2], (double)t0) : (double)t0;
+          u[3] = seen[(size_t)k] ? std::max(u[3], (double)t1) : (double)t1;
+          seen[(size_t)k] = 1;
+          b->ncore++;
+          continue;
+        }
         ex.push_back((double)x1 - (double)x0);
         et.push_back((double)t1 - (double)t0);
+      }
+      for (int k = 0; k < cp.nbins; k++) {
+        if (!seen[(size_t)k]) continue;
+        b->core_bin.push_back(k);
+        b->core_box.insert(b->core_box.end(), &un[(size_t)4 * (size_t)k], &un[(size_t)4 * (size_t)k] + 4);
       }
       auto trimmed = [](std::vector<double>& v) {
         if (v.empty()) return 0.0;
diff --git a/sxmc_amd/csrc/sxmc_plan.h b/sxmc_amd/csrc/sxmc_plan.h
--- a/sxmc_amd/csrc/sxmc_plan.h
+++ b/sxmc_amd/csrc/sxmc_plan.h
@@ -254,6 +254,155 @@
   }
 }
 
+inline void box_interval(int type, double c0, double& xl, double& xh, double tl, double th, bool& fin) {
+  const double pc = 0.0 + c0 * 1.0;
+  if (type == SXMC_SYST_SHIFT) {
+    xl = xl + pc;
+    xh = xh + pc;
+  } else if (type == SXMC_SYST_SCALE || type == SXMC_SYST_CTSCALE) {
+    const double s = 1 + pc;
+    const double a = type == SXMC_SYST_SCALE ? xl * s : 1 + (xl - 1) * s;
+    const double b = type == SXMC_SYST_SCALE ? xh * s : 1 + (xh - 1) * s;
+    xl = s >= 0.0 ? a : b;
+    xh = s >= 0.0 ? b : a;
+  } else if (type == SXMC_SYST_RESOLUTION_SCALE) {
+    const double dl = xl - th, dh = xh - tl, a = pc * dl, b = pc * dh;
+    const double ml = pc >= 0.0 ? a : b, mh = pc >= 0.0 ? b : a;
+    fin = fin && std::isfinite(dl) && std::isfinite(dh) && std::isfinite(ml) && std::isfinite(mh);
+    xl = xl + ml;
+    xh = xh + mh;
+  } else {
+    fin = false;
+  }
+  fin = fin && std::isfinite(xl) && std::isfinite(xh);
+}
+inline bool box_image_bins(const int* types, const double* coef, int nops, double xl, double xh, double tl, double th,
+                           double lower, double upper, double scale, int* b0, int* b1) {
+  bool fin = std::isfinite(xl) && std::isfinite(xh) && std::isfinite(tl) && std::isfinite(th);
+  for (int q = 0; q < nops && fin; q++) box_interval(types[q], coef[q], xl, xh, tl, th, fin);
+  if (!fin) return false;
+  *b0 = !(xl >= lower) ? -1 : (!(xl < upper) ? 0x7FFFFFFF : (int)((xl - lower) * scale));
+  *b1 = !(xh >= lower) ? -1 : (!(xh < upper) ? 0x7FFFFFFF : (int)((xh - lower) * scale));
+  return true;
+}
+
+struct CoreDesign {
+  double shift_bins = 0.02;
+  double scale = 0.01;
+  double res = 0.05;
+  double quantile = 0.025;
+  double stretch = 1.05;
+  double allowance = 1e-3;
+  unsigned min_granules = 4;
+};
+inline double core_design_half(const CoreDesign& ds, int type, double bin_width) {
+  return type == SXMC_SYST_SHIFT ? ds.shift_bins * bin_width : type == SXMC_SYST_RESOLUTION_SCALE ? ds.res : ds.scale;
+}
+inline bool core_box_holds(const int* types, int nops, const CoreDesign& ds, double xl, double xh, double tl, double th,
+                           double lower, double upper, double scale, int k) {
+  if (nops < 0 || nops > 8) return false;
+  const double w = 1.0 / scale;
+  for (unsigned corner = 0; corner < (1u << nops); corner++) {
+    double coef[8];
+    for (int q = 0; q < nops; q++) coef[q] = ((corner >> q) & 1u ? 1.0 : -1.0) * core_design_half(ds, types[q], w);
+    int b0, b1;
+    if (!box_image_bins(types, coef, nops, xl, xh, tl, th, lower, upper, scale, &b0, &b1)) return false;
+    if (b0 != k || b1 != k) return false;
+  }
+  return true;
+}
+inline bool core_plan(const int* types, int nops, int nbins, double lower, double upper, double scale, double D,
+                      const CoreDesign& ds, SxCorePlan& cp) {
+  cp = SxCorePlan();
+  if (nbins < 1 || nbins > SXMC_CORE_MAX_BINS || nops < 1 || nops > 8 || !(D > 0.0) || !std::isfinite(D) ||
+      !(scale > 0.0) || !std::isfinite(lower) || !std::isfinite(upper)) {
+    return false;
+  }
+  cp.nbins = nbins;
+  cp.lower = lower;
+  cp.upper = upper;
+  cp.scale = scale;
+  cp.D = (float)D;
+  const double w = 1.0 / scale, Dw = (double)cp.D * (1.0 + 0x1p-20);
+  bool any = false;
+  for (int k = 0; k < nbins; k++) {
+    cp.in_lo[k] = 1.0f;
+    cp.in_hi[k] = 0.0f;
+    const double lo = lower + k * w, hi = lower + (k + 1) * w;
+    double under = 0.0, over = 0.0;
+    bool ok = true;
+    for (unsigned corner = 0; corner < (1u << nops) && ok; corner++) {
+      double xl = lo, xh = hi;
+      bool fin = true;
+      for (int q = 0; q < nops && fin; q++) {
+        box_interval(types[q], ((corner >> q) & 1u ? 1.0 : -1.0) * core_design_half(ds, types[q], w), xl, xh, lo - Dw, hi + Dw, fin);
+      }
+      ok = fin;
+      under = std::max(under, lo - xl);
+      over = std::max(over, xh - hi);
+    }
+    if (!ok) continue;
+    const float a = std::nextafterf((float)(lo + ds.stretch * under + ds.allowance * w), INFINITY);
+    const float b = std::nextafterf((float)(hi - ds.stretch * over - ds.allowance * w), -INFINITY);
+    if (!(a <= b)) continue;
+    if (!core_box_holds(types, nops, ds, (double)a, (double)b, (double)a - Dw, (double)b + Dw, lower, upper, scale, k)) continue;
+    cp.in_lo[k] = a;
+    cp.in_hi[k] = b;
+    any = true;
+  }
+  if (!any) cp.nbins = 0;
+  return any;
+}
+inline unsigned core_keep_count(unsigned count, unsigned min_granules) {
+  const unsigned whole = count & ~255u;
+  return whole >= 256u * std::max(min_granules, 1u) ? whole : 0u;
+}
+
+struct CoreLayout {
+  std::vector<unsigned> order;
+  std::vector<int> cls;
+  std::vector<size_t> bucket_first;
+};
+inline void core_layout(const float* x, const float* t, const float* r, const unsigned* bucket, size_t n, unsigned outside,
+                        const SxCorePlan& cp, unsigned min_granules, CoreLayout& o) {
+  o = CoreLayout();
+  o.cls.assign(n, 0);
+  std::vector<unsigned> byr(n);
+  for (size_t i = 0; i < n; i++) byr[i] = (unsigned)i;
+  auto nan_last = [](float a, float b) { return (a == a) && (!(b == b) || a < b); };
+  std::stable_sort(byr.begin(), byr.end(), [&](unsigned a, unsigned b) { return nan_last(r[a], r[b]); });
+  const size_t nb = (size_t)std::max(cp.nbins, 1);
+  std::vector<unsigned> count((size_t)outside * nb, 0u), taken((size_t)outside * nb, 0u);
+  std::vector<int> bin(n, -1);
+  for (size_t i = 0; i < n; i++) {
+    if (bucket[i] == outside || cp.nbins < 1 || !std::isfinite(r[i])) continue;
+    bin[i] = sx_core_bin(cp, x[i], t[i]);
+    if (bin[i] >= 0) count[(size_t)bucket[i] * nb + (size_t)bin[i]]++;
+  }
+  for (unsigned row : byr) {
+    if (bin[row] < 0) continue;
+    const size_t cell = (size_t)bucket[row] * nb + (size_t)bin[row];
+    if (taken[cell] < core_keep_count(count[cell], min_granules)) {
+      taken[cell]++;
+      o.cls[row] = 1 + bin[row];
+    }
+  }
+  std::vector<unsigned> kept;
+  for (unsigned row : byr)
+    if (bucket[row] != outside) kept.push_back(row);
+  std::stable_sort(kept.begin(), kept.end(), [&](unsigned a, unsigned b) {
+    const bool ca = o.cls[a] != 0, cb = o.cls[b] != 0;
+    if (ca != cb) return ca;
+    if (ca) return o.cls[a] < o.cls[b];
+    return nan_last(x[a], x[b]);
+  });
+  std::stable_sort(kept.begin(), kept.end(), [&](unsigned a, unsigned b) { return bucket[a] < bucket[b]; });
+  o.order = kept;
+  for (size_t i = 0; i < kept.size(); i++)
+    if (i == 0 || bucket[kept[i]] != bucket[kept[i - 1]]) o.bucket_first.push_back(i);
+  o.bucket_first.push_back(kept.size());
+}
+
 struct BucketTables {
   std::vector<unsigned> dir, tkeys, tslot;
 };
```

Result: slower. 7337 (-42.5%).
